# ma-compbio/MATCHA

Measured on AMD Instinct MI355X. Metric: training hyperedges/sec at k∈{2..5}, embed_dim=64; 1/2/4/8 MI355X, higher is better.
Workload: dtype f32; 1 GPU; hg38_1mb bins (N=3067), k in {2,3,4,5} mixed-k zero-padded to L=5, embed_dim=64, front end=table, neg_num=3, dropout on, AdamW lr=1e-3, 400000 known hyperedges; parallelism=dp1, hipgraph=False, table_gradient_exchange=none, embedding_backward=float atomics, exchange_overlapped=False

## Files before the change

### matcha_amd/csrc/fused_bwd.hip

```cpp
#include <stdlib.h>
#include <string.h>

#include <type_traits>

#include "bf16x3.hpp"
#include "kernels.hpp"
#include "tail_reduce.hpp"
#include "fb_unfold.hpp"

namespace matcha {

typedef float f32x16 __attribute__((ext_vector_type(16)));

namespace {

constexpr int kLd = 68;
constexpr int kMaxChunks = 64;
constexpr int kRsrcRaw32 = 0x00020000;
constexpr uint32_t kOffPastAny = 0x80000000u;

#define ZR8(p)                                                                                           \
  do {                                                                                                   \
    *reinterpret_cast<float4*>(p) = make_float4(0.f, 0.f, 0.f, 0.f);                                     \
    *reinterpret_cast<float4*>((p) + 4) = make_float4(0.f, 0.f, 0.f, 0.f);                               \
  } while (0)


#define FB_PIN(addr, x) asm volatile("" : "+v"(addr), "+v"((x).a), "+v"((x).b), "+v"((x).c), "+v"((x).d))
template <int ML>
__device__ __forceinline__ void attn_row8_kv(const float* __restrict__ Qs, const float* __restrict__ Xs, const float* __restrict__ Fs,
                                             const float* __restrict__ xpad, const float* __restrict__ Ps, float* __restrict__ dSs, int li, int li0,
                                             int k, int n_pad, int sub, float inv_temp, V8& o, V8& gq, V8& accK, V8& accV) {
  const float padf = (float)n_pad;
  const bool hp = n_pad > 0;
  float p[ML], ds[ML], pp;
  {
    const float4 pa = *reinterpret_cast<const float4*>(&Ps[li * 8]), pb = *reinterpret_cast<const float4*>(&Ps[li * 8 + 4]);
    const float w[8] = {pa.x, pa.y, pa.z, pa.w, pb.x, pb.y, pb.z, pb.w};
#pragma unroll
    for (int j = 0; j < ML; ++j) p[j] = (j < k) ? w[j] : 0.f;
    pp = hp ? w[7] : 0.f;
  }
  const float ppf = padf * pp;
  const int ro0 = li0 * kLd + 8 * sub;
  const V8 go = ld8(&Fs[li * kLd + 8 * sub]);
  const V8 vp = ld8(xpad + 8 * sub);
  const float dsp_raw = group_sum8_dpp(dot8(go, vp));
  float sig = ppf * dsp_raw;
  o = scale8(ppf, vp);
  V8 a = scale8(ppf * dsp_raw, vp);
  V8 vn = ld8(&Xs[ro0]), vn2 = ld8(&Xs[ro0 + (1 < k ? 1 : 0) * kLd]);
#pragma unroll
  for (int j = 0; j < ML; ++j) {
    const V8 v = vn;
    vn = vn2;
    if (j + 2 < ML) {
      int ad = ro0 + (j + 2 < k ? j + 2 : 0) * kLd;
      FB_PIN(ad, o);
      vn2 = ld8(&Xs[ad]);
    }
    axpy8(o, p[j], v);
    const float d = group_sum8_dpp(dot8(go, v));
    ds[j] = d;
    const float wd = p[j] * d;
    sig += wd;
    axpy8(a, wd, v);
  }
#pragma unroll
  for (int j = 0; j < ML; ++j) ds[j] = p[j] * (ds[j] - sig) * inv_temp;
  const float dspf = padf * (pp * (dsp_raw - sig) * inv_temp);
  axpy8(accV, ppf, go);
  {
    const float ns = -sig;
    axpy8(a, ns, o);
    gq = scale8(inv_temp, a);
  }
  {
    int ad = li * kLd + 8 * sub;
    FB_PIN(ad, gq);
    const V8 q = ld8(&Qs[ad]);
    axpy8(accK, dspf, q);
  }
  if (sub == 1) {
    float* dst = dSs + li * 8;
    *reinterpret_cast<float4*>(dst) = make_float4(ds[0], ds[1 % ML], ML > 2 ? ds[2 % ML] : 0.f, ML > 3 ? ds[3 % ML] : 0.f);
    if (ML > 4) *reinterpret_cast<float4*>(dst + 4) = make_float4(ds[4 % ML], ML > 5 ? ds[5 % ML] : 0.f, ML > 6 ? ds[6 % ML] : 0.f, ML > 7 ? ds[7 % ML] : 0.f);
  }
}

#define FB_PIN1(addr, s) asm volatile("" : "+v"(addr), "+v"(s))
template <int ML>
__device__ __forceinline__ void attn_row8_v(const float* __restrict__ Qs, const float* __restrict__ Xs, const float* __restrict__ Ys, const float* __restrict__ Ds,
                                            const float* __restrict__ xpad, const float* __restrict__ ypad, const float* __restrict__ Ps, float* __restrict__ dSs,
                                            int li, int li0, int k, int n_pad, int sub, float inv_temp, V8& gq, V8& accK, V8& accU) {
  const float padf = (float)n_pad;
  const bool hp = n_pad > 0;
  float p[ML], ds[ML], pp;
  {
    const float4 pa = *reinterpret_cast<const float4*>(&Ps[li * 8]), pb = *reinterpret_cast<const float4*>(&Ps[li * 8 + 4]);
    const float w[8] = {pa.x, pa.y, pa.z, pa.w, pb.x, pb.y, pb.z, pb.w};
#pragma unroll
    for (int j = 0; j < ML; ++j) p[j] = (j < k) ? w[j] : 0.f;
    pp = hp ? w[7] : 0.f;
  }
  const float ppf = padf * pp;
  const int ro0 = li0 * kLd + 8 * sub;
  const V8 go = ld8(&Ds[li * kLd + 8 * sub]);
  const float dsp_raw = group_sum8_dpp(dot8(go, ld8(ypad + 8 * sub)));
  float sig = ppf * dsp_raw;
  {
    V8 vn = ld8(&Ys[ro0]), vn2 = ld8(&Ys[ro0 + (1 < k ? 1 : 0) * kLd]);
    float part = 0.f;
#pragma unroll
    for (int j = 0; j < ML; ++j) {
      const V8 v = vn;
      vn = vn2;
      if (j + 2 < ML) {
        int ad = ro0 + (j + 2 < k ? j + 2 : 0) * kLd;
        FB_PIN1(ad, part);
        vn2 = ld8(&Ys[ad]);
      }
      part = dot8(go, v);
      const float d = group_sum8_dpp(part);
      ds[j] = d;
      sig += p[j] * d;
    }
  }
#pragma unroll
  for (int j = 0; j < ML; ++j) ds[j] = p[j] * (ds[j] - sig) * inv_temp;
  const float dspf = padf * (pp * (dsp_raw - sig) * inv_temp);
  axpy8(accU, ppf, go);
  gq = scale8(dspf, ld8(xpad + 8 * sub));
  {
    V8 vn = ld8(&Xs[ro0]), vn2 = ld8(&Xs[ro0 + (1 < k ? 1 : 0) * kLd]);
#pragma unroll
    for (int j = 0; j < ML; ++j) {
      const V8 v = vn;
      vn = vn2;
      if (j + 2 < ML) {
        int ad = ro0 + (j + 2 < k ? j + 2 : 0) * kLd;
        FB_PIN(ad, gq);
        vn2 = ld8(&Xs[ad]);
      }
      axpy8(gq, ds[j], v);
    }
  }
  {
    int ad = li * kLd + 8 * sub;
    FB_PIN(ad, gq);
    const V8 q = ld8(&Qs[ad]);
    axpy8(accK, dspf, q);
  }
  if (sub == 1) {
    float* dst = dSs + li * 8;
    *reinterpret_cast<float4*>(dst) = make_float4(ds[0], ds[1 % ML], ML > 2 ? ds[2 % ML] : 0.f, ML > 3 ? ds[3 % ML] : 0.f);
    if (ML > 4) *reinterpret_cast<float4*>(dst + 4) = make_float4(ds[4 % ML], ML > 5 ? ds[5 % ML] : 0.f, ML > 6 ? ds[6 % ML] : 0.f, ML > 7 ? ds[7 % ML] : 0.f);
  }
}

template <int ML>
__device__ __forceinline__ void attn_col8(const float* __restrict__ Qs, const float* __restrict__ Fs, const float* __restrict__ Ps,
                                          const float* __restrict__ dSs, int li, int li0, int k, int sub, V8& gk, V8& gv) {
  const int jj = li - li0;
  gk = zero8();
  gv = zero8();
  const int ro0 = li0 * kLd + 8 * sub;
  V8 qn = ld8(&Qs[ro0]), gn = ld8(&Fs[ro0]);
#pragma unroll
  for (int i = 0; i < ML; ++i) {
    const V8 q = qn, go = gn;
    const int ri = li0 + (i < k ? i : 0);
    const float pl = Ps[ri * 8 + jj], dl = dSs[ri * 8 + jj];
    const float pij = (i < k) ? pl : 0.f, dsij = (i < k) ? dl : 0.f;
    if (i + 1 < ML) {
      int a = ro0 + (i + 1 < k ? i + 1 : 0) * kLd;
      FB_PIN(a, gk);
      qn = ld8(&Qs[a]); gn = ld8(&Fs[a]);
    }
    axpy8(gv, pij, go);
    axpy8(gk, dsij, q);
  }
}

#ifdef FB_TIMING
#define FB_T(i) do { const long long now__ = wall_clock64(); tph[i] += now__ - tlast; tlast = now__; } while (0)
#else
#define FB_T(i) do { } while (0)
#endif

#define MFMA16(A, B, C) __builtin_amdgcn_mfma_f32_16x16x4f32((A), (B), (C), 0, 0, 0)

constexpr int kWgSlabM = 2 * 4096 + 4 * 64;
constexpr int kVecOffM = 2 * 4096;
constexpr int kTileH = 32 * kLd;
constexpr int kPS = 80;
constexpr int kPlane = 32 * kPS;
constexpr int kPT = 3 * kPlane;
typedef Planes<kPS, 16> PL;
__device__ __forceinline__ Frag3 frag_row(const short* __restrict__ p) { return PL::row(p); }
__device__ __forceinline__ void frag_store(short* __restrict__ p, const Frag3& f) { PL::store(p, f); }
__device__ __forceinline__ Frag3 frag_col(const short* __restrict__ p) { return PL::col(p); }

struct FusedBwdHArgs {
  const float* X; const float* dDyn; const int32_t* count; const int32_t* half_meta; const int32_t* tok_pos;
  int L; int nhalves; int nchunks;
  const float* mB; const float* mM;
  float* dxh; int64_t tcap;
  int dx_atomic;
  float* wslab;
  const float* rimg;
  const int32_t* xrow;
  const float* rn; int64_t rn_head;
  const float* vn;
  float* dx_node;
};
constexpr size_t kBwdLdsBytes = (size_t)2 * kTileH * 4 + (size_t)4 * kPT * 2 + (64 + 256 + 256 + 32 + 32) * 4;
static_assert(2 * kBwdLdsBytes <= 160 * 1024, "two workgroups per CU");

template <int ML, bool NODE, bool VTAB = false>
__global__ __launch_bounds__(256) __attribute__((amdgpu_waves_per_eu(2, 2))) void fused_bwdh_kernel(FusedBwdHArgs g) {
  static_assert(NODE || !VTAB, "the value table belongs to the node route");
  extern __shared__ __attribute__((aligned(16))) float lds[];
  float* Xs = lds;
  float* Gs = lds + kTileH;
  short* Xp = reinterpret_cast<short*>(lds + 2 * kTileH);
  short* Dp = Xp + kPT;
  short* RBp = Dp + kPT;
  short* FBp = RBp + kPT;
  float* Rs = reinterpret_cast<float*>(RBp);
  float* Fs = reinterpret_cast<float*>(FBp);
  float* Ds = reinterpret_cast<float*>(Dp);
  float* ypad = Ds + kTileH;
  float* sm = reinterpret_cast<float*>(FBp + kPT);
  float* xpad = sm;
  float* dSs = xpad + 64;
  float* Ps = dSs + 256;
  int* tinfo = reinterpret_cast<int*>(Ps + 256);
  int* keys_s = tinfo + 32;

  const int tid = threadIdx.x, lane = tid & 63, wave = tid >> 6;
  const int c16 = lane & 15, kq = lane >> 4;
  const int fb = 16 * wave;
  const int srow = tid >> 4, sc4 = (tid & 15) * 4;

  int head, chunk;
  if ((g.nchunks & 7) == 0) {
    const int xcd = blockIdx.x & 7, j = blockIdx.x >> 3;
    head = j & 7;
    chunk = (j >> 3) * 8 + xcd;
  } else {
    head = blockIdx.x & 7;
    chunk = blockIdx.x >> 3;
  }
  const int tr = g.count[1];
  int nh = g.count[3];
  if (nh > g.nhalves) nh = g.nhalves;
  const int per = (nh + g.nchunks - 1) / g.nchunks;
  const int tile_lo = chunk * per;
  const int tile_hi = (tile_lo + per < nh) ? tile_lo + per : nh;
  const float inv_temp = 0.125f;
#ifdef FB_TIMING
  long long tph[8] = {0, 0, 0, 0, 0, 0, 0, 0};
  long long tlast = wall_clock64();
#endif

  if (tid < 16) {
    const float4 xv = *reinterpret_cast<const float4*>(g.X + (NODE ? (int64_t)0 : (int64_t)tr * 64) + sc4);
    if constexpr (NODE) {
      *reinterpret_cast<float4*>(&xpad[sc4]) = xv;
    } else {
      float m, rs;
      ln_row16(xv, m, rs);
      *reinterpret_cast<float4*>(&xpad[sc4]) = make_float4((xv.x - m) * rs, (xv.y - m) * rs, (xv.z - m) * rs, (xv.w - m) * rs);
    }
  }
  if constexpr (VTAB) {
    static_assert((size_t)(kTileH + 64) * 4 <= (size_t)kPT * 2, "dDyn rows + y_pad fit the Dp region");
    if (tid >= 64 && tid < 80) *reinterpret_cast<float4*>(&ypad[sc4]) = *reinterpret_cast<const float4*>(g.vn + (int64_t)head * g.rn_head + sc4);
  }

  f32x4 ab0 = {0.f, 0.f, 0.f, 0.f}, ab1 = ab0, ab2 = ab0, ab3 = ab0, am0 = ab0, am1 = ab0, am2 = ab0, am3 = ab0;
  V8 accK = zero8(), accV = zero8();
  f2 cd0 = {0.f, 0.f}, cd1 = cd0;
  V8 accR = zero8();

  const int4* meta = reinterpret_cast<const int4*>(g.half_meta);
  const int4 mzero = make_int4(0, 0, 0, 0);
  int4 mc = tile_lo < tile_hi ? meta[tile_lo] : mzero;
// ... 63 lines not shown
      const P3 p0__ = split2(dm__.x, dm__.y), p1__ = split2(dm__.z, dm__.w);                             \
      short* d__ = Dp + row__ * kPS + sc4;                                                               \
      *reinterpret_cast<u32x2*>(d__) = (u32x2){p0__.h, p1__.h}; *reinterpret_cast<u32x2*>(d__ + kPlane) = (u32x2){p0__.m, p1__.m}; \
      *reinterpret_cast<u32x2*>(d__ + 2 * kPlane) = (u32x2){p0__.l, p1__.l};                             \
    }                                                                                                    \
    cd0 += (f2){dm__.x, dm__.y}; cd1 += (f2){dm__.z, dm__.w};                                            \
  } while (0)
#define FBH_RIMG_GLOAD(HALF)                                                                             \
  do {                                                                                                   \
    const f32x4* r__ = reinterpret_cast<const f32x4*>(g.rimg + ((int64_t)(HALF) * MATCHA_N_HEAD + head) * kImgRecH);  \
    if (tid < 64) pn = __builtin_nontemporal_load(r__ + 512 + tid);                                      \
    if (!r_tab) { ri0 = __builtin_nontemporal_load(r__ + tid); ri1 = __builtin_nontemporal_load(r__ + 256 + tid); } \
  } while (0)
  Frag3 Mf[2], Bf[2];
  {
    if constexpr (NODE) { FBH_KEY_GLOAD(0, mc); FBH_KEY_GLOAD(1, mc); }
    FBH_ROWS_GLOAD(mc, false);
    if constexpr (NODE) { if (r_tab) FBH_R_GLOAD(); FBH_KEY_GLOAD(0, mn); FBH_KEY_GLOAD(1, mn); }
    if (tile_lo < tile_hi) FBH_RIMG_GLOAD(tile_lo);
    const float* mp = g.mM + (int64_t)head * 4096 + (8 * kq) * 64 + fb + c16;
    const float* bp = g.mB + (int64_t)head * 4096 + (8 * kq) * 64 + fb + c16;
#pragma unroll
    for (int s = 0; s < 2; ++s) {
      float vm[8], vb[8];
#pragma unroll
      for (int j = 0; j < 8; ++j) { vm[j] = mp[(32 * s + j) * 64]; vb[j] = bp[(32 * s + j) * 64]; }
      Mf[s] = split8(vm); Bf[s] = split8(vb);
    }
  }

#define FBH_STAGE(M, DXN)                                                                                \
  do {                                                                                                   \
    const int n_real = (M).y;                                                                            \
    FBH_ROW_STAGE(0); FBH_ROW_STAGE(1);                                                                  \
    if (tid < 32) tinfo[tid] = tid < n_real ? ((tid - (tpn & 255)) | (tpn & ~255)) : 0;                  \
    if (((DXN) || (VTAB && g.dx_node)) && tid < 32) keys_s[tid] = kyn;                                   \
    if constexpr (VTAB) {                                                                                \
      *reinterpret_cast<f32x4*>(&Fs[srow * kLd + sc4]) = yi0; *reinterpret_cast<f32x4*>(&Fs[(srow + 16) * kLd + sc4]) = yi1; \
    }                                                                                                    \
    if (r_tab) {                                                                                         \
      *reinterpret_cast<f32x4*>(&Rs[srow * kLd + sc4]) = ri0; *reinterpret_cast<f32x4*>(&Rs[(srow + 16) * kLd + sc4]) = ri1; \
    } else {                                                                                             \
      f32x4* d__ = reinterpret_cast<f32x4*>(&Rs[(lane & 31) * kLd + 8 * wave + 4 * (lane >> 5)]);        \
      d__[0] = ri0; d__[8] = ri1;                                                                        \
    }                                                                                                    \
    if (tid < 64) reinterpret_cast<f32x4*>(Ps)[tid] = pn;                                                \
  } while (0)
  if (tile_lo < tile_hi) FBH_STAGE(mc, false);

  auto walk = [&](auto dxn_c) __attribute__((always_inline)) {
  constexpr bool DXN = decltype(dxn_c)::value;
  for (int tile = tile_lo; tile < tile_hi; ++tile) {
    const int4 mnn = tile + 2 < tile_hi ? meta[tile + 2] : mzero;
    const int t0 = mc.x, n_real = mc.y;
    __syncthreads();
    FB_T(7);
    int tid_ = tid;
    asm volatile("" : "+v"(tid_));
    const int lane = tid_ & 63, wave = tid_ >> 6;
    const int c16 = lane & 15, kq = lane >> 4;
    const int fb = 16 * wave;
    const int srow = tid_ >> 4, sc4 = (tid_ & 15) * 4;
    const int sub = lane & 7;
    (void)srow; (void)sc4;
    if constexpr (!VTAB) {
      f32x4 acc0 = {0.f, 0.f, 0.f, 0.f}, acc1 = acc0;
      const short* dp = Dp + c16 * kPS + 8 * kq;
#pragma unroll
      for (int s = 0; s < 2; ++s) {
        const Frag3 b0 = frag_row(dp + 32 * s), b1 = frag_row(dp + 16 * kPS + 32 * s);
        acc0 = mma6(acc0, Mf[s], b0); acc1 = mma6(acc1, Mf[s], b1);
      }
      *reinterpret_cast<f32x4*>(&Fs[c16 * kLd + fb + 4 * kq]) = acc0;
      *reinterpret_cast<f32x4*>(&Fs[(16 + c16) * kLd + fb + 4 * kq]) = acc1;
      FB_T(1);
      __syncthreads();
      FB_T(7);
    }
    if constexpr (VTAB) {
      FB_T(1);
      V8 q0, k0, v0;
      const int la = wave * 8 + (lane >> 3);
      const bool acta = la < n_real;
      int ia = 0;
      if (acta) { ia = tinfo[la]; attn_row8_v<ML>(Rs, Xs, Fs, Ds, xpad, ypad, Ps, dSs, la, ia & 255, ia >> 8, g.L - (ia >> 8), sub, inv_temp, q0, accK, accV); }
      __builtin_amdgcn_sched_barrier(0);
      FB_T(2);
      __syncthreads();
      FB_T(7);
      if (acta) {
        attn_col8<ML>(Rs, Ds, Ps, dSs, la, ia & 255, ia >> 8, sub, k0, v0);
        st8(&Gs[la * kLd + 8 * sub], k0);
      } else {
        ZR8(&Gs[la * kLd + 8 * sub]);
        v0 = zero8(); q0 = zero8();
      }
      frag_store(FBp + la * kPS + 8 * sub, split8(v0));
      FB_T(3);
      __syncthreads();
      FB_T(7);
      frag_store(RBp + la * kPS + 8 * sub, split8(q0));
      accR.a += q0.a; accR.b += q0.b; accR.c += q0.c; accR.d += q0.d;
    } else {
      V8 o0, q0, k0, v0;
      const int la = wave * 8 + (lane >> 3);
      const bool acta = la < n_real;
      int ia = 0;
      if (acta) { ia = tinfo[la]; attn_row8_kv<ML>(Rs, Xs, Fs, xpad, Ps, dSs, la, ia & 255, ia >> 8, g.L - (ia >> 8), sub, inv_temp, o0, q0, accK, accV); }
      __builtin_amdgcn_sched_barrier(0);
      FB_T(2);
      __syncthreads();
      FB_T(7);
      if (acta) {
        attn_col8<ML>(Rs, Fs, Ps, dSs, la, ia & 255, ia >> 8, sub, k0, v0);
        k0.a += v0.a; k0.b += v0.b; k0.c += v0.c; k0.d += v0.d;
        st8(&Gs[la * kLd + 8 * sub], k0);
      } else {
        ZR8(&Gs[la * kLd + 8 * sub]);
      }
      FB_T(3);
      __syncthreads();
      FB_T(7);
      if (!acta) { o0 = zero8(); q0 = zero8(); }
      frag_store(FBp + la * kPS + 8 * sub, split8(o0));
      frag_store(RBp + la * kPS + 8 * sub, split8(q0));
      accR.a += q0.a; accR.b += q0.b; accR.c += q0.c; accR.d += q0.d;
    }
    FB_T(4);
    __syncthreads();
    FB_T(7);
    FBH_ROWS_GLOAD(mn, DXN);
    if constexpr (NODE) { if (r_tab) FBH_R_GLOAD(); FBH_KEY_GLOAD(0, mnn); FBH_KEY_GLOAD(1, mnn); }
    if constexpr (DXN) { if (tile + 1 < tile_hi) FBH_RIMG_GLOAD(tile + 1); }
    if (DXN || g.dx_atomic) {
      const float* gp = Gs + (4 * kq) * kLd + fb + c16;
      f32x4 dx0 = {gp[0], gp[kLd], gp[2 * kLd], gp[3 * kLd]};
      f32x4 dx1 = {gp[16 * kLd], gp[17 * kLd], gp[18 * kLd], gp[19 * kLd]};
      const short* arow = RBp + c16 * kPS + 8 * kq;
#pragma unroll
      for (int s = 0; s < 2; ++s) {
        const Frag3 a0 = frag_row(arow + 32 * s), a1 = frag_row(arow + 16 * kPS + 32 * s);
        dx0 = mma6(dx0, a0, Bf[s]); dx1 = mma6(dx1, a1, Bf[s]);
      }
      if constexpr (VTAB) {
        const short* urow = FBp + c16 * kPS + 8 * kq;
#pragma unroll
        for (int s = 0; s < 2; ++s) {
          const Frag3 a0 = frag_row(urow + 32 * s), a1 = frag_row(urow + 16 * kPS + 32 * s);
          dx0 = mma6(dx0, a0, Mf[s]); dx1 = mma6(dx1, a1, Mf[s]);
        }
      }
      if constexpr (DXN) {
        const int4 ka = *reinterpret_cast<const int4*>(&keys_s[4 * kq]), kb = *reinterpret_cast<const int4*>(&keys_s[16 + 4 * kq]);
        const int k0[4] = {ka.x, ka.y, ka.z, ka.w}, k1[4] = {kb.x, kb.y, kb.z, kb.w};
        const __amdgpu_buffer_rsrc_t ah = __builtin_amdgcn_make_buffer_rsrc(g.dx_node + (int64_t)head * g.rn_head, 0, (int)(g.rn_head * 4), kRsrcRaw32);
        const uint32_t col4 = 4u * (uint32_t)(fb + c16);
#pragma unroll
        for (int reg = 0; reg < 4; ++reg) {
          __builtin_amdgcn_raw_ptr_buffer_atomic_fadd_f32(dx0[reg], ah, 4 * kq + reg < n_real ? (uint32_t)k0[reg] * 256u + col4 : kOffPastAny, 0, 0);
          __builtin_amdgcn_raw_ptr_buffer_atomic_fadd_f32(dx1[reg], ah, 16 + 4 * kq + reg < n_real ? (uint32_t)k1[reg] * 256u + col4 : kOffPastAny, 0, 0);
        }
      } else {
      float* out = g.dxh + ((int64_t)t0 + 4 * kq) * 64 + fb + c16;
#pragma unroll
      for (int reg = 0; reg < 4; ++reg) {
        if (4 * kq + reg < n_real) unsafeAtomicAdd(out + reg * 64, dx0[reg]);
        if (16 + 4 * kq + reg < n_real) unsafeAtomicAdd(out + (16 + reg) * 64, dx1[reg]);
      }
      }
    } else {
      f32x4 dx0 = *reinterpret_cast<const f32x4*>(&Gs[c16 * kLd + fb + 4 * kq]);
      f32x4 dx1 = *reinterpret_cast<const f32x4*>(&Gs[(16 + c16) * kLd + fb + 4 * kq]);
      const short* arow = RBp + c16 * kPS + 8 * kq;
#pragma unroll
      for (int s = 0; s < 2; ++s) {
        const Frag3 a0 = frag_row(arow + 32 * s), a1 = frag_row(arow + 16 * kPS + 32 * s);
        dx0 = mma6(dx0, Bf[s], a0); dx1 = mma6(dx1, Bf[s], a1);
      }
      if constexpr (VTAB) {
        const short* urow = FBp + c16 * kPS + 8 * kq;
#pragma unroll
        for (int s = 0; s < 2; ++s) {
          const Frag3 a0 = frag_row(urow + 32 * s), a1 = frag_row(urow + 16 * kPS + 32 * s);
          dx0 = mma6(dx0, Mf[s], a0); dx1 = mma6(dx1, Mf[s], a1);
        }
      }
      float* out = g.dxh + ((int64_t)head * g.tcap + t0 + c16) * 64 + fb + 4 * kq;
      if (c16 < n_real) *reinterpret_cast<f32x4*>(out) = dx0;
      if (16 + c16 < n_real) *reinterpret_cast<f32x4*>(out + 16 * 64) = dx1;
    }
    FB_T(5);
    if constexpr (!DXN) { if (tile + 1 < tile_hi) FBH_RIMG_GLOAD(tile + 1); }
    {
      const int blk = ((4 * kq + ((lane & 15) >> 2)) * kPS) + 4 * (lane & 3);
      const Frag3 xb = frag_col(Xp + blk + fb);
      Frag3 zb;
      if constexpr (!VTAB) zb = frag_col(FBp + blk + fb);
// ... 269 lines not shown
      dc += vb[mat * 64 + row];
      if (mat > 0) dpad += vb[192 + (mat - 1) * 64 + row];
    }
  fb_unfold_rows(a, slice, mat, head, s, dc, dpad, red);
}

__global__ __launch_bounds__(512) void fb_unfold2_kernel(Unfold2Args a) {
  fb_unfold2_vec(a, threadIdx.x >> 6, threadIdx.x & 63);
}

__global__ __launch_bounds__(256) void lnhat_bwd_kernel(const float* __restrict__ X, const float* __restrict__ dxh, int64_t tcap,
                                                        const float* __restrict__ dxpad, const float* __restrict__ dXs,
                                                        float* __restrict__ dZ0, const int32_t* __restrict__ count, int nslab) {
  const int T = count[0];
  const int64_t t = (int64_t)blockIdx.x * 16 + (threadIdx.x >> 4);
  const int c4 = (threadIdx.x & 15) * 4;
  if (t >= T) return;
  const float4 xv = *reinterpret_cast<const float4*>(X + t * 64 + c4);
  float m, rs;
  ln_row16(xv, m, rs);
  const float4 xh = make_float4((xv.x - m) * rs, (xv.y - m) * rs, (xv.z - m) * rs, (xv.w - m) * rs);
  float4 d;
  if (t < T - 1) {
    d = *reinterpret_cast<const float4*>(dxh + t * 64 + c4);
    for (int hd = 1; hd < nslab; ++hd) {
      const float4 v = *reinterpret_cast<const float4*>(dxh + ((int64_t)hd * tcap + t) * 64 + c4);
      d.x += v.x; d.y += v.y; d.z += v.z; d.w += v.w;
    }
  } else {
    d = *reinterpret_cast<const float4*>(dxpad + c4);
  }
  const float a = group_sum<16>((d.x + d.y) + (d.z + d.w)) * (1.f / 64.f);
  const float b = group_sum<16>((d.x * xh.x + d.y * xh.y) + (d.z * xh.z + d.w * xh.w)) * (1.f / 64.f);
  const float4 s = *reinterpret_cast<const float4*>(dXs + t * 64 + c4);
  float4 o;
  o.x = (rs * (d.x - a - xh.x * b) + s.x) * (1.f - xv.x * xv.x);
  o.y = (rs * (d.y - a - xh.y * b) + s.y) * (1.f - xv.y * xv.y);
  o.z = (rs * (d.z - a - xh.z * b) + s.z) * (1.f - xv.z * xv.z);
  o.w = (rs * (d.w - a - xh.w * b) + s.w) * (1.f - xv.w * xv.w);
  *reinterpret_cast<float4*>(dZ0 + t * 64 + c4) = o;
}

int chunks_for(int ntiles) {
  const int cus = device_cu_count();
  int c = cus / MATCHA_N_HEAD;
  if (c > kMaxChunks) c = kMaxChunks;
  if (c > ntiles) c = ntiles;
  return c < 1 ? 1 : c;
}

}

const float* fused_bwd_dxpad(const float* ws) { return ws + (size_t)MATCHA_N_HEAD * kMaxChunks * kWgSlab + 32 * 3 * 3 * 64; }

size_t fused_bwd_ws_floats(int64_t B, int L) {
  (void)B; (void)L;
  return (size_t)MATCHA_N_HEAD * kMaxChunks * kWgSlab + (size_t)32 * 3 * 3 * 64 + 64;
}

int launch_fused_bwd_merged(const matcha_tensors& p, const Ragged& rg, int64_t B, int L, const FusedBwdLaunch& a, matcha_tensors& grads, hipStream_t st) {
  const int64_t tcap = B * L + 1;
  const float *folded = a.folded, *X = a.x.X, *xhatN = a.x.xhat, *rn = a.x.rn, *vn = a.x.vn, *dXs = a.dXs;
  const int32_t* xrow = a.x.xrow;
  const bool dx_atomic = a.dx_atomic;
  float *dxh = a.dxh, *ws = a.ws;
  MATCHA_CHECK_ARG(!xrow || xhatN, "fused backward: the node route needs the table of normalised rows");
  MATCHA_CHECK_ARG(!rn || xrow, "fused backward: the r table belongs to the node route");
  MATCHA_CHECK_ARG(!vn || rn, "fused backward: the value table needs the r table");
  MATCHA_CHECK_ARG(!a.dx_node || (vn && dx_atomic && a.dx_zeroed), "fused backward: per-node d x_hat sums need the value table, the atomics and a caller that zeroed them");
  MATCHA_CHECK_ARG(!a.dx_node || a.x.rows * 256 < ((int64_t)1 << 31), "fused backward: a head's replica of the per-node sums is addressed through a buffer descriptor of < 2^31 bytes");
  if (dx_atomic && !a.dx_zeroed) MATCHA_TRY(zero_async(dxh, (size_t)tcap * 64 * sizeof(float), st));
  int nchunks = 2 * chunks_for(rg.nhalves);
  if (nchunks > kMaxChunks) nchunks = kMaxChunks;
  if (nchunks > rg.nhalves) nchunks = rg.nhalves > 0 ? rg.nhalves : 1;
  float* wslab = ws;
  float* chain = ws + (size_t)MATCHA_N_HEAD * kMaxChunks * kWgSlabM;
  float* part = ws + (size_t)MATCHA_N_HEAD * kMaxChunks * kWgSlab;
  float* dxpad = part + 32 * 3 * 3 * 64;
  const size_t wsz = (size_t)MATCHA_N_HEAD * 64 * 64, csz = (size_t)MATCHA_N_HEAD * 64;
  const MergedView mv = merged_view(a.merged);
  {
    FusedBwdHArgs g;
    g.X = xrow ? xhatN : X; g.dDyn = a.dDyn; g.count = rg.count; g.half_meta = rg.half_meta; g.tok_pos = rg.tok_pos; g.L = L; g.nhalves = rg.nhalves; g.nchunks = nchunks;
    g.mB = mv.B; g.mM = mv.M; g.dxh = dxh; g.tcap = tcap; g.dx_atomic = dx_atomic ? 1 : 0; g.wslab = wslab; g.rimg = a.rimg; g.xrow = xrow;
    g.rn = rn; g.rn_head = a.x.rows * 64; g.vn = vn; g.dx_node = a.dx_node ? dxh : nullptr;
    const size_t lds = kBwdLdsBytes;
    auto launch = [&](auto kfn) {
      (void)hipFuncSetAttribute(reinterpret_cast<const void*>(kfn), hipFuncAttributeMaxDynamicSharedMemorySize, 160 * 1024);
      hipLaunchKernelGGL(kfn, dim3(MATCHA_N_HEAD * nchunks), dim3(256), lds, st, g);
    };
    ProfScope ps(MATCHA_PROF_FUSED_BWD, (double)tcap * MATCHA_N_HEAD * 8.0 * 2.0 * 64.0 * 64.0, st);
    dispatch_ml(L, [&](auto ml) {
      constexpr int ML = decltype(ml)::value;
      if (vn) launch(fused_bwdh_kernel<ML, true, true>); else if (xrow) launch(fused_bwdh_kernel<ML, true>); else launch(fused_bwdh_kernel<ML, false>);
    });
    MATCHA_CHECK_LAUNCH("fused_bwdh_kernel");
  }
  {
    ChainArgs c;
    c.wslab = wslab; c.nchunks = nchunks; c.red = chain + (size_t)MATCHA_N_HEAD * kWgSlab;
    c.wq = folded; c.wk = folded + wsz; c.wv = folded + 2 * wsz; c.cq = folded + 3 * wsz; c.cv = c.cq + 2 * csz;
    c.fc1_w = p.fc1_w; c.out = chain; c.dxpad = dxpad;
    TailReduceArgs tl;
    if (a.tail) tl = *a.tail; else memset(&tl, 0, sizeof(tl));
    const int tail_blocks = a.tail ? kTailRoleBlocks : 0;
    hipLaunchKernelGGL(fbm_reduce_kernel, dim3((unsigned)(kFbmReduceBlocks + tail_blocks)), dim3(256), 0, st, c, tl, tail_blocks);
    MATCHA_CHECK_LAUNCH("fbm_reduce_kernel");
    UnfoldArgs u;
    u.wslab = chain; u.nchunks = 1; u.X = X; u.count = rg.count; u.x_pad_row0 = xrow ? 1 : 0;
    u.W[0] = p.w_q; u.W[1] = p.w_k; u.W[2] = p.w_v;
    u.g[0] = p.ln_q_g; u.g[1] = p.ln_k_g; u.g[2] = p.ln_v_g;
    u.b[0] = p.ln_q_b; u.b[1] = p.ln_k_b; u.b[2] = p.ln_v_b;
    u.gW[0] = grads.w_q; u.gW[1] = grads.w_k; u.gW[2] = grads.w_v; u.gfc1 = grads.fc1_w;
    u.part = part;
    MATCHA_CHECK_ARG(!a.unfold2 || a.paired, "fused backward: handing the final vectors on belongs to the paired launches");
    hipLaunchKernelGGL(fbm_chain_kernel, dim3(4, 4, MATCHA_N_HEAD), dim3(256), 0, st, c, u, a.paired ? 1 : 0, a.unfold2 ? 1 : 0);
    MATCHA_CHECK_LAUNCH("fbm_chain_kernel");
    if (!a.paired) {
      hipLaunchKernelGGL(fb_unfold_kernel, dim3(4, 4, MATCHA_N_HEAD), dim3(256), 0, st, u);
      MATCHA_CHECK_LAUNCH("fb_unfold_kernel");
    }
    Unfold2Args b;
    b.part = part; b.wslab = chain; b.nchunks = 1;
    b.dg[0] = grads.ln_q_g; b.dg[1] = grads.ln_k_g; b.dg[2] = grads.ln_v_g;
    b.db[0] = grads.ln_q_b; b.db[1] = grads.ln_k_b; b.db[2] = grads.ln_v_b;
    b.dfc1_b = grads.fc1_b; b.dxpad = dxpad; b.dxpad_add = a.unfold2 ? 2 : 1;
    if (a.unfold2) {
      *a.unfold2 = b;
    } else {
      hipLaunchKernelGGL(fb_unfold2_kernel, dim3(1), dim3(512), 0, st, b);
      MATCHA_CHECK_LAUNCH("fb_unfold2_kernel");
    }
  }
  if (float* dZ0 = a.dZ0) {
    MATCHA_CHECK_ARG(!xrow, "fused backward: the node route has no dZ0 output");
    hipLaunchKernelGGL(lnhat_bwd_kernel, dim3((unsigned)cdiv(tcap, 16)), dim3(256), 0, st, X, dxh, tcap, dxpad, dXs, dZ0, rg.count, dx_atomic ? 1 : MATCHA_N_HEAD);
    MATCHA_CHECK_LAUNCH("lnhat_bwd_kernel");
  }
  return MATCHA_OK;
}

}
```

### matcha_amd/csrc/fused_fwd32.hip

```cpp
#include "kernels.hpp"
#include "prep_heads.hpp"
#include "ragged_roles.hpp"

#ifndef F32_ABL
#define F32_ABL 0
#endif

namespace matcha {

typedef float f32x16 __attribute__((ext_vector_type(16)));

namespace {

constexpr int kLdH = 68;
constexpr int kHT = 32 * kLdH;
constexpr float kEps32 = 1e-5f;
constexpr int kTailVec32 = 2 * 4096;
constexpr int kTailSlab32 = 2 * 4096 + 10 * 64;

struct FL { f32x16 lo, hi; };

__device__ __forceinline__ float xhalf_sum(float v) {
  float a = v, b = v;
  asm volatile("s_nop 1\n\tv_permlane32_swap_b32 %0, %1" : "+v"(a), "+v"(b));
// ... 95 lines not shown
__device__ __forceinline__ FL fl_unpark_lds(const float* __restrict__ base, int off) {
  asm volatile("" : "+v"(off));
  return fl_load(base + off);
}
#define F32_WAVE_SYNC() asm volatile("s_waitcnt lgkmcnt(0)" ::: "memory")

#define MFMA32(A, B, C) __builtin_amdgcn_mfma_f32_32x32x2f32((A), (B), (C), 0, 0, 0)

#define MFMA_BF(A, B, C) __builtin_amdgcn_mfma_f32_32x32x16_bf16(__builtin_bit_cast(bf16x8, (A)), __builtin_bit_cast(bf16x8, (B)), (C), 0, 0, 0)
#ifndef F32_WIN
#define F32_WIN 6
#endif

struct B3 { u32x4 h, m, l; };
#define FL_CHUNK(V, C, J) ((C) < 2 ? (V).lo[8 * ((C) & 1) + (J)] : (V).hi[8 * ((C) & 1) + (J)])
#define FL_SPLIT(OUT, V, C)                                                                              \
  do {                                                                                                   \
    _Pragma("unroll") for (int q__ = 0; q__ < 4; ++q__) {                                                \
      if (F32_ABL & 128) { (OUT).h[q__] = __builtin_bit_cast(uint32_t, FL_CHUNK(V, C, 2 * q__)); (OUT).m[q__] = (OUT).h[q__]; (OUT).l[q__] = (OUT).h[q__]; continue; } \
      const P3 p__ = split2(FL_CHUNK(V, C, 2 * q__), FL_CHUNK(V, C, 2 * q__ + 1));                       \
      (OUT).h[q__] = p__.h; (OUT).m[q__] = p__.m; (OUT).l[q__] = p__.l;                                  \
    }                                                                                                    \
  } while (0)
#define WB_MMA(ACC, XB, S)                                                                               \
  do {                                                                                                   \
    const u32x4 ah__ = W_[(3 * (S)) % F32_WIN], am__ = W_[(3 * (S) + 1) % F32_WIN], al__ = W_[(3 * (S) + 2) % F32_WIN]; \
    if constexpr (((S) & 1) == 0) {                                                                      \
      ACC.lo = MFMA_BF(al__, (XB).h, ACC.lo); ACC.lo = MFMA_BF(ah__, (XB).l, ACC.lo); ACC.lo = MFMA_BF(am__, (XB).m, ACC.lo); \
      ACC.lo = MFMA_BF(am__, (XB).h, ACC.lo); ACC.lo = MFMA_BF(ah__, (XB).m, ACC.lo); ACC.lo = MFMA_BF(ah__, (XB).h, ACC.lo); \
    } else {                                                                                             \
      ACC.hi = MFMA_BF(al__, (XB).h, ACC.hi); ACC.hi = MFMA_BF(ah__, (XB).l, ACC.hi); ACC.hi = MFMA_BF(am__, (XB).m, ACC.hi); \
      ACC.hi = MFMA_BF(am__, (XB).h, ACC.hi); ACC.hi = MFMA_BF(ah__, (XB).m, ACC.hi); ACC.hi = MFMA_BF(ah__, (XB).h, ACC.hi); \
    }                                                                                                    \
  } while (0)
#define WB_REFILL(S, PF)                                                                                 \
  do {                                                                                                   \
    if ((PF) && !(F32_ABL & 32)) {                                                                       \
      W_[(3 * (S)) % F32_WIN] = wp[lane]; W_[(3 * (S) + 1) % F32_WIN] = (wp + 64)[lane]; W_[(3 * (S) + 2) % F32_WIN] = (wp + 128)[lane]; \
    }                                                                                                    \
    wp += 192;                                                                                           \
    asm volatile("" ::: "memory");          \
    __builtin_amdgcn_sched_barrier(0);                                                                   \
  } while (0)
#define WB_CHUNK(ACC, B, C, PF)                                                                          \
  do {                                                                                                   \
    B3 xb__;                                                                                             \
    FL_SPLIT(xb__, B, C);                                                                                \
    WB_MMA(ACC, xb__, 2 * (C)); WB_REFILL(2 * (C), PF); WB_MMA(ACC, xb__, 2 * (C) + 1); WB_REFILL(2 * (C) + 1, PF); \
  } while (0)
#define W32_CHAIN(ACC, B, PF_LAST)                                                                       \
  do { WB_CHUNK(ACC, B, 0, true); WB_CHUNK(ACC, B, 1, true); WB_CHUNK(ACC, B, 2, true); WB_CHUNK(ACC, B, 3, PF_LAST); } while (0)
#define W32_CHAIN_XS(ACC, XS, PF_LAST)                                                                   \
  do {                                                                                                   \
    WB_MMA(ACC, XS[0], 0); WB_REFILL(0, true); WB_MMA(ACC, XS[0], 1); WB_REFILL(1, true);                \
    WB_MMA(ACC, XS[1], 2); WB_REFILL(2, true); WB_MMA(ACC, XS[1], 3); WB_REFILL(3, true);                \
    WB_MMA(ACC, XS[2], 4); WB_REFILL(4, true); WB_MMA(ACC, XS[2], 5); WB_REFILL(5, true);                \
    WB_MMA(ACC, XS[3], 6); WB_REFILL(6, PF_LAST); WB_MMA(ACC, XS[3], 7); WB_REFILL(7, PF_LAST);          \
  } while (0)
#define W32_PRIME_AT(MAT)                                                                                \
  do {                                                                                                   \
    wp = g.wfrag + (MAT) * kFragU4;                                                                      \
    _Pragma("unroll") for (int i__ = 0; i__ < F32_WIN; ++i__) W_[i__] = (wp + i__ * 64)[lane];           \
    wp += F32_WIN * 64;                                                                                  \
  } while (0)

__device__ __forceinline__ FL fl_zero() {
  FL v;
#pragma unroll
  for (int e = 0; e < 16; ++e) { v.lo[e] = 0.f; v.hi[e] = 0.f; }
  return v;
}

}

__global__ __launch_bounds__(256) void prep_heads_kernel(PrepArgs a) {
  __shared__ __attribute__((aligned(16))) float sm[kPrepLdsFloats];
  prep_heads_role(a, blockIdx.x, blockIdx.y, blockIdx.z, sm);
}

struct Fwd32Args {
  const float* X;
  const int32_t* xrow;
  const int32_t* row_off; const int32_t* tok_slot; const int32_t* count; const int32_t* half_meta; const int32_t* tok_pos;
  int L;
  const u32x4* wfrag;
  HeadParams hp;
  const float* y; const float* w;
  float* Y; float* H1; float* H2;
  float* logits; float* row_loss;
  const uint64_t* seed;
  float p_fc1, p_pff;
  float* ddyn0; float* dXs; float* tslab; float alpha_over_B;
  int objective;
  float* qkv;
  float* tail_dh2;
  const float* rn;
  int rn_rows;
  float* dxs_node;
};

template <int ML>
__global__ __launch_bounds__(64) __attribute__((amdgpu_waves_per_eu(2, 2))) void fused_fwd32_kernel(Fwd32Args g) {
  extern __shared__ __attribute__((aligned(16))) float lds[];
#ifdef FF_TIMING
  long long tph[16] = {0};
  long long tlast = wall_clock64();
#define FF_T(i) do { const long long now__ = wall_clock64(); tph[i] += now__ - tlast; tlast = now__; } while (0)
#else
#define FF_T(i) do { } while (0)
#endif
  float* TK = lds;
  float* TV = lds + kHT;
  float* outs = lds + 2 * kHT;
  float* douts = outs + 32;
  const int lane = threadIdx.x, r = lane & 31, h = lane >> 5;

  const int4 meta = reinterpret_cast<const int4*>(g.half_meta)[blockIdx.x];
  const int t0 = meta.x, n = meta.y, b0 = meta.z, n_h = meta.w;
  if (n_h <= 0) return;
  const int tok_pad = g.count[1];
  const float inv_temp = 0.125f;
  const bool real = r < n;

  const u32x4* wp;
  u32x4 W_[F32_WIN];
  W32_PRIME_AT(g.rn ? 2 : 0);
  {
    const f32x4* bsrc = reinterpret_cast<const f32x4*>(g.wfrag + (kNMat + 1) * kFragU4);
    for (int i4 = lane; i4 < kNBias * 16; i4 += 64) reinterpret_cast<f32x4*>(TV)[i4] = bsrc[i4];
  }
#define F32_BIAS(ROW) fl_vec(TV + (ROW) * 64 + 4 * h)

  int64_t xoff = F32_ROW();
  if (g.xrow) xoff = (int64_t)g.xrow[F32_TOK()] * 64 + 4 * h;
  FL xh = fl_load(g.X + xoff);
  int pos = 0, k = 0;
  if (real) {
    const int tp = g.tok_pos[F32_TOK()];
    pos = tp & 255; k = tp >> 8;
  }
  const int li0 = r - pos;
  float rx;
  {
    float mean;
    fl_stats(xh, mean, rx);
#pragma unroll
    for (int e = 0; e < 16; ++e) { xh.lo[e] = (xh.lo[e] - mean) * rx; xh.hi[e] = (xh.hi[e] - mean) * rx; }
  }
  constexpr int kRec = kImgRecH;
  float* const img_base = g.qkv ? g.qkv + (int64_t)blockIdx.x * MATCHA_N_HEAD * kImgRecH : nullptr;
  const bool img_on = g.qkv != nullptr && real;
#define F32_IMG_STORE(ACC, HD, M)                                                                        \
  do {                                                                                                   \
    if (img_on && !(F32_ABL & 2)) {                                                                      \
      int l__ = lane;                                                                                    \
      asm volatile("" : "+v"(l__));                                                                      \
      f32x4* d__ = reinterpret_cast<f32x4*>(img_base + (HD) * kRec + (M) * 4096 + l__ * 4);             \
      _Pragma("unroll") for (int g__ = 0; g__ < 4; ++g__) {                                              \
        if (F32_ABL & 16) {                                                                              \
          d__[g__ * 64] = (f32x4){ACC.lo[4 * g__], ACC.lo[4 * g__ + 1], ACC.lo[4 * g__ + 2], ACC.lo[4 * g__ + 3]};   \
          d__[(4 + g__) * 64] = (f32x4){ACC.hi[4 * g__], ACC.hi[4 * g__ + 1], ACC.hi[4 * g__ + 2], ACC.hi[4 * g__ + 3]}; \
        } else {                                                                                         \
        __builtin_nontemporal_store((f32x4){ACC.lo[4 * g__], ACC.lo[4 * g__ + 1], ACC.lo[4 * g__ + 2], ACC.lo[4 * g__ + 3]}, d__ + g__ * 64); \
        __builtin_nontemporal_store((f32x4){ACC.hi[4 * g__], ACC.hi[4 * g__ + 1], ACC.hi[4 * g__ + 2], ACC.hi[4 * g__ + 3]}, d__ + (4 + g__) * 64); \
        }                                                                                                \
      }                                                                                                  \
// ... 299 lines not shown
struct NodeRArgs { const float* X; const u32x4* wfrag; float* rn; int rows; float* vn; int ncompact; CompactArgs compact; };
__global__ __launch_bounds__(64) void node_r_kernel(NodeRArgs g) {
  const int lane = threadIdx.x, r = lane & 31, h = lane >> 5;
  if ((int)blockIdx.y < g.ncompact) {
    __shared__ int offs[kCompactRoleSb + 1];
    tile_compact_role(g.compact, (int)blockIdx.x, (int)gridDim.x, lane, offs);
    return;
  }
  const int by = (int)blockIdx.y - g.ncompact;
  const int hd = by & 7;
  const bool vrole = by >= MATCHA_N_HEAD;
  const int row = (int)blockIdx.x * 32 + r;
  const bool live = row < g.rows;
  const u32x4* wp;
  u32x4 W_[F32_WIN];
  W32_PRIME_AT(vrole ? (hd < 7 ? 2 * hd + 2 : 15) : (hd == 0 ? 0 : 2 * hd - 1));
  FL xh = fl_load(g.X + (int64_t)(live ? row : g.rows - 1) * 64 + 4 * h);
  {
    float mean, rx;
    fl_stats(xh, mean, rx);
#pragma unroll
    for (int e = 0; e < 16; ++e) { xh.lo[e] = (xh.lo[e] - mean) * rx; xh.hi[e] = (xh.hi[e] - mean) * rx; }
  }
  B3 xs[4];
  FL_SPLIT(xs[0], xh, 0); FL_SPLIT(xs[1], xh, 1); FL_SPLIT(xs[2], xh, 2); FL_SPLIT(xs[3], xh, 3);
  FL q = F32_BIAS(kBiasR + hd);
  if (vrole) q = fl_zero();
  W32_CHAIN_XS(q, xs, false);
  if (live) fl_store_global((vrole ? g.vn : g.rn) + ((int64_t)hd * g.rows + row) * 64 + 4 * h, q);
}

size_t node_r_floats(int64_t rows) { return (size_t)MATCHA_N_HEAD * rows * 64; }
int launch_node_r(const float* XN, const float* frag, int64_t rows, float* rn, hipStream_t st, float* vn, const CompactArgs* compact) {
  NodeRArgs g;
  g.X = XN; g.wfrag = reinterpret_cast<const u32x4*>(frag); g.rn = rn; g.rows = (int)rows; g.vn = vn;
  g.ncompact = 0;
  g.compact = CompactArgs{};
  if (compact) {
    if (compact->first == 1 && compact->nsb <= kCompactRoleSb) { g.ncompact = 1; g.compact = *compact; }
    else MATCHA_TRY(launch_tile_compact(*compact, st));
  }
  ProfScope ps(MATCHA_PROF_FUSED_FWD, 0.0, st);
  hipLaunchKernelGGL(node_r_kernel, dim3((unsigned)cdiv(rows, 32), (vn ? 2 * MATCHA_N_HEAD : MATCHA_N_HEAD) + g.ncompact), dim3(64), 0, st, g);
  MATCHA_CHECK_LAUNCH("node_r_kernel");
  return MATCHA_OK;
}

static int fwd32h_max_halves() { return 2 * device_cu_count(); }

bool fused_small_batch(const Ragged& rg) { return rg.nhalves <= fwd32h_max_halves() && !options().disable_small_batch; }

size_t fused_frag_floats() { return (size_t)(kNMat + 1) * kFragU4 * 4 + (size_t)kNBias * 64; }
size_t fused_tail_slab32_floats(int64_t B, int L) { return (size_t)(ragged_halves_cap(B, L) + 2) * kTailSlab32; }

size_t fused_merged_floats() { return (size_t)2 * MATCHA_N_HEAD * 4096 + MATCHA_N_HEAD * 64 + 64; }
MergedView merged_view(const float* m) {
  return MergedView{m, m + (size_t)MATCHA_N_HEAD * 4096, m + (size_t)2 * MATCHA_N_HEAD * 4096, m + (size_t)2 * MATCHA_N_HEAD * 4096 + MATCHA_N_HEAD * 64};
}
void prep_heads_args(const matcha_tensors& p, float* folded, float* merged, float* frag, PrepArgs& a) {
  const size_t wsz = (size_t)MATCHA_N_HEAD * 64 * 64, csz = (size_t)MATCHA_N_HEAD * 64;
  a.Wq = p.w_q; a.Wk = p.w_k; a.Wv = p.w_v;
  a.gq = p.ln_q_g; a.gk = p.ln_k_g; a.gv = p.ln_v_g; a.bq = p.ln_q_b; a.bv = p.ln_v_b;
  a.fc1_w = p.fc1_w; a.fc1_b = p.fc1_b; a.p0w = p.pff0_w; a.p0b = p.pff0_b; a.p1w = p.pff1_w; a.p1b = p.pff1_b;
  a.fwq = folded; a.fwk = folded + wsz; a.fwv = folded + 2 * wsz; a.fcq = folded + 3 * wsz; a.fcv = a.fcq + 2 * csz;
  const MergedView v = merged_view(merged);
  a.B = const_cast<float*>(v.B); a.M = const_cast<float*>(v.M); a.bvec = const_cast<float*>(v.bvec); a.bdyn = const_cast<float*>(v.bdyn);
  a.frag = reinterpret_cast<u32x4*>(frag);
}
int launch_prep_heads(const matcha_tensors& p, float* folded, float* merged, float* frag, hipStream_t st) {
  PrepArgs a;
  prep_heads_args(p, folded, merged, frag, a);
  hipLaunchKernelGGL(prep_heads_kernel, dim3(kPrepGridX, kPrepGridY, kPrepGridZ), dim3(256), 0, st, a);
  MATCHA_CHECK_LAUNCH("prep_heads_kernel");
  return MATCHA_OK;
}

int launch_fused_fwd32(const matcha_tensors& p, const Ragged& rg, int64_t B, int L, const FusedFwdLaunch& a, hipStream_t st) {
  Fwd32Args g;
  g.xrow = a.x.xrow;
  MATCHA_CHECK_ARG(!a.x.rn || a.x.xrow, "fused forward: the r table belongs to the node route");
  g.rn = a.x.rn; g.rn_rows = (int)a.x.rows;
  g.tail_dh2 = nullptr; g.dxs_node = nullptr;
  g.X = a.x.X; g.row_off = rg.row_off; g.tok_slot = rg.tok_slot; g.count = rg.count; g.half_meta = rg.half_meta; g.tok_pos = rg.tok_pos;
  g.L = L;
  g.wfrag = reinterpret_cast<const u32x4*>(a.frag);
  g.hp = HeadParams{p.pff_ln_g, p.pff_ln_b, p.ln1_g, p.ln1_b, p.ln2_g, p.ln2_b, p.cls_w, p.cls_b};
  const bool target = a.objective == MATCHA_OBJECTIVE_SOFTPLUS_MSE ? a.y != nullptr : (a.y && a.w);
  g.objective = a.objective;
  g.y = a.y; g.w = a.w; g.Y = a.Y; g.H1 = a.H1; g.H2 = a.H2; g.logits = a.logits; g.row_loss = target ? a.row_loss : nullptr;
  g.seed = a.seed; g.p_fc1 = a.p_fc1; g.p_pff = a.p_pff;
  g.ddyn0 = target ? a.ddyn0 : nullptr; g.dXs = a.dXs; g.tslab = a.tslab; g.alpha_over_B = a.alpha / (float)B; g.qkv = a.rimg;
  ProfScope ps(MATCHA_PROF_FUSED_FWD, (double)(B * L + 1) * (MATCHA_N_HEAD * 4.0 + 2.0) * 2.0 * 64.0 * 64.0, st);
  if (a.small) {
    MATCHA_CHECK_ARG(!a.x.xrow, "fused forward: the node route runs the large-batch kernel only");
    const size_t ldsh = ((size_t)10 * kHT + 64) * sizeof(float);
    dispatch_ml(L, [&](auto ml) {
      auto kfn = fused_fwd32h_kernel<decltype(ml)::value>;
      (void)hipFuncSetAttribute(reinterpret_cast<const void*>(kfn), hipFuncAttributeMaxDynamicSharedMemorySize, (int)ldsh);
      hipLaunchKernelGGL(kfn, dim3(rg.nhalves), dim3(512), ldsh, st, g);
    });
    MATCHA_CHECK_LAUNCH("fused_fwd32h_kernel");
    return MATCHA_OK;
  }
  g.tail_dh2 = g.ddyn0 ? a.tail_dh2 : nullptr;
  MATCHA_CHECK_ARG(!a.dxs_node || (a.x.xrow && g.ddyn0), "fused forward: per-node dXs sums belong to the node route with the tail's backward in the kernel");
  g.dxs_node = a.dxs_node;
  const size_t lds = ((size_t)2 * kHT + 64) * sizeof(float);
  dispatch_ml(L, [&](auto ml) { hipLaunchKernelGGL(fused_fwd32_kernel<decltype(ml)::value>, dim3(rg.nhalves), dim3(64), lds, st, g); });
  MATCHA_CHECK_LAUNCH("fused_fwd32_kernel");
  return MATCHA_OK;
}

}
```

### matcha_amd/csrc/fused_fwd32_tail.hpp

```cpp
  uint32_t thr1 = 0, thr2 = 0, hrow1 = 0, hrow2 = 0;
  float ks1 = 1.f, ks2 = 1.f;
  const bool drop1 = g.p_fc1 > 0.f, drop2 = g.p_pff > 0.f;
  if (drop1 || drop2) {
    const uint32_t slot = (uint32_t)g.tok_slot[F32_TOK()];
    const uint64_t seed = *g.seed;
    hrow1 = lowbias32(slot ^ rng_key(seed, kStreamDropFc1));
    hrow2 = lowbias32(slot ^ rng_key(seed, kStreamDropPff));
    if (drop1) { thr1 = dropout_threshold(g.p_fc1); ks1 = 1.f / (1.f - g.p_fc1); }
    if (drop2) { thr2 = dropout_threshold(g.p_pff); ks2 = 1.f / (1.f - g.p_pff); }
  }
  F32_TAIL_SYNC();
  for (int i4 = lane; i4 < 112; i4 += 64) {
    const int v = i4 >> 4;
    const float* src = (v == 0 ? g.hp.gp : v == 1 ? g.hp.bp : v == 2 ? g.hp.g1 : v == 3 ? g.hp.b1 : v == 4 ? g.hp.g2 : v == 5 ? g.hp.b2 : g.hp.wc) + 4 * (i4 & 15);
    *reinterpret_cast<f32x4*>(TV + 4 * i4) = *reinterpret_cast<const f32x4*>(src);
  }
  float* T1 = TK;
  float* T2 = TV;
  float* myrow = krow;
  const float* tpar = T2 + 4 * h;
  uint32_t keep1 = 0, keep2 = 0;
  FL y;
  {
#pragma unroll
    for (int e = 0; e < 32; ++e) {
      const int f = 32 * (e >> 4) + 8 * ((e >> 2) & 3) + (e & 3);
      float v = e < 16 ? dyn.lo[e] : dyn.hi[e - 16];
      const bool kp = lowbias32((uint32_t)(f + 4 * h) ^ hrow1) >= thr1;
      keep1 |= kp ? (1u << e) : 0u;
      v = (kp && real) ? v * ks1 : 0.f;
      if (e < 16) y.lo[e] = v; else y.hi[e - 16] = v;
    }
    F32_PARK_Y(y);
  }
  FL h1 = F32_BIAS(kBiasConv0);
  W32_CHAIN(h1, y, true);
  {
#pragma unroll
    for (int e = 0; e < 32; ++e) {
      const int f = 32 * (e >> 4) + 8 * ((e >> 2) & 3) + (e & 3);
      float v = fast_tanh(e < 16 ? h1.lo[e] : h1.hi[e - 16]);
      const bool kp = lowbias32((uint32_t)(f + 4 * h) ^ hrow2) >= thr2;
      keep2 |= kp ? (1u << e) : 0u;
      v = kp ? v * ks2 : 0.f;
      if (e < 16) h1.lo[e] = v; else h1.hi[e - 16] = v;
    }
    F32_PARK_H1(h1);
  }
  FL h2 = y;
  {
    const FL b1v = F32_BIAS(kBiasConv1);
#pragma unroll
    for (int e = 0; e < 16; ++e) { h2.lo[e] += b1v.lo[e]; h2.hi[e] += b1v.hi[e]; }
  }
  W32_CHAIN(h2, h1, false);
  if (g.H2 && !g.ddyn0 && r <= n) fl_store_global(g.H2 + F32_ROW(), h2);
  FF_T(7);
  F32_TAIL_SYNC();
  float rh, ru;
  FL uh;
  {
    FL hh;
    {
      float mh;
      fl_stats(h2, mh, rh);
#pragma unroll
      for (int e = 0; e < 16; ++e) { hh.lo[e] = (h2.lo[e] - mh) * rh; hh.hi[e] = (h2.hi[e] - mh) * rh; }
    }
    FL u;
    const FL Gp = fl_vec(tpar + 0 * 64), Bp = fl_vec(tpar + 1 * 64);
#pragma unroll
    for (int e = 0; e < 16; ++e) { u.lo[e] = hh.lo[e] * Gp.lo[e] + Bp.lo[e]; u.hi[e] = hh.hi[e] * Gp.hi[e] + Bp.hi[e]; }
    if (g.ddyn0) F32_PARK_HH(hh);
    float mu;
    fl_stats(u, mu, ru);
#pragma unroll
    for (int e = 0; e < 16; ++e) { uh.lo[e] = (u.lo[e] - mu) * ru; uh.hi[e] = (u.hi[e] - mu) * ru; }
  }
  F32_XH_RELOAD();
  FL df;
  {
    const FL G1 = fl_vec(tpar + 2 * 64), B1 = fl_vec(tpar + 3 * 64);
    const FL G2 = fl_vec(tpar + 4 * 64), B2 = fl_vec(tpar + 5 * 64);
#pragma unroll
    for (int e = 0; e < 16; ++e) {
      df.lo[e] = (uh.lo[e] * G1.lo[e] + B1.lo[e]) - (xh.lo[e] * G2.lo[e] + B2.lo[e]);
      df.hi[e] = (uh.hi[e] * G1.hi[e] + B1.hi[e]) - (xh.hi[e] * G2.hi[e] + B2.hi[e]);
    }
  }
  {
    const FL Wc = fl_vec(tpar + 6 * 64);
    float s0 = 0.f, s1 = 0.f;
#pragma unroll
    for (int e = 0; e < 16; ++e) { s0 += df.lo[e] * df.lo[e] * Wc.lo[e]; s1 += df.hi[e] * df.hi[e] * Wc.hi[e]; }
    const float o = xhalf_sum(s0 + s1) + g.hp.bc[0];
    if (h == 0) outs[r] = real ? o : 0.f;
  }
  F32_TAIL_SYNC();
  for (int e = lane; e < n_h; e += 64) {
    const int64_t b = b0 + e;
    const int lo_g = g.row_off[b];
    const int lo = lo_g - t0, kk = g.row_off[b + 1] - lo_g;
    float yb = 0.f, wb = 0.f;
    const bool mse = g.objective == MATCHA_OBJECTIVE_SOFTPLUS_MSE;
    if (g.row_loss) { yb = g.y[b]; wb = mse ? 0.f : g.w[b]; }
    float tot = 0.f;
    for (int i = 0; i < kk; ++i) tot += outs[lo + i];
    const float z = tot / ((float)kk + 1e-15f);
    g.logits[b] = z;
    float dz = 0.f;
    if (mse) {
      const float big = z > 20.f ? 1.f : 0.f;
      const float err = (big != 0.f ? z : log1pf(expf(z))) - yb;
      if (g.row_loss) g.row_loss[b] = err * err;
      dz = g.alpha_over_B * 2.f * err * (big != 0.f ? 1.f : 1.f / (1.f + expf(-z)));
    } else {
      if (g.row_loss) g.row_loss[b] = wb * (fmaxf(z, 0.f) - z * yb + log1pf(expf(-fabsf(z))));
      if (g.ddyn0) dz = g.alpha_over_B * wb * (1.f / (1.f + expf(-z)) - yb);
    }
    if (g.ddyn0) {
      const float dout = dz / ((float)kk + 1e-15f);
      for (int i = 0; i < kk; ++i) douts[lo + i] = dout;
    }
  }
  FF_T(8);
  if (!g.ddyn0 || (F32_ABL & 4)) return;

  F32_TAIL_SYNC();
  const float dout = real ? douts[r] : 0.f;
  float* tsl = g.tslab + (int64_t)blockIdx.x * kTailSlab32;
#define F32_COLSUM(V, SLOT)                                                                              \
  do {                                                                                                   \
    F32_TAIL_SYNC();                                                                                     \
    fl_store(myrow, V);                                                                                  \
    F32_TAIL_SYNC();                                                                                     \
    float c0__ = 0.f, c1__ = 0.f, c2__ = 0.f, c3__ = 0.f;                                                \
    _Pragma("unroll") for (int t__ = 0; t__ < 32; t__ += 4) {                                            \
      c0__ += T1[t__ * kLdH + lane]; c1__ += T1[(t__ + 1) * kLdH + lane];                                \
      c2__ += T1[(t__ + 2) * kLdH + lane]; c3__ += T1[(t__ + 3) * kLdH + lane];                          \
    }                                                                                                    \
    cs_last = (c0__ + c1__) + (c2__ + c3__);                                                             \
    tsl[kTailVec32 + (SLOT) * 64 + lane] = cs_last;                                                      \
  } while (0)
  float cs_last = 0.f, db1 = 0.f;
  FL dh2;
  {
    FL ddn;
    {
      const FL Wc = fl_vec(tpar + 6 * 64);
      FL aw;
#pragma unroll
      for (int e = 0; e < 16; ++e) {
        aw.lo[e] = df.lo[e] * df.lo[e] * dout; aw.hi[e] = df.hi[e] * df.hi[e] * dout;
        ddn.lo[e] = 2.f * df.lo[e] * Wc.lo[e] * dout; ddn.hi[e] = 2.f * df.hi[e] * Wc.hi[e] * dout;
      }
      F32_COLSUM(aw, 6);
    }
    {
      const FL G2 = fl_vec(tpar + 4 * 64);
      FL t;
#pragma unroll
      for (int e = 0; e < 16; ++e) { t.lo[e] = -ddn.lo[e] * xh.lo[e]; t.hi[e] = -ddn.hi[e] * xh.hi[e]; }
      F32_COLSUM(t, 4);
#pragma unroll
      for (int e = 0; e < 16; ++e) { t.lo[e] = -ddn.lo[e] * G2.lo[e]; t.hi[e] = -ddn.hi[e] * G2.hi[e]; }
      const float a = xhalf_sum(fl_sum(t)) * (1.f / 64.f), b = xhalf_sum(fl_dot(t, xh)) * (1.f / 64.f);
#pragma unroll
      for (int e = 0; e < 16; ++e) { t.lo[e] = rx * (t.lo[e] - a - xh.lo[e] * b); t.hi[e] = rx * (t.hi[e] - a - xh.hi[e] * b); }
      F32_DXS_OUT(t);
    }
    {
      FL t;
#pragma unroll
      for (int e = 0; e < 16; ++e) { t.lo[e] = ddn.lo[e] * uh.lo[e]; t.hi[e] = ddn.hi[e] * uh.hi[e]; }
      F32_COLSUM(t, 2);
      F32_COLSUM(ddn, 3);
      db1 = cs_last;
    }
    FL du;
    {
      const FL G1 = fl_vec(tpar + 2 * 64);
#pragma unroll
      for (int e = 0; e < 16; ++e) { du.lo[e] = ddn.lo[e] * G1.lo[e]; du.hi[e] = ddn.hi[e] * G1.hi[e]; }
      const float a = xhalf_sum(fl_sum(du)) * (1.f / 64.f), b = xhalf_sum(fl_dot(du, uh)) * (1.f / 64.f);
#pragma unroll
// ... 100 lines not shown
```

### matcha_amd/csrc/kernels.hpp

```cpp
#pragma once
#include "common.hpp"

namespace matcha {

struct GemmArgs {
  const float* A[3];
  const float* B[3];
  float* C[3];
  int64_t M, N, K;
  int64_t lda, ldb, ldc;
  int batch;
  int flags;
  const float* bias[3];
  const float* residual;
  const float* aux;
  const int64_t* row_ids;
  const uint64_t* seed;
  uint32_t stream_id;
  float p_drop;
  float aux_scale;
  const int32_t* m_dev;
  const int32_t* a_row_map;
  const int32_t* c_row_map;
  const int32_t* seg;
  int n_groups;
  int64_t b_group_stride;
  const int32_t* rng_row_map;
};

struct Ragged {
  int32_t* row_off;
  int32_t* tok_slot;
  int64_t* tok_id;
  int32_t* count;
  int32_t* blk_sum;
  int nblk;
  int ntiles;
  int32_t* tok_pos;
  int32_t* tok_key;
  int32_t* tile_meta;
  int32_t* sb_tiles;
  int32_t* sb_cnt;
  int32_t* sb_first;
  int nsb, sb_cap;
  int32_t* half_meta;
  int32_t* tok_tile;
  int32_t* sb_htiles;
  int32_t* sb_hcnt;
  int nhalves, sb_hcap;
};
size_t ragged_bytes(int64_t B, int L);
int ragged_tiles_cap(int64_t B, int L);
int ragged_halves_cap(int64_t B, int L);
void ragged_carve(int64_t B, int L, char* base, Ragged& r);
struct PlanDeferred; struct TilePackArgs; struct CompactArgs;
int launch_ragged_plan(const int64_t* x, int64_t B, int L, int64_t n_nodes, int32_t* status, const Ragged& r, hipStream_t st, int level = 2,
                       int64_t* node_ids = nullptr, int32_t* node_cnt = nullptr, float* node_zero = nullptr,
                       PlanDeferred* defer = nullptr);

struct HeadParams {
  const float *gp, *bp, *g1, *b1, *g2, *b2, *wc, *bc;
};

int launch_gemm_rm(bool b_kn, const GemmArgs& g, hipStream_t st);
size_t gemm_tn_ws_bytes(int64_t M, int64_t N, int64_t R);
int launch_gemm_tn(const float* A, const float* B, float* C, float* colsum, int64_t M, int64_t N, int64_t R, int64_t lda,
                   int64_t ldb, const int64_t* b_gather, bool accumulate, void* ws, size_t ws_bytes, hipStream_t st,
                   const int32_t* r_dev = nullptr, const float* out_scale_dev = nullptr, float out_scale = 1.f);
int launch_slab_reduce(const float* slab, float* out1, int64_t n1, float* out2, int64_t stride, int P, bool accumulate, hipStream_t st,
                       const float* scale_dev = nullptr, float scale = 1.f);

struct BmmProduct {
  const float* A; int64_t a_rs, a_cs, a_hs;
  const float* B; int64_t b_rs, b_cs, b_hs;
  float* C; int64_t c_rs, c_hs;
  int accumulate;
};
bool bmm_heads_supported(int d);
int launch_bmm_heads(const BmmProduct* prods, int n, int d, hipStream_t st);

bool gemm_wide_eligible(bool b_kn, const GemmArgs& g);
int launch_gemm_wide(bool b_kn, const GemmArgs& g, hipStream_t st);
bool gemm_tn_wide_eligible(int64_t M, int64_t N, int64_t R, int64_t lda, int64_t ldb, const float* A, const float* B, const int64_t* b_gather);
size_t gemm_tn_wide_ws_bytes(int64_t M, int64_t N, int64_t R);
int launch_gemm_tn_wide(const float* A, const float* B, int64_t M, int64_t N, int64_t R, int64_t lda, int64_t ldb, bool colsum, void* ws,
                        size_t ws_bytes, const int32_t* r_dev, int* P_out, int64_t* slab_stride_out, hipStream_t st);

int launch_embed_fwd(const int64_t* x, int64_t T, int d, const float* table, const float* dense, const matcha_frozen& f,
                     int n_attr, const float* Wa, const float* ba, float* x0, hipStream_t st, const int32_t* t_dev = nullptr);
int launch_embed_scatter(const int64_t* x, int64_t T, int d, const float* dx0, float* dtable, hipStream_t st, const int32_t* t_dev = nullptr);
int launch_gather_rows(const int64_t* ids, int64_t T, int d, const float* table, int64_t n_nodes, float* rows, int32_t* status, hipStream_t st);
int launch_check_ids(const int64_t* ids, int64_t T, int64_t n_nodes, int32_t* status, hipStream_t st);
int launch_expand_embedding(const int64_t* x, int64_t B, int L, int d, const int32_t* row_off, const float* H2, const float* X, const float* gp,
                            const float* bp, float* dynamic, float* static_, hipStream_t st);

size_t table_grad_ws_bytes(int64_t n, int n_nodes);
int launch_table_grad(const int32_t* ids, const float* rows, int64_t n, int d, int n_nodes, float* dtable, void* ws, size_t ws_bytes, hipStream_t st);

struct Options {
  int disable_fused;
  int disable_merged;
  int disable_small_batch;
  int disable_wide_gemm;
  int disable_node_front;
  int disable_node_r;
  int disable_node_v;
  int disable_node_dx;
  int disable_launch_pairs;
  int debug_nan, fused_dbg;
};
Options& options();
int launch_fill_i32(int32_t* p, int n, int32_t v, hipStream_t st);
int zero_async(void* p, size_t bytes, hipStream_t st);
int launch_ln3_fwd(const float* X, int64_t T, int d, const float* gq, const float* bq, const float* gk, const float* bk,
                   const float* gv, const float* bv, float* qin, float* kin, float* vin, float* stats, hipStream_t st,
                   const int32_t* t_dev = nullptr);
int launch_ln3_bwd(const float* X, const float* dqin, const float* dkin, const float* dvin, const float* dXs, int64_t T, int d,
                   const float* gq, const float* gk, const float* gv, float* dZ0, float* slab, float* dgq, float* dbq,
                   float* dgk, float* dbk, float* dgv, float* dbv, hipStream_t st, const int32_t* t_dev = nullptr);
int launch_head_fwd(const int32_t* row_off, const float* H2, const float* X, int64_t B, int L, int d, const HeadParams& hp,
                    const float* y, const float* w, float* logits, float* row_loss, float* bce_out, hipStream_t st,
                    int objective = MATCHA_OBJECTIVE_BCE);
int launch_head_bwd(const int32_t* row_off, const float* H2, const float* X, int64_t B, int L, int d, const HeadParams& hp,
                    const float* y, const float* w, const float* logits, const float* dlogits, float alpha, float* dH2,
                    float* dXs, float* slab, const HeadParams& ghp, hipStream_t st, int objective = MATCHA_OBJECTIVE_BCE,
                    const int32_t* xrow = nullptr);
int launch_head_scores(const int32_t* row_off, const int32_t* tok_slot, const float* H2, const float* X, int64_t B, int L, int d,
                       const HeadParams& hp, float* scores, float* logits, int lowest, int64_t* order, hipStream_t st);
size_t colsum_slab_bytes(int64_t n, int nv, int d);
int launch_loss_reduce(const float* row_loss, int64_t B, float* bce_out, hipStream_t st, bool zero_recon = false,
                       float* zero_buf = nullptr, size_t zero_bytes = 0);

size_t fused_fold_floats();
size_t fused_tail_slab_floats(int64_t B, int L);
size_t fused_tail_partial_floats();
int launch_tail_reduce(const float* tslab, const Ragged& rg, int L, matcha_tensors& grads, hipStream_t st, bool halves, float* partial);
bool fused_small_batch(const Ragged& rg);

size_t fused_frag_floats();
size_t fused_tail_slab32_floats(int64_t B, int L);
size_t fused_merged_floats();
struct MergedView { const float* B; const float* M; const float* bvec; const float* bdyn; };
MergedView merged_view(const float* merged);
int launch_prep_heads(const matcha_tensors& p, float* folded, float* merged, float* frag, hipStream_t st);
struct NodeOperands {
  float* X;
  const int32_t* xrow;
  float* xhat;
  float* rn;
  float* vn;
  int64_t rows;
};
struct FusedFwdLaunch {
  const float* frag;
  NodeOperands x;
  bool small;
  const float *y, *w;
  int objective;
  float *Y, *H1, *H2;
  float *logits, *row_loss;
  const uint64_t* seed; float p_fc1, p_pff;
  float *ddyn0, *dXs, *tslab; float alpha;
  float* rimg;
  float* tail_dh2;
  float* dxs_node = nullptr;
};
int launch_fused_fwd32(const matcha_tensors& p, const Ragged& rg, int64_t B, int L, const FusedFwdLaunch& a, hipStream_t st);
size_t node_r_floats(int64_t rows);
int launch_node_r(const float* XN, const float* frag, int64_t rows, float* rn, hipStream_t st, float* vn = nullptr, const CompactArgs* compact = nullptr);
int tail_bwd_grid();
size_t tail_bwd_slab_floats();
int launch_tail_bwd64(const matcha_tensors& p, const float* dH2, const float* Y, const float* H1, const Ragged& rg, const uint64_t* seed, float p_fc1,
                      float p_pff, float* ddyn0, float* slab, const float* vslab, float* zero_rows, int64_t zero_floats, hipStream_t st,
                      const float* row_loss = nullptr, int64_t B = 0, float* losses = nullptr, bool zero_recon = false);

size_t fused_bwd_ws_floats(int64_t B, int L);
struct TailReduceArgs;
struct Unfold2Args;
struct FusedBwdLaunch {
  const float *folded, *merged;
  NodeOperands x;
  const float *dDyn, *dXs;
  const float* rimg;
  float* dxh;
  float* ws;
  float* dZ0;
  bool dx_atomic, dx_zeroed;
  bool dx_node = false;
  const TailReduceArgs* tail;
  bool paired = false;
  Unfold2Args* unfold2 = nullptr;
};
int launch_fused_bwd_merged(const matcha_tensors& p, const Ragged& rg, int64_t B, int L, const FusedBwdLaunch& a, matcha_tensors& grads, hipStream_t st);
size_t fused_qkv_floats(int64_t B, int L);
constexpr int kImgRecH = 2048 + 256;

const float* fused_bwd_dxpad(const float* ws);

bool enc128_shape(int d);
size_t enc128_ws_floats();
size_t enc128_rec_floats(const Ragged& rg);
int launch_enc128_fwd(const matcha_tensors& p, const float* lwB, const float* lwM, const float* X, const Ragged& rg, int64_t B, int L, float* Y, float* rec,
                      float* ws, const int32_t* tok_slot, const uint64_t* seed, float p_drop, hipStream_t st);
int launch_enc128_bwd(const matcha_tensors& p, const float* lwB, const float* lwM, const float* X, const float* dDyn, const float* dXs, const Ragged& rg,
                      int64_t B, int L, float* dxh, const float* rec, float* ws, float* lwdB, float* lwdM, matcha_tensors& grads, float* dZ0,
                      hipStream_t st);

bool front_bwd_supported(int d, int n_attr);
struct PrepSpec { const matcha_tensors* p; float* folded; float* merged; float* frag; };
int launch_front_fwd(const matcha_tensors& p, const int64_t* ids, const float* table, const float* dense, const matcha_frozen& f, int n_attr,
                     const Ragged& rg, int64_t tcap, float* x0, float* X, hipStream_t st, const PrepSpec* prep = nullptr,
                     const int32_t* count = nullptr,
                     const TilePackArgs* pack = nullptr);
size_t front_bwd_ws_floats();
int launch_front_bwd(const matcha_tensors& p, const float* X, const float* dxh, int nslab, int64_t tcap, const float* dxpad, const float* dXs, const float* x0,
                     const int64_t* ids, const matcha_frozen& f, int n_attr, const Ragged& rg, float* dX0, float* dtable, float* ws,
                     matcha_tensors& grads, hipStream_t st, int32_t* touched = nullptr,
                     const int32_t* node_count = nullptr);
int launch_node_xhat(const float* XN, const int32_t* node_count, int64_t rows_cap, float* xhatN, hipStream_t st);
int launch_node_scatter(const float* XN, const float* dxh, const float* dxpad, const float* dXs, const Ragged& rg, int64_t tcap, float* G, hipStream_t st,
                        const int32_t* node_count = nullptr, int64_t rows = 0,
                        const Unfold2Args* unfold2 = nullptr);

int launch_attn_fwd(const float* Q, const float* K, const float* V, const int32_t* row_off, int64_t B, int L, int d, float* O, float* P,
                    hipStream_t st, bool shared_kv = false);
int launch_attn_bwd(const float* Q, const float* K, const float* V, const float* P, const float* dO, const int32_t* row_off, int64_t B, int L,
                    int d, float* dQ, float* dK, float* dV, float* slab, hipStream_t st, bool shared_kv = false, float* dKsum = nullptr,
                    float* dVsum = nullptr);
size_t attn_bwd_slab_bytes(int64_t B, int d);
bool attn_wide_eligible(int d);
int launch_attn_fwd_wide(const float* Q, const float* K, const float* V, const int32_t* row_off, int64_t B, int L, int d, float inv_temp, float* O,
                         float* P, int nblk, hipStream_t st, bool shared_kv = false);
int launch_attn_bwd_wide(const float* Q, const float* K, const float* V, const float* P, const float* dO, const int32_t* row_off, int64_t B, int L,
                         int d, float inv_temp, float* dQ, float* dK, float* dV, float* slab, int nblk, hipStream_t st, bool shared_kv = false,
                         float* dKs = nullptr, float* dVs = nullptr);

size_t long_plan_bytes(int64_t B, int L);
void long_plan_carve(int64_t B, int L, char* base, Ragged& r, uint32_t** mask);
int launch_long_plan(const int64_t* x, int64_t B, int L, int64_t n_nodes, int32_t* status, const Ragged& r, uint32_t* mask, hipStream_t st);
int launch_attn_long(const float* Q, const float* K, const float* V, const int32_t* row_off, int64_t B, int L, int d, int64_t kv_ld, int kv_head,
                     float* O, hipStream_t st, const uint32_t* mask = nullptr, float* attn = nullptr);
size_t attn_long_bwd_slab_bytes(int64_t B, int d);
int launch_attn_long_bwd(const float* Q, const float* K, const float* V, const float* dO, const int32_t* row_off, int64_t B, int L, int d,
                         int64_t kv_ld, int kv_head, float* dQ, float* dK, float* dV, float* slab, hipStream_t st);

}
```

### matcha_amd/csrc/layerwise.hip

```cpp
#include <string.h>

#include <mutex>

#include "layerwise.hpp"

namespace matcha {

GemmArgs gemm1(const TokenChain& w, const float* A, const float* B, float* C, int64_t M, int64_t N, int64_t K, bool b_kn) {
  GemmArgs g;
  memset(&g, 0, sizeof(g));
  g.A[0] = A; g.B[0] = B; g.C[0] = C; g.batch = 1;
  g.M = M; g.N = N; g.K = K; g.lda = K; g.ldb = b_kn ? N : K; g.ldc = N;
  g.aux_scale = 1.f;
  g.m_dev = w.rg.count;
  g.rng_row_map = w.rg.tok_slot;
  return g;
}

int merged_weights(const matcha_shape& s, const matcha_tensors& p, const TokenChain& w, hipStream_t st) {
  const int64_t d = s.d, hd = (int64_t)MATCHA_N_HEAD * d;
  const BmmProduct pr[2] = {
      {p.w_k, 1, d, d * d, p.w_q, d, 1, d * d, w.lwB, d, d * d, 0},
      {p.fc1_w, hd, 1, d, p.w_v, d, 1, d * d, w.lwM, hd, d, 0}};
  return launch_bmm_heads(pr, 2, s.d, st);
// ... 102 lines not shown
    if (recon_out && zero_recon) MATCHA_TRY(zero_async(recon_out, 2 * sizeof(float), c.st));
  } else {
    MATCHA_TRY(adj_forward(s, p, c.f, c.o, w.rg.tok_id, Tn, w.node, recon_out, w.adj_ws, w.adj_ws_bytes, c.st, w.rg.count, w.rg.tok_slot));
  }
  MATCHA_TRY(launch_embed_fwd(w.rg.tok_id, Tn, d, s.mode == 0 ? p.table : nullptr, s.mode == 0 ? nullptr : w.node, c.f, s.n_attr, p.attr_w, p.attr_b, w.x0,
                              c.st, w.rg.count));
  GemmArgs g = gemm1(w, w.x0, p.next_w, w.X, Tn, d, d);
  g.flags = MATCHA_EPI_BIAS | MATCHA_EPI_TANH; g.bias[0] = p.next_b;
  MATCHA_TRY(launch_gemm_rm(false, g, c.st));
  nan_check("x0", w.x0, w.rg.count, 0, d, c.st);
  nan_check("X", w.X, w.rg.count, 0, d, c.st);
  return MATCHA_OK;
}

int chain_attn_fwd(const ChainCall& c, const TokenChain& w) {
  const matcha_shape& s = c.s;
  const matcha_tensors& p = c.p;
  const int64_t Tn = c.Tn(), B = c.B;
  const int d = s.d, L = c.L;
  const int64_t hd = (int64_t)MATCHA_N_HEAD * d;
  const int32_t* cnt = w.rg.count;
  const bool train = c.o.training != 0;
  MATCHA_TRY(launch_ln3_fwd(w.X, Tn, d, p.ln_q_g, p.ln_q_b, p.ln_k_g, p.ln_k_b, p.ln_v_g, p.ln_v_b, w.qin, w.kin, w.vin, w.stats, c.st, cnt));
  if (c.c.merged) {
    MATCHA_TRY(merged_weights(s, p, w, c.st));
    GemmArgs g = gemm1(w, w.qin, w.lwB, w.Q, Tn, hd, d);
    MATCHA_TRY(launch_gemm_rm(false, g, c.st));
  } else {
    GemmArgs g = gemm1(w, w.qin, p.w_q, w.Q, Tn, hd, d);
    g.A[1] = w.kin; g.B[1] = p.w_k; g.C[1] = w.K;
    g.A[2] = w.vin; g.B[2] = p.w_v; g.C[2] = w.V;
    g.batch = 3;
    MATCHA_TRY(launch_gemm_rm(false, g, c.st));
  }
  nan_check("qin", w.qin, cnt, 0, d, c.st);
  nan_check("Q", w.Q, cnt, 0, hd, c.st);
  nan_check("K", w.K, cnt, 0, hd, c.st);
  nan_check("V", w.V, cnt, 0, hd, c.st);
  if (c.c.long_attn) {
    if (c.c.merged) MATCHA_TRY(launch_attn_long(w.Q, w.kin, w.vin, w.rg.row_off, B, L, d, d, 0, w.O, c.st, w.mask, w.P));
    else MATCHA_TRY(launch_attn_long(w.Q, w.K, w.V, w.rg.row_off, B, L, d, hd, d, w.O, c.st, w.mask, w.P));
    if (c.c.keep) MATCHA_TRY(launch_long_zero_row(w.O, w.rg.row_off + B, hd, c.st));
  } else {
    if (c.c.merged) MATCHA_TRY(launch_attn_fwd(w.Q, w.kin, w.vin, w.rg.row_off, B, L, d, w.O, w.P, c.st, true));
    else MATCHA_TRY(launch_attn_fwd(w.Q, w.K, w.V, w.rg.row_off, B, L, d, w.O, w.P, c.st));
  }
  nan_check("O", w.O, cnt + 1, 0, hd, c.st);
  GemmArgs g = gemm1(w, w.O, c.c.merged ? w.lwM : p.fc1_w, w.Y, Tn, d, hd);
  g.flags = MATCHA_EPI_BIAS | MATCHA_EPI_ROWMASK; g.bias[0] = p.fc1_b; g.row_ids = w.rg.tok_id;
  if (train && c.o.p_drop_fc1 > 0.f) { g.flags |= MATCHA_EPI_DROPOUT; g.seed = c.o.seed; g.stream_id = kStreamDropFc1; g.p_drop = c.o.p_drop_fc1; }
  return launch_gemm_rm(false, g, c.st);
}

int chain_tail_fwd(const ChainCall& c, const TokenChain& w, const float* y, const float* w_bce, float* logits, float* losses, int objective,
                   bool stop_before_head) {
  const matcha_tensors& p = c.p;
  const int64_t Tn = c.Tn();
  const int d = c.s.d;
  const bool train = c.o.training != 0;
  {
    GemmArgs g = gemm1(w, w.Y, p.pff0_w, w.H1, Tn, d, d);
    g.flags = MATCHA_EPI_BIAS | MATCHA_EPI_TANH; g.bias[0] = p.pff0_b;
    if (train && c.o.p_drop_pff > 0.f) { g.flags |= MATCHA_EPI_DROPOUT; g.seed = c.o.seed; g.stream_id = kStreamDropPff; g.p_drop = c.o.p_drop_pff; }
    MATCHA_TRY(launch_gemm_rm(false, g, c.st));
  }
  {
    GemmArgs g = gemm1(w, w.H1, p.pff1_w, w.H2, Tn, d, d);
    g.flags = MATCHA_EPI_BIAS | MATCHA_EPI_RESIDUAL; g.bias[0] = p.pff1_b; g.residual = w.Y;
    MATCHA_TRY(launch_gemm_rm(false, g, c.st));
  }
  nan_check("Y", w.Y, w.rg.count, 0, d, c.st);
  nan_check("H1", w.H1, w.rg.count, 0, d, c.st);
  nan_check("H2", w.H2, w.rg.count, 0, d, c.st);
  if (stop_before_head) return MATCHA_OK;
  HeadParams hp = {p.pff_ln_g, p.pff_ln_b, p.ln1_g, p.ln1_b, p.ln2_g, p.ln2_b, p.cls_w, p.cls_b};
  MATCHA_TRY(launch_head_fwd(w.rg.row_off, w.H2, w.X, c.B, c.L, d, hp, y, w_bce, w.logits ? w.logits : logits, w.row_loss, losses, c.st, objective));
  if (w.logits && logits && hipMemcpyAsync(logits, w.logits, c.B * sizeof(float), hipMemcpyDeviceToDevice, c.st) != hipSuccess) {
    set_error("%s: logits copy failed", c.fn); return MATCHA_EHIP;
  }
  return MATCHA_OK;
}

int chain_tail_bwd(const ChainCall& c, const TokenChain& w, const float* X, const int32_t* xrow, const float* y, const float* w_bce, const float* dlogits,
                   int objective, matcha_tensors& g_) {
  const matcha_tensors& p = c.p;
  const int64_t Tn = c.Tn();
  const int d = c.s.d;
  const int32_t* cnt = w.rg.count;
  const bool train = c.o.training != 0;
  const bool drop_fc1 = train && c.o.p_drop_fc1 > 0.f, drop_pff = train && c.o.p_drop_pff > 0.f;
  HeadParams hp = {p.pff_ln_g, p.pff_ln_b, p.ln1_g, p.ln1_b, p.ln2_g, p.ln2_b, p.cls_w, p.cls_b};
  HeadParams ghp = {g_.pff_ln_g, g_.pff_ln_b, g_.ln1_g, g_.ln1_b, g_.ln2_g, g_.ln2_b, g_.cls_w, g_.cls_b};
  MATCHA_TRY(launch_head_bwd(w.rg.row_off, w.H2, X, c.B, c.L, d, hp, y, w_bce, w.logits, dlogits, c.o.alpha, w.dH2, w.dXs, w.slab, ghp, c.st, objective, xrow));
  MATCHA_TRY(launch_gemm_tn(w.dH2, w.H1, g_.pff1_w, g_.pff1_b, d, d, Tn, d, d, nullptr, true, w.gemm_ws, w.gemm_ws_bytes, c.st, cnt));
  {
    GemmArgs g = gemm1(w, w.dH2, p.pff1_w, w.dZ1, Tn, d, d, true);
    g.flags = MATCHA_EPI_DTANH; g.aux = w.H1;
    if (drop_pff) { g.flags |= MATCHA_EPI_DROPOUT; g.seed = c.o.seed; g.stream_id = kStreamDropPff; g.p_drop = c.o.p_drop_pff; g.aux_scale = 1.f - c.o.p_drop_pff; }
    MATCHA_TRY(launch_gemm_rm(true, g, c.st));
  }
  MATCHA_TRY(launch_gemm_tn(w.dZ1, w.Y, g_.pff0_w, g_.pff0_b, d, d, Tn, d, d, nullptr, true, w.gemm_ws, w.gemm_ws_bytes, c.st, cnt));
  GemmArgs g = gemm1(w, w.dZ1, p.pff0_w, w.ddyn0, Tn, d, d, true);
  g.flags = MATCHA_EPI_RESIDUAL | MATCHA_EPI_ROWMASK; g.residual = w.dH2; g.row_ids = w.rg.tok_id;
  if (drop_fc1) { g.flags |= MATCHA_EPI_DROPOUT; g.seed = c.o.seed; g.stream_id = kStreamDropFc1; g.p_drop = c.o.p_drop_fc1; }
  return launch_gemm_rm(true, g, c.st);
}

int chain_attn_bwd(const ChainCall& c, const TokenChain& w, matcha_tensors& g_) {
  const matcha_shape& s = c.s;
  const matcha_tensors& p = c.p;
  const int64_t Tn = c.Tn(), B = c.B;
  const int d = s.d, L = c.L;
  const int64_t hd = (int64_t)MATCHA_N_HEAD * d;
  const int32_t* cnt = w.rg.count;
  if (c.c.merged) {
    MATCHA_TRY(zero_async(w.lwdM, (size_t)hd * d * sizeof(float), c.st));
    MATCHA_TRY(zero_async(w.lwdB, (size_t)hd * d * sizeof(float), c.st));
    MATCHA_TRY(launch_gemm_tn(w.ddyn0, w.O, w.lwdM, g_.fc1_b, d, hd, Tn, d, hd, nullptr, true, w.gemm_ws, w.gemm_ws_bytes, c.st, cnt));
    {
      GemmArgs g = gemm1(w, w.ddyn0, w.lwM, w.dO, Tn, hd, d, true);
      MATCHA_TRY(launch_gemm_rm(true, g, c.st));
    }
    if (c.c.long_attn) MATCHA_TRY(launch_attn_long_bwd(w.Q, w.kin, w.vin, w.dO, w.rg.row_off, B, L, d, d, 0, w.dQ, w.dkin, w.dvin, w.slab, c.st));
    else MATCHA_TRY(launch_attn_bwd(w.Q, w.kin, w.vin, w.P, w.dO, w.rg.row_off, B, L, d, w.dQ, w.dK, w.dV, w.slab, c.st, true, w.dkin, w.dvin));
    MATCHA_TRY(launch_gemm_tn(w.dQ, w.qin, w.lwdB, nullptr, hd, d, Tn, hd, d, nullptr, true, w.gemm_ws, w.gemm_ws_bytes, c.st, cnt));
    {
      GemmArgs g = gemm1(w, w.dQ, w.lwB, w.dqin, Tn, d, hd, true);
      MATCHA_TRY(launch_gemm_rm(true, g, c.st));
    }
    MATCHA_TRY(merged_chain(s, p, g_, w, c.st));
  } else {
    MATCHA_TRY(launch_gemm_tn(w.ddyn0, w.O, g_.fc1_w, g_.fc1_b, d, hd, Tn, d, hd, nullptr, true, w.gemm_ws, w.gemm_ws_bytes, c.st, cnt));
    {
      GemmArgs g = gemm1(w, w.ddyn0, p.fc1_w, w.dO, Tn, hd, d, true);
      MATCHA_TRY(launch_gemm_rm(true, g, c.st));
    }
    if (c.c.long_attn) MATCHA_TRY(launch_attn_long_bwd(w.Q, w.K, w.V, w.dO, w.rg.row_off, B, L, d, hd, d, w.dQ, w.dK, w.dV, w.slab, c.st));
    else MATCHA_TRY(launch_attn_bwd(w.Q, w.K, w.V, w.P, w.dO, w.rg.row_off, B, L, d, w.dQ, w.dK, w.dV, w.slab, c.st));
    MATCHA_TRY(launch_gemm_tn(w.dQ, w.qin, g_.w_q, nullptr, hd, d, Tn, hd, d, nullptr, true, w.gemm_ws, w.gemm_ws_bytes, c.st, cnt));
    MATCHA_TRY(launch_gemm_tn(w.dK, w.kin, g_.w_k, nullptr, hd, d, Tn, hd, d, nullptr, true, w.gemm_ws, w.gemm_ws_bytes, c.st, cnt));
    MATCHA_TRY(launch_gemm_tn(w.dV, w.vin, g_.w_v, nullptr, hd, d, Tn, hd, d, nullptr, true, w.gemm_ws, w.gemm_ws_bytes, c.st, cnt));
    GemmArgs g = gemm1(w, w.dQ, p.w_q, w.dqin, Tn, d, hd, true);
    g.A[1] = w.dK; g.B[1] = p.w_k; g.C[1] = w.dkin;
    g.A[2] = w.dV; g.B[2] = p.w_v; g.C[2] = w.dvin;
    g.batch = 3;
    MATCHA_TRY(launch_gemm_rm(true, g, c.st));
  }
  MATCHA_TRY(launch_ln3_bwd(w.X, w.dqin, w.dkin, w.dvin, w.dXs, Tn, d, p.ln_q_g, p.ln_k_g, p.ln_v_g, w.dZ0, w.slab, g_.ln_q_g, g_.ln_q_b, g_.ln_k_g,
                            g_.ln_k_b, g_.ln_v_g, g_.ln_v_b, c.st, cnt));
  return encoder_done(c.o, c.st, c.fn);
}

int chain_front_bwd(const ChainCall& c, const TokenChain& w, const float* drecon, matcha_tensors& g_, int32_t* touched) {
  const matcha_shape& s = c.s;
  const int64_t Tn = c.Tn();
  const int d = s.d;
  const int32_t* cnt = w.rg.count;
  const int64_t* ids = w.rg.tok_id;
  MATCHA_TRY(launch_gemm_tn(w.dZ0, w.x0, g_.next_w, g_.next_b, d, d, Tn, d, d, nullptr, true, w.gemm_ws, w.gemm_ws_bytes, c.st, cnt));
  {
    GemmArgs g = gemm1(w, w.dZ0, c.p.next_w, w.dX0, Tn, d, d, true);
    MATCHA_TRY(launch_gemm_rm(true, g, c.st));
  }
  MATCHA_CHECK_ARG(c.f.attr_table, "%s: the layer-by-layer attribute_nn backward gathers attr_table rows (also under attr_mode 1)", c.fn);
  MATCHA_TRY(launch_gemm_tn(w.dX0, c.f.attr_table, g_.attr_w, g_.attr_b, d, s.n_attr, Tn, d, c.f.attr_ld > 0 ? c.f.attr_ld : s.n_attr, ids, true,
                            w.gemm_ws, w.gemm_ws_bytes, c.st, cnt));
  if (s.mode == 0) {
    MATCHA_CHECK_ARG(g_.table, "%s: table mode without a table gradient buffer", c.fn);
    if (c.o.deterministic || c.o.sparse_table_grad) MATCHA_TRY(table_gradient(s, c.o, w, Tn, g_, c.st));
    else MATCHA_TRY(launch_embed_scatter(ids, Tn, d, w.dX0, g_.table, c.st, cnt));
    if (touched) MATCHA_TRY(launch_fill_i32(touched, 2, 1, c.st));
    return MATCHA_OK;
  }
  return adj_backward(s, c.p, c.f, c.o, ids, Tn, w.dX0, drecon, g_, touched, w.adj_ws, w.adj_ws_bytes, w.gemm_ws, w.gemm_ws_bytes, c.st, w.rg.tok_slot);
}

// ... 26 lines not shown
```

### matcha_amd/csrc/layerwise.hpp

```cpp
#pragma once
#include <unordered_map>
#include <utility>

#include "kernels.hpp"

namespace matcha {

int adj_forward(const matcha_shape& s, const matcha_tensors& p, const matcha_frozen& f, const matcha_step_opts& o, const int64_t* x, int64_t T,
                float* node_out, float* recon_out, void* ws, size_t ws_bytes, hipStream_t st, const int32_t* t_dev, const int32_t* slot_map,
                float* fused_x0 = nullptr, float* fused_X = nullptr, bool save = false, bool fused_node = false);
int adj_backward(const matcha_shape& s, const matcha_tensors& p, const matcha_frozen& f, const matcha_step_opts& o, const int64_t* x, int64_t T,
                 float* dnode, const float* drecon, matcha_tensors& g, int32_t* touched, void* ws, size_t ws_bytes, void* gemm_ws,
                 size_t gemm_ws_bytes, hipStream_t st, const int32_t* slot_map, bool fused = false);
size_t adj_workspace_bytes(const matcha_shape& s, int64_t T);

struct TokenChain {
  Ragged rg;
  float *x0, *X, *qin, *kin, *vin, *stats, *Q, *K, *V, *P, *O, *Y, *H1, *H2, *row_loss, *logits, *node;
  float *dH2, *dXs, *dZ1, *ddyn0, *dO, *dQ, *dK, *dV, *dqin, *dkin, *dvin, *dZ0, *dX0;
  float* slab;      size_t slab_bytes;
  float* gemm_ws;   size_t gemm_ws_bytes;
  void* adj_ws;     size_t adj_ws_bytes;
  void* tg_ws;      size_t tg_ws_bytes;
  float *lwB, *lwM, *lwdB, *lwdM;
  uint32_t* mask;
};

struct ChainOpts {
  bool merged;
  bool long_attn;
  bool keep;
};

struct ChainCall {
  const matcha_shape& s; const matcha_tensors& p; const matcha_frozen& f; const matcha_step_opts& o;
  int64_t B; int L; hipStream_t st; ChainOpts c; const char* fn;
  int64_t Tn() const { return B * L + 1; }
};

GemmArgs gemm1(const TokenChain& w, const float* A, const float* B, float* C, int64_t M, int64_t N, int64_t K, bool b_kn = false);
int merged_weights(const matcha_shape& s, const matcha_tensors& p, const TokenChain& w, hipStream_t st);
int merged_chain(const matcha_shape& s, const matcha_tensors& p, matcha_tensors& g, const TokenChain& w, hipStream_t st);
void chain_scratch_bytes(const matcha_shape& s, int64_t B, int L, bool long_attn, TokenChain& w);
int check_shape_fields(const matcha_shape* s, const char* fn);
int check_chain_params(const matcha_tensors& p, const matcha_frozen& f, const char* fn);

int chain_front_fwd(const ChainCall& c, const TokenChain& w, float* recon_out, bool zero_recon);
int chain_attn_fwd(const ChainCall& c, const TokenChain& w);
int chain_tail_fwd(const ChainCall& c, const TokenChain& w, const float* y, const float* w_bce, float* logits, float* losses, int objective,
                   bool stop_before_head);
int chain_tail_bwd(const ChainCall& c, const TokenChain& w, const float* X, const int32_t* xrow, const float* y, const float* w_bce, const float* dlogits,
                   int objective, matcha_tensors& g);
int chain_attn_bwd(const ChainCall& c, const TokenChain& w, matcha_tensors& g);
int chain_front_bwd(const ChainCall& c, const TokenChain& w, const float* drecon, matcha_tensors& g, int32_t* touched);

int table_gradient(const matcha_shape& s, const matcha_step_opts& o, const TokenChain& w, int64_t Tn, matcha_tensors& g, hipStream_t st);
int encoder_done(const matcha_step_opts& o, hipStream_t st, const char* fn = "matcha_backward");
void nan_check(const char* name, const float* p, const int32_t* rows_dev, int64_t rows, int64_t width, hipStream_t st);

struct StepRoute {
  bool compact;
  bool half_plan;
  bool fused;
  bool merged_layerwise, enc128;
  bool front, adj_fused;
  bool small;
  bool lif;
  bool split_tail, dx_zeroed;
  bool node;
  bool node_r, node_v;
  bool node_dx;
  bool paired;
  bool long_rows;
};
extern std::unordered_map<const void*, std::pair<StepRoute, uint64_t>> g_fwd_state;
void note_forward(const void* ws, const StepRoute& route);
bool recorded_route(const void* ws, StepRoute& route);
void forget_forward(const void* ws);

}
```

### matcha_amd/csrc/model.hip

```cpp
#include <stdlib.h>
#include <string.h>

#include <unordered_map>

#include "layerwise.hpp"
#include "tail_reduce.hpp"
#include "fb_unfold.hpp"
#include "ragged_roles.hpp"

namespace matcha {

thread_local char g_err[512] = "";
void set_error(const char* fmt, ...) {
  va_list ap;
  va_start(ap, fmt);
  vsnprintf(g_err, sizeof(g_err), fmt, ap);
  va_end(ap);
}

int device_cu_count() {
  static int cache[64] = {};
  int dev = 0;
  if (hipGetDevice(&dev) != hipSuccess) { (void)hipGetLastError(); return 256; }
  if (dev >= 0 && dev < 64 && cache[dev] > 0) return cache[dev];
  int n = 0;
  if (hipDeviceGetAttribute(&n, hipDeviceAttributeMultiprocessorCount, dev) != hipSuccess || n <= 0) { (void)hipGetLastError(); return 256; }
  if (dev >= 0 && dev < 64) cache[dev] = n;
  return n;
}

int g_prof_class = 0;
static hipEvent_t* g_prof_ev = nullptr;
static int g_prof_cap = 0, g_prof_used = 0;
static double g_prof_work = 0.0;
void prof_record(bool start, double work, hipStream_t st) {
  if (start) {
    if (g_prof_used + 2 > g_prof_cap) {
      const int ncap = g_prof_cap ? 2 * g_prof_cap : 1024;
      hipEvent_t* ne = (hipEvent_t*)realloc(g_prof_ev, sizeof(hipEvent_t) * ncap);
      if (!ne) return;
      g_prof_ev = ne;
      for (int i = g_prof_cap; i < ncap; ++i)
        if (hipEventCreate(&g_prof_ev[i]) != hipSuccess) { g_prof_cap = i & ~1; return; }
      g_prof_cap = ncap;
    }
    g_prof_work += work;
    (void)hipEventRecord(g_prof_ev[g_prof_used], st);
  } else if (g_prof_used + 1 < g_prof_cap) {
    (void)hipEventRecord(g_prof_ev[g_prof_used + 1], st);
    g_prof_used += 2;
  }
}

int g_launch_log = 0;
namespace {
struct LaunchCount { const char* name; int64_t n; };
constexpr int kLaunchNames = 128;
LaunchCount g_launches[kLaunchNames];
int g_launch_names = 0;
}
void note_launch(const char* name) {
  for (int i = 0; i < g_launch_names; ++i)
    if (g_launches[i].name == name || strcmp(g_launches[i].name, name) == 0) { ++g_launches[i].n; return; }
  if (g_launch_names < kLaunchNames) g_launches[g_launch_names++] = LaunchCount{name, 1};
}

bool adj_fused_eligible(const matcha_shape& s, const matcha_frozen& f);

struct Workspace : TokenChain {
  float* folded;
  float* enc;
  float* enc_rec; size_t enc_rec_floats;
  float* merged;
  float* frag;
  float* fb_ws;
  float* tslab;
  float* tpart;
  float* tslab2;
  float* qkv;
  float* front_ws;
  float *XN, *x0N, *xhN, *GN; int64_t* node_ids; int32_t* node_cnt;
  float* RN;
  float* VN;
  size_t total;
};

struct OptionName { const char* name; int Options::*field; };
static const OptionName kOptionNames[] = {
    {"disable_fused", &Options::disable_fused}, {"disable_merged", &Options::disable_merged}, {"disable_small_batch", &Options::disable_small_batch},
    {"disable_wide_gemm", &Options::disable_wide_gemm}, {"disable_node_front", &Options::disable_node_front}, {"disable_node_r", &Options::disable_node_r}, {"disable_node_v", &Options::disable_node_v}, {"disable_node_dx", &Options::disable_node_dx}, {"disable_launch_pairs", &Options::disable_launch_pairs}, {"debug_nan", &Options::debug_nan}, {"fused_dbg", &Options::fused_dbg}};
Options& options() {
  static Options o = [] {
    Options v;
    memset(&v, 0, sizeof(v));
    for (const OptionName& n : kOptionNames) {
      char env[64] = "MATCHA_";
      size_t k = strlen(env);
      for (const char* c = n.name; *c && k + 1 < sizeof(env); ++c) env[k++] = (char)((*c >= 'a' && *c <= 'z') ? *c - 32 : *c);
      env[k] = 0;
      const char* e = getenv(env);
      if (e) v.*(n.field) = (*e == 0) ? 1 : atoi(e);
      if (e && v.*(n.field) == 0 && strcmp(e, "0") != 0) v.*(n.field) = 1;
    }
    return v;
  }();
  return o;
}
static bool merged_layerwise_shape(const matcha_shape& s) { return s.d >= 128 && s.d % 64 == 0; }
static bool merged_layerwise(const matcha_shape& s) { return merged_layerwise_shape(s) && attn_wide_eligible(s.d) && !options().disable_merged; }
static bool enc128_enabled(const matcha_shape& s, const matcha_step_opts& o) { return enc128_shape(s.d) && merged_layerwise(s) && options().disable_fused != 1 && !o.deterministic && !o.sparse_table_grad; }
static bool fused_enabled(const matcha_shape& s) { return s.d == 64 && options().disable_fused != 1 && !options().disable_merged; }
static bool node_front_shape(const matcha_shape& s, int64_t B, int L) { return s.mode == 0 && s.d == 64 && front_bwd_supported(s.d, s.n_attr) && B * L + 1 >= 4 * ((int64_t)s.n_nodes + 1); }
static bool node_v_shape(const matcha_shape& s, int64_t B, int L) { return B * L + 1 >= 64 * ((int64_t)s.n_nodes + 1); }
static bool node_dx_shape(const matcha_shape& s, int64_t B, int L) { return node_v_shape(s, B, L); }
static bool has_target(int objective, const float* y, const float* w) { return objective == MATCHA_OBJECTIVE_SOFTPLUS_MSE ? y != nullptr : (y && w); }
static int check_objective(int32_t objective, const char* fn) {
  if (objective == MATCHA_OBJECTIVE_BCE || objective == MATCHA_OBJECTIVE_SOFTPLUS_MSE) return MATCHA_OK;
  set_error("%s: unknown objective %d (MATCHA_OBJECTIVE_BCE or MATCHA_OBJECTIVE_SOFTPLUS_MSE)", fn, (int)objective);
  return MATCHA_EINVAL;
}
static size_t carve(const matcha_shape& s, int64_t B, int L, char* base, Workspace& w, bool compact = false) {
  const int64_t Tn = B * L + 1, d = s.d, hd = (int64_t)MATCHA_N_HEAD * d;
  size_t off = 0;
  auto take_always = [&](size_t n_floats) {
    float* p = base ? (float*)(base + off) : nullptr;
    off += align_up(n_floats * sizeof(float), 256);
    return p;
  };
  auto take = [&](size_t n_floats) { return compact ? (float*)nullptr : take_always(n_floats); };
  {
    const size_t rb = ragged_bytes(B, L);
    if (base) ragged_carve(B, L, base + off, w.rg);
    off += align_up(rb, 256);
  }
  w.x0 = take_always(Tn * d); w.X = take_always(Tn * d);
  w.qin = take(Tn * d); w.kin = take(Tn * d); w.vin = take(Tn * d);
  w.stats = take(Tn * 2);
  w.Q = take(Tn * hd); w.K = take(Tn * hd); w.V = take(Tn * hd);
  w.P = take(B * MATCHA_N_HEAD * L * L);
  w.O = take(Tn * hd);
  w.Y = take(Tn * d); w.H1 = take(Tn * d); w.H2 = take(Tn * d);
  w.row_loss = take_always(B); w.logits = take_always(B);
  w.node = take_always(s.mode == 1 ? Tn * d : 0);
  w.dH2 = take(Tn * d); w.dXs = take(Tn * d); w.dZ1 = take(Tn * d); w.ddyn0 = take(Tn * d);
  w.dO = w.O; w.dQ = w.K; w.dK = w.Q; w.dV = w.V;
  w.dqin = w.qin; w.dkin = w.kin; w.dvin = w.vin;
  w.dZ0 = take(Tn * d); w.dX0 = take(Tn * d);
  chain_scratch_bytes(s, B, L, false, w);
  w.slab = take(w.slab_bytes / sizeof(float));
  w.gemm_ws = take(w.gemm_ws_bytes / sizeof(float));
  w.adj_ws_bytes = (s.mode == 1) ? adj_workspace_bytes(s, Tn) : 0;
  w.adj_ws = take_always(w.adj_ws_bytes / sizeof(float));
  w.folded = take_always(s.d == 64 ? fused_fold_floats() : 0);
  w.frag = take_always(s.d == 64 ? fused_frag_floats() : 0);
  w.merged = take_always(s.d == 64 ? fused_merged_floats() : 0);
  {
    const size_t nm = merged_layerwise_shape(s) ? (size_t)hd * d : 0;
    w.lwB = take_always(nm); w.lwM = take_always(nm);
    w.lwdB = take(nm); w.lwdM = take(nm);
  }
  w.enc = take_always(enc128_shape((int)d) ? enc128_ws_floats() : 0);
  w.enc_rec = w.Q;
  w.enc_rec_floats = (w.Q && w.O) ? (size_t)((w.O + Tn * hd) - w.Q) : 0;
  w.fb_ws = take(s.d == 64 ? fused_bwd_ws_floats(B, L) : 0);
  w.tpart = take(s.d == 64 ? fused_tail_partial_floats() : 0);
  w.tslab = take(s.d == 64 ? fused_tail_slab32_floats(B, L) : 0);
  w.tslab2 = take(s.d == 64 ? tail_bwd_slab_floats() : 0);
  w.qkv = take(s.d == 64 ? fused_qkv_floats(B, L) : 0);
  w.front_ws = take(front_bwd_supported(s.d, s.n_attr) ? front_bwd_ws_floats() : 0);
  w.tg_ws_bytes = (s.mode == 0 && !compact) ? table_grad_ws_bytes(Tn, s.n_nodes) : 0;
  w.tg_ws = take(w.tg_ws_bytes / sizeof(float));
  {
    const size_t nn = node_front_shape(s, B, L) ? (size_t)(s.n_nodes + 1) : 0;
    w.XN = take_always(nn * 64); w.x0N = take(nn * 64); w.xhN = take(nn * 64); w.GN = take(nn * 64);
    w.node_ids = reinterpret_cast<int64_t*>(take_always(nn * 2));
    w.node_cnt = reinterpret_cast<int32_t*>(take_always(nn ? 64 : 0));
    w.RN = nn ? (compact ? take_always(node_r_floats((int64_t)nn)) : w.Q) : nullptr;
    w.VN = (nn && !compact && w.Q) ? w.Q + node_r_floats((int64_t)nn) : nullptr;
  }
  w.total = off;
  return off;
}

static bool compact_forward(const matcha_shape& s, const matcha_step_opts& o, bool force_layerwise) { return !force_layerwise && o.forward_only && fused_enabled(s); }
static StepRoute decide_route(const matcha_shape& s, const matcha_step_opts& o, int64_t B, int L, const Workspace& w, const matcha_frozen& f,
                              const float* y, const float* w_bce, int objective, bool force_layerwise, bool want_losses) {
  StepRoute r;
  r.compact = compact_forward(s, o, force_layerwise);
  r.fused = !force_layerwise && fused_enabled(s);
  r.merged_layerwise = merged_layerwise(s);
  r.enc128 = !force_layerwise && enc128_enabled(s, o) && (o.forward_only || enc128_rec_floats(w.rg) <= w.enc_rec_floats);
  r.half_plan = fused_enabled(s) || r.enc128;
  r.front = r.fused && front_bwd_supported(s.d, s.n_attr) && (options().disable_fused & 2) == 0;
  r.adj_fused = r.front && s.mode == 1 && adj_fused_eligible(s, f);
  r.small = r.fused && fused_small_batch(w.rg);
  const bool atomics = !o.deterministic && !o.sparse_table_grad;
  r.node = r.front && node_front_shape(s, B, L) && !r.small && atomics && !options().disable_node_front;
  r.node_r = r.node && !options().disable_node_r;
  r.node_v = r.node_r && !o.forward_only && w.VN && node_v_shape(s, B, L) && !options().disable_node_v;
  r.lif = r.fused && o.loss_in_forward && !o.forward_only && has_target(objective, y, w_bce);
  r.split_tail = r.lif && !r.small && (options().fused_dbg & 1) == 0;
  r.dx_zeroed = r.lif && atomics && (r.split_tail || r.small) && want_losses;
  r.node_dx = r.node_v && r.lif && r.split_tail && r.dx_zeroed && node_dx_shape(s, B, L) && !options().disable_node_dx;
  r.paired = r.fused && !options().disable_launch_pairs;
  r.long_rows = false;
  return r;
}
static NodeOperands node_operands(const StepRoute& r, const matcha_shape& s, const Workspace& w) {
  const int64_t rows = (int64_t)s.n_nodes + 1;
  return r.node ? NodeOperands{w.XN, w.rg.tok_key, w.xhN, r.node_r ? w.RN : nullptr, r.node_v ? w.VN : nullptr, rows} : NodeOperands{w.X, nullptr, nullptr, nullptr, nullptr, rows};
}

static int check_shape(const matcha_shape* s, int64_t B, int32_t L) {
  MATCHA_TRY(check_shape_fields(s, nullptr));
  MATCHA_CHECK_ARG(L >= 1 && L <= MATCHA_MAX_L, "L=%d outside 1..%d", L, MATCHA_MAX_L);
  MATCHA_CHECK_ARG(B >= 1 && B * (int64_t)L < (1ll << 31) - 2, "B=%lld must be >= 1 and B*L < 2^31", (long long)B);
  MATCHA_CHECK_ARG(s->d == 64 || B * (int64_t)L + 1 <= 65535ll * 128, "B*L=%lld exceeds the %lld token rows the layer-by-layer kernels (embed_dim != 64) launch",
                   (long long)(B * (int64_t)L), 65535ll * 128);
  return MATCHA_OK;
}

}

using namespace matcha;

extern "C" int matcha_abi_version(void) { return MATCHA_ABI_VERSION; }
extern "C" const char* matcha_last_error(void) { return g_err; }
extern "C" int matcha_device_count(void) {
  int n = 0;
  if (hipGetDeviceCount(&n) != hipSuccess) { (void)hipGetLastError(); return 0; }
  return n;
}

extern "C" int matcha_profile_select(int32_t kernel_class) {
  g_prof_class = kernel_class;
  g_prof_used = 0;
  g_prof_work = 0.0;
  return MATCHA_OK;
}

extern "C" int matcha_launch_log(int32_t on) {
  if (on) g_launch_names = 0;
  g_launch_log = on ? 1 : 0;
  return MATCHA_OK;
}

extern "C" int matcha_launch_log_read(char* out, size_t cap) {
  MATCHA_CHECK_ARG(out && cap > 0, "matcha_launch_log_read: null buffer");
  size_t n = 0;
  out[0] = 0;
  for (int i = 0; i < g_launch_names; ++i) {
    const int k = snprintf(out + n, cap - n, "%s %lld\n", g_launches[i].name, (long long)g_launches[i].n);
    if (k < 0 || (size_t)k >= cap - n) { set_error("matcha_launch_log_read: buffer too small"); return MATCHA_ENOMEM; }
    n += (size_t)k;
  }
  return MATCHA_OK;
}

extern "C" int matcha_profile_read(double* total_ms, int64_t* launches, double* work) {
  double ms = 0.0;
  for (int i = 0; i + 1 < g_prof_used; i += 2) {
    if (hipEventSynchronize(g_prof_ev[i + 1]) != hipSuccess) { set_error("matcha_profile_read: event sync failed"); return MATCHA_EHIP; }
    float t = 0.f;
    if (hipEventElapsedTime(&t, g_prof_ev[i], g_prof_ev[i + 1]) != hipSuccess) { set_error("matcha_profile_read: elapsed failed"); return MATCHA_EHIP; }
    ms += t;
  }
  if (total_ms) *total_ms = ms;
  if (launches) *launches = g_prof_used / 2;
  if (work) *work = g_prof_work;
  g_prof_used = 0;
  g_prof_work = 0.0;
  return MATCHA_OK;
}

extern "C" size_t matcha_workspace_bytes(const matcha_shape* shp, int64_t B, int32_t L) {
  if (check_shape(shp, B, L) != MATCHA_OK) return 0;
  Workspace w;
  return carve(*shp, B, L, nullptr, w);
}

extern "C" size_t matcha_workspace_bytes_forward(const matcha_shape* shp, int64_t B, int32_t L) {
  if (check_shape(shp, B, L) != MATCHA_OK) return 0;
  Workspace w;
  return carve(*shp, B, L, nullptr, w, fused_enabled(*shp));
}

static int forward_impl(const matcha_shape* shp, const matcha_tensors* params, const matcha_frozen* frozen,
                        const matcha_step_opts* opts, const int64_t* x, int64_t B, int32_t L, const float* y,
                        const float* w_bce, float* logits, float* losses, void* ws, size_t ws_bytes,
                        matcha_stream_t stream, bool force_layerwise, bool stop_before_head, int objective) {
  MATCHA_TRY(check_shape(shp, B, L));
  MATCHA_CHECK_ARG(params && frozen && opts && x && ws, "matcha_forward: null pointer");
  MATCHA_CHECK_ARG(((uintptr_t)ws) % 256 == 0, "matcha_forward: workspace must be 256-byte aligned");
  const matcha_shape& s = *shp;
  const matcha_tensors& p = *params;
  hipStream_t st = (hipStream_t)stream;
  Workspace w;
  const size_t need = carve(s, B, L, (char*)ws, w, compact_forward(s, *opts, force_layerwise));
  if (ws_bytes < need) { set_error("matcha_forward: workspace %zu < %zu bytes", ws_bytes, need); return MATCHA_ENOMEM; }
  const int64_t Tn = B * L + 1;
  const bool train = opts->training != 0;
  MATCHA_CHECK_ARG(!train || opts->seed || (opts->p_drop_adj <= 0 && opts->p_drop_fc1 <= 0 && opts->p_drop_pff <= 0),
                   "matcha_forward: training with dropout needs opts->seed");
  MATCHA_TRY(check_chain_params(p, *frozen, "matcha_forward"));
  const int32_t* cnt = w.rg.count;
  const int64_t* ids = w.rg.tok_id;

  const StepRoute route = decide_route(s, *opts, B, L, w, *frozen, y, w_bce, objective, force_layerwise, losses != nullptr);
  const bool keep = !opts->forward_only;
  const NodeOperands nx = node_operands(route, s, w);
  const bool tgt = has_target(objective, y, w_bce);
  PlanDeferred deferred;
  deferred.pending = false;
  MATCHA_TRY(launch_ragged_plan(x, B, L, s.n_nodes, opts->status, w.rg, st, route.half_plan ? 1 : 0, route.node ? w.node_ids : nullptr, route.node ? w.node_cnt : nullptr,
                                (route.node && keep) ? w.GN : nullptr,
                                (route.paired && route.node) ? &deferred : nullptr));
  float* recon_out = losses ? losses + 1 : nullptr;
  const bool recon_zero_in_loss = s.mode == 0 && recon_out && route.fused && tgt;
  if (s.mode == 0) MATCHA_CHECK_ARG(p.table, "matcha_forward: table mode without table");
  const ChainCall chain{s, p, *frozen, *opts, B, L, st, {route.merged_layerwise, false, keep}, "matcha_forward"};
  if (!route.front) {
    MATCHA_TRY(chain_front_fwd(chain, w, recon_out, !recon_zero_in_loss));
  } else if (s.mode == 0) {
    if (recon_out && !recon_zero_in_loss) MATCHA_TRY(zero_async(recon_out, 2 * sizeof(float), st));
  } else if (route.adj_fused) {
    MATCHA_TRY(adj_forward(s, p, *frozen, *opts, ids, Tn, nullptr, recon_out, w.adj_ws, w.adj_ws_bytes, st, cnt, w.rg.tok_slot, keep ? w.x0 : nullptr, w.X, keep));
  } else {
    MATCHA_TRY(adj_forward(s, p, *frozen, *opts, ids, Tn, w.node, recon_out, w.adj_ws, w.adj_ws_bytes, st, cnt, w.rg.tok_slot));
  }
  const bool prep_in_front = route.front && !route.adj_fused;
  if (prep_in_front) {
    const PrepSpec prep = {&p, w.folded, w.merged, w.frag};
    if (route.node) {
      MATCHA_TRY(launch_front_fwd(p, w.node_ids, p.table, nullptr, *frozen, s.n_attr, w.rg, nx.rows, keep ? w.x0N : nullptr, nx.X, st, &prep, w.node_cnt,
                                  deferred.pending ? &deferred.pack : nullptr));
      if (keep) MATCHA_TRY(launch_node_xhat(nx.X, w.node_cnt, nx.rows, nx.xhat, st));
      if (nx.rn) MATCHA_TRY(launch_node_r(nx.X, w.frag, nx.rows, nx.rn, st, nx.vn, deferred.pending ? &deferred.compact : nullptr));
      else if (deferred.pending) MATCHA_TRY(launch_tile_compact(deferred.compact, st));
    } else
    MATCHA_TRY(launch_front_fwd(p, ids, s.mode == 0 ? p.table : nullptr, s.mode == 0 ? nullptr : w.node, *frozen, s.n_attr, w.rg, Tn, keep ? w.x0 : nullptr, w.X, st, &prep));
  }
  if (keep) note_forward(ws, route); else forget_forward(ws);
  if (route.fused) {
    const bool save = keep && !route.lif;
    if (!prep_in_front) MATCHA_TRY(launch_prep_heads(p, w.folded, w.merged, w.frag, st));
    float* lg_out = (logits && !save) ? logits : w.logits;
    FusedFwdLaunch a;
    a.frag = w.frag; a.small = route.small; a.y = y; a.w = w_bce; a.objective = objective; a.logits = lg_out; a.row_loss = w.row_loss;
    a.x = nx;
    a.Y = keep ? w.Y : nullptr; a.H1 = keep ? w.H1 : nullptr; a.H2 = keep ? w.H2 : nullptr; a.rimg = keep ? w.qkv : nullptr;
    a.seed = opts->seed; a.p_fc1 = train ? opts->p_drop_fc1 : 0.f; a.p_pff = train ? opts->p_drop_pff : 0.f; a.alpha = opts->alpha;
    a.ddyn0 = route.lif ? w.ddyn0 : nullptr; a.dXs = w.dXs; a.tslab = w.tslab; a.tail_dh2 = route.split_tail ? w.dH2 : nullptr;
    a.dxs_node = route.node_dx ? w.GN : nullptr;
    MATCHA_CHECK_ARG(!route.node_dx || nx.rows <= Tn, "matcha_forward: the heads' per-node d x_hat rows do not fit dO");
    MATCHA_TRY(launch_fused_fwd32(p, w.rg, B, L, a, st));
    if (route.split_tail)
      MATCHA_TRY(launch_tail_bwd64(p, w.dH2, w.Y, w.H1, w.rg, opts->seed, a.p_fc1, a.p_pff, w.ddyn0, w.tslab2, w.tslab, route.dx_zeroed ? w.dO : nullptr,
                                   route.node_dx ? (int64_t)MATCHA_N_HEAD * nx.rows * 64 : 0, st, w.row_loss, B, tgt ? losses : nullptr, recon_zero_in_loss));
    const bool zero_in_loss = route.dx_zeroed && !route.split_tail;
    if (tgt && losses && !route.split_tail)
      MATCHA_TRY(launch_loss_reduce(w.row_loss, B, losses, st, recon_zero_in_loss, zero_in_loss ? w.dO : nullptr, zero_in_loss ? (size_t)Tn * 64 * sizeof(float) : 0));
    if (logits && lg_out != logits && hipMemcpyAsync(logits, w.logits, B * sizeof(float), hipMemcpyDeviceToDevice, st) != hipSuccess) {
      set_error("logits copy failed"); return MATCHA_EHIP;
    }
    return MATCHA_OK;
  }
  if (route.enc128) {
    MATCHA_TRY(merged_weights(s, p, w, st));
    MATCHA_TRY(launch_enc128_fwd(p, w.lwB, w.lwM, w.X, w.rg, B, L, w.Y, keep ? w.enc_rec : nullptr, w.enc, w.rg.tok_slot, opts->seed,
                                 (train && opts->p_drop_fc1 > 0.f) ? opts->p_drop_fc1 : 0.f, st));
  } else {
    MATCHA_TRY(chain_attn_fwd(chain, w));
  }
  return chain_tail_fwd(chain, w, y, w_bce, logits, losses, objective, stop_before_head);
}

extern "C" int matcha_forward(const matcha_shape* shp, const matcha_tensors* params, const matcha_frozen* frozen,
                              const matcha_step_opts* opts, const int64_t* x, int64_t B, int32_t L, const float* y,
                              const float* w_bce, float* logits, float* losses, void* ws, size_t ws_bytes,
                              matcha_stream_t stream) {
  return forward_impl(shp, params, frozen, opts, x, B, L, y, w_bce, logits, losses, ws, ws_bytes, stream, false, false, MATCHA_OBJECTIVE_BCE);
}

extern "C" int matcha_forward_objective(int32_t objective, const matcha_shape* shp, const matcha_tensors* params, const matcha_frozen* frozen,
                                        const matcha_step_opts* opts, const int64_t* x, int64_t B, int32_t L, const float* y,
                                        const float* w, float* logits, float* losses, void* ws, size_t ws_bytes, matcha_stream_t stream) {
  MATCHA_TRY(check_objective(objective, "matcha_forward_objective"));
  return forward_impl(shp, params, frozen, opts, x, B, L, y, w, logits, losses, ws, ws_bytes, stream, false, false, objective);
}

extern "C" int matcha_get_embedding(const matcha_shape* shp, const matcha_tensors* params, const matcha_frozen* frozen,
                                    const matcha_step_opts* opts, const int64_t* x, int64_t B, int32_t L, float* dynamic,
                                    float* static_, float* attn, float* losses, void* ws, size_t ws_bytes, matcha_stream_t stream) {
  MATCHA_CHECK_ARG(dynamic && static_ && opts, "matcha_get_embedding: null pointer");
  matcha_step_opts o = *opts;
  o.forward_only = 0;
  o.loss_in_forward = 0;
  MATCHA_TRY(forward_impl(shp, params, frozen, &o, x, B, L, nullptr, nullptr, nullptr, losses, ws, ws_bytes, stream, true, true, MATCHA_OBJECTIVE_BCE));
  Workspace w;
  carve(*shp, B, L, (char*)ws, w);
  if (attn && hipMemcpyAsync(attn, w.P, (size_t)B * MATCHA_N_HEAD * L * L * sizeof(float), hipMemcpyDeviceToDevice, (hipStream_t)stream) != hipSuccess) {
    set_error("matcha_get_embedding: attention copy failed"); return MATCHA_EHIP;
  }
  return launch_expand_embedding(x, B, L, shp->d, w.rg.row_off, w.H2, w.X, params->pff_ln_g, params->pff_ln_b, dynamic, static_, (hipStream_t)stream);
}

extern "C" int matcha_debug_layout(const matcha_shape* shp, int64_t B, int32_t L, char* out, size_t cap) {
  MATCHA_TRY(check_shape(shp, B, L));
  MATCHA_CHECK_ARG(out && cap > 0, "matcha_debug_layout: null buffer");
  Workspace w;
  char* const base = reinterpret_cast<char*>((uintptr_t)1 << 20);
  const size_t total = carve(*shp, B, L, base, w);
  struct { const char* name; const void* p; } f[] = {
      {"plan", w.rg.row_off}, {"x0", w.x0}, {"X", w.X}, {"qin", w.qin}, {"kin", w.kin}, {"vin", w.vin}, {"stats", w.stats}, {"Q", w.Q}, {"K", w.K}, {"V", w.V},
      {"P", w.P}, {"O_dxh", w.O}, {"Y", w.Y}, {"H1", w.H1}, {"H2", w.H2}, {"row_loss", w.row_loss}, {"logits", w.logits}, {"node", w.node}, {"dH2", w.dH2},
      {"dXs", w.dXs}, {"dZ1", w.dZ1}, {"ddyn0", w.ddyn0}, {"dZ0", w.dZ0}, {"dX0", w.dX0}, {"slab", w.slab}, {"gemm_ws", w.gemm_ws}, {"adj_ws", w.adj_ws},
      {"folded", w.folded}, {"frag", w.frag}, {"merged", w.merged}, {"lwB", w.lwB}, {"lwM", w.lwM}, {"lwdB", w.lwdB}, {"lwdM", w.lwdM}, {"enc", w.enc}, {"fb_ws", w.fb_ws},
      {"tpart", w.tpart}, {"tslab", w.tslab}, {"tslab2", w.tslab2}, {"qkv_records", w.qkv}, {"front_ws", w.front_ws}, {"tg_ws", w.tg_ws}, {"XN", w.XN}, {"x0N", w.x0N}, {"xhN", w.xhN}, {"GN", w.GN},
      {"node_ids", w.node_ids}, {"node_cnt", w.node_cnt}, {"RN", w.RN}, {"VN", w.VN}};
  size_t n = 0;
  for (const auto& e : f) {
    if (!e.p) continue;
    const int k = snprintf(out + n, cap - n, "%s %zu\n", e.name, (size_t)((const char*)e.p - base));
    if (k < 0 || (size_t)k >= cap - n) { set_error("matcha_debug_layout: buffer too small"); return MATCHA_ENOMEM; }
    n += (size_t)k;
  }
  const int k = snprintf(out + n, cap - n, "end %zu\n", total);
  if (k < 0 || (size_t)k >= cap - n) { set_error("matcha_debug_layout: buffer too small"); return MATCHA_ENOMEM; }
  return MATCHA_OK;
}

extern "C" int matcha_random_chrom_dev_supported(const matcha_shape* shp, const matcha_frozen* frozen) {
  if (!shp || !frozen) return 0;
  if (shp->mode == 0) return 1;
  return adj_fused_eligible(*shp, *frozen) && fused_enabled(*shp) && front_bwd_supported(shp->d, shp->n_attr) ? 1 : 0;
}

extern "C" int matcha_set_option(const char* name, int32_t value) {
  MATCHA_CHECK_ARG(name, "matcha_set_option: null name");
  for (const OptionName& n : kOptionNames)
    if (strcmp(n.name, name) == 0) { options().*(n.field) = value; return MATCHA_OK; }
  set_error("matcha_set_option: unknown option '%s'", name);
  return MATCHA_EINVAL;
}

extern "C" int32_t matcha_get_option(const char* name) {
  if (!name) return -1;
  for (const OptionName& n : kOptionNames)
    if (strcmp(n.name, name) == 0) return options().*(n.field);
  return -1;
}

extern "C" int matcha_table_grad_rows(const matcha_shape* shp, int64_t B, int32_t L, void* ws, size_t ws_bytes,
                                      const int32_t** ids, const float** rows, const int32_t** n_tokens, int64_t* cap) {
  MATCHA_TRY(check_shape(shp, B, L));
  MATCHA_CHECK_ARG(ws && ids && rows && cap, "matcha_table_grad_rows: null pointer");
  MATCHA_CHECK_ARG(shp->mode == 0, "matcha_table_grad_rows: table mode only");
  Workspace w;
  const size_t need = carve(*shp, B, L, (char*)ws, w);
  if (ws_bytes < need) { set_error("matcha_table_grad_rows: workspace %zu < %zu bytes", ws_bytes, need); return MATCHA_ENOMEM; }
  *ids = w.rg.tok_key;
  *rows = w.dX0;
  if (n_tokens) *n_tokens = w.rg.count + 1;
  *cap = B * (int64_t)L + 1;
  return MATCHA_OK;
}

static int backward_impl(const matcha_shape* shp, const matcha_tensors* params, const matcha_frozen* frozen,
                         const matcha_step_opts* opts, const int64_t* x, int64_t B, int32_t L, const float* y,
                         const float* w_bce, const float* dlogits, const float* drecon, matcha_tensors* grads,
                         int32_t* touched, void* ws, size_t ws_bytes, matcha_stream_t stream, int objective) {
  MATCHA_TRY(check_shape(shp, B, L));
  MATCHA_CHECK_ARG(params && frozen && opts && x && ws && grads, "matcha_backward: null pointer");
  MATCHA_CHECK_ARG(dlogits || has_target(objective, y, w_bce),
                   objective == MATCHA_OBJECTIVE_BCE ? "matcha_backward: need dlogits or (y, w)" : "matcha_backward: need dlogits or y");
  const matcha_shape& s = *shp;
  const matcha_tensors& p = *params;
  matcha_tensors& g_ = *grads;
  hipStream_t st = (hipStream_t)stream;
  Workspace w;
  const size_t need = carve(s, B, L, (char*)ws, w);
  if (ws_bytes < need) { set_error("matcha_backward: workspace %zu < %zu bytes", ws_bytes, need); return MATCHA_ENOMEM; }
  const int64_t Tn = B * L + 1;
  const int64_t* ids = w.rg.tok_id;

  StepRoute route;
  MATCHA_CHECK_ARG(recorded_route(ws, route) && !route.long_rows,
                   "matcha_backward: no matcha_forward on record for this workspace (one backward per forward, same ws pointer)");
  MATCHA_CHECK_ARG(!route.fused || route.lif == (opts->loss_in_forward && has_target(objective, y, w_bce)),
                   "matcha_backward: loss_in_forward / targets differ from the forward's on this workspace");
  MATCHA_CHECK_ARG(!(route.lif && dlogits), "matcha_backward: opts->loss_in_forward excludes an explicit dlogits");
  forget_forward(ws);
  const bool tail_in_bwd = route.lif && (route.split_tail || route.small);
  const bool dx_zeroed = route.dx_zeroed && !opts->deterministic && !opts->sparse_table_grad;
  TailReduceArgs tail_args;
  const NodeOperands nx = node_operands(route, s, w);
  const ChainCall chain{s, p, *frozen, *opts, B, L, st, {route.merged_layerwise, false, true}, "matcha_backward"};
  if (route.lif) {
    if (route.split_tail) tail_reduce_args(w.tslab2, w.rg, L, g_, true, tail_bwd_grid(), true, tail_args);
    else if (route.small) tail_reduce_args(w.tslab, w.rg, L, g_, true, -1, false, tail_args);
    else MATCHA_TRY(launch_tail_reduce(w.tslab, w.rg, L, g_, st, true, w.tpart));
  } else {
    MATCHA_TRY(chain_tail_bwd(chain, w, nx.X, nx.xrow, y, w_bce, dlogits, objective, g_));
  }
  if (route.fused) {
    const bool dx_atomic = !opts->deterministic && !opts->sparse_table_grad;
    MATCHA_CHECK_ARG(!route.node || dx_atomic, "matcha_backward: deterministic / sparse_table_grad differ from the forward's on this workspace");
    FusedBwdLaunch a;
    a.folded = w.folded; a.merged = w.merged; a.x = nx; a.dDyn = w.ddyn0; a.dXs = w.dXs; a.rimg = w.qkv;
    a.dxh = w.dO; a.ws = w.fb_ws; a.dZ0 = route.front ? nullptr : w.dZ0;
    a.dx_atomic = dx_atomic; a.dx_zeroed = dx_zeroed; a.tail = tail_in_bwd ? &tail_args : nullptr;
    a.dx_node = route.node_dx;
    Unfold2Args unfold2;
    const bool unfold2_in_scatter = route.paired && route.front && route.node;
    a.paired = route.paired; a.unfold2 = unfold2_in_scatter ? &unfold2 : nullptr;
    MATCHA_CHECK_ARG(!route.node_dx || (dx_zeroed && nx.rows <= Tn), "matcha_backward: the heads' per-node d x_hat rows do not fit dO");
    MATCHA_TRY(launch_fused_bwd_merged(p, w.rg, B, L, a, g_, st));
    if (!unfold2_in_scatter) MATCHA_TRY(encoder_done(*opts, st));
    if (route.front) {
      if (s.mode == 0) MATCHA_CHECK_ARG(g_.table, "matcha_backward: table mode without a table gradient buffer");
      if (route.node) {
        MATCHA_TRY(launch_node_scatter(nx.X, w.dO, fused_bwd_dxpad(w.fb_ws), w.dXs, w.rg, Tn, w.GN, st, route.node_dx ? w.node_cnt : nullptr, nx.rows,
                                       unfold2_in_scatter ? &unfold2 : nullptr));
        if (unfold2_in_scatter) MATCHA_TRY(encoder_done(*opts, st));
        MATCHA_TRY(launch_front_bwd(p, nx.X, nullptr, 1, nx.rows, fused_bwd_dxpad(w.fb_ws), w.GN, w.x0N, w.node_ids, *frozen, s.n_attr, w.rg, nullptr, g_.table, w.front_ws, g_, st, touched, w.node_cnt));
        return MATCHA_OK;
      }
      const bool rows_out = s.mode == 1 || opts->deterministic || opts->sparse_table_grad;
      MATCHA_TRY(launch_front_bwd(p, w.X, w.dO, dx_atomic ? 1 : MATCHA_N_HEAD, Tn, fused_bwd_dxpad(w.fb_ws), w.dXs, w.x0, ids, *frozen, s.n_attr, w.rg,
                                  rows_out ? w.dX0 : nullptr, rows_out ? nullptr : g_.table, w.front_ws, g_, st, s.mode == 0 ? touched : nullptr));
      if (s.mode == 0) MATCHA_TRY(table_gradient(s, *opts, w, Tn, g_, st));
      else MATCHA_TRY(adj_backward(s, p, *frozen, *opts, ids, Tn, w.dX0, drecon, g_, touched, w.adj_ws, w.adj_ws_bytes, w.gemm_ws, w.gemm_ws_bytes, st, w.rg.tok_slot, route.adj_fused));
      return MATCHA_OK;
    }
  } else if (route.enc128) {
    MATCHA_TRY(launch_enc128_bwd(p, w.lwB, w.lwM, w.X, w.ddyn0, w.dXs, w.rg, B, L, w.dqin, w.enc_rec, w.enc, w.lwdB, w.lwdM, g_, w.dZ0, st));
    MATCHA_TRY(merged_chain(s, p, g_, w, st));
    MATCHA_TRY(encoder_done(*opts, st));
  } else {
    MATCHA_TRY(chain_attn_bwd(chain, w, g_));
  }
  return chain_front_bwd(chain, w, drecon, g_, touched);
}

extern "C" int matcha_backward(const matcha_shape* shp, const matcha_tensors* params, const matcha_frozen* frozen,
                               const matcha_step_opts* opts, const int64_t* x, int64_t B, int32_t L, const float* y,
                               const float* w_bce, const float* dlogits, const float* drecon, matcha_tensors* grads,
                               int32_t* touched, void* ws, size_t ws_bytes, matcha_stream_t stream) {
  return backward_impl(shp, params, frozen, opts, x, B, L, y, w_bce, dlogits, drecon, grads, touched, ws, ws_bytes, stream, MATCHA_OBJECTIVE_BCE);
}

extern "C" int matcha_backward_objective(int32_t objective, const matcha_shape* shp, const matcha_tensors* params, const matcha_frozen* frozen,
                                         const matcha_step_opts* opts, const int64_t* x, int64_t B, int32_t L, const float* y,
                                         const float* w, const float* dlogits, const float* drecon, matcha_tensors* grads,
                                         int32_t* touched, void* ws, size_t ws_bytes, matcha_stream_t stream) {
  MATCHA_TRY(check_objective(objective, "matcha_backward_objective"));
  return backward_impl(shp, params, frozen, opts, x, B, L, y, w, dlogits, drecon, grads, touched, ws, ws_bytes, stream, objective);
}

extern "C" int matcha_node_embeddings(const matcha_shape* shp, const matcha_tensors* params, const matcha_frozen* frozen,
                                      const int64_t* ids, int64_t T, float* rows, void* ws, size_t ws_bytes,
                                      int32_t* status, matcha_stream_t stream) {
  MATCHA_CHECK_ARG(shp && params && frozen && ids && rows, "matcha_node_embeddings: null pointer");
  MATCHA_CHECK_ARG(shp->d >= 4 && shp->d <= 256 && shp->d % 4 == 0, "matcha_node_embeddings: d=%d", shp->d);
  hipStream_t st = (hipStream_t)stream;
  if (shp->mode == 0) {
    MATCHA_CHECK_ARG(params->table, "matcha_node_embeddings: null table");
    return launch_gather_rows(ids, T, shp->d, params->table, shp->n_nodes, rows, status, st);
  }
  MATCHA_TRY(launch_check_ids(ids, T, shp->n_nodes, status, st));
  matcha_step_opts o;
  memset(&o, 0, sizeof(o));
  o.random_chrom = -1;
  MATCHA_CHECK_ARG(ws && ws_bytes >= adj_workspace_bytes(*shp, T), "matcha_node_embeddings: adj mode needs a workspace of matcha_workspace_bytes()");
  return adj_forward(*shp, *params, *frozen, o, ids, T, rows, nullptr, ws, ws_bytes, st, nullptr, nullptr, nullptr, nullptr, false, true);
}
```

### matcha_amd/csrc/ragged.hip

```cpp
#include "kernels.hpp"
#include "ragged_roles.hpp"

namespace matcha {

constexpr int kRpt = 1;
constexpr int kRowsPerBlock = 256 * kRpt;

__device__ __forceinline__ int block_exclusive_scan_256(int v, int* lds4, int* total) {
  const int lane = threadIdx.x & 63, wave = threadIdx.x >> 6;
  int incl = v;
#pragma unroll
  for (int o = 1; o < 64; o <<= 1) {
    const int u = __shfl_up(incl, o, 64);
    if (lane >= o) incl += u;
  }
  if (lane == 63) lds4[wave] = incl;
  __syncthreads();
  int base = 0;
  for (int w = 0; w < wave; ++w) base += lds4[w];
  if (total) *total = lds4[0] + lds4[1] + lds4[2] + lds4[3];
  return base + incl - v;
}

__global__ __launch_bounds__(256) void row_count_kernel(const int64_t* __restrict__ x, int64_t B, int L, int32_t* __restrict__ blk_sum) {
  __shared__ int lds4[4];
  const int64_t b0 = (int64_t)blockIdx.x * kRowsPerBlock + threadIdx.x * kRpt;
  int cnt = 0;
  for (int i = 0; i < kRpt; ++i)
    if (b0 + i < B)
      for (int l = 0; l < L; ++l) cnt += x[(b0 + i) * L + l] != 0 ? 1 : 0;
  int total;
  (void)block_exclusive_scan_256(cnt, lds4, &total);
  if (threadIdx.x == 0) blk_sum[blockIdx.x] = total;
}

__global__ __launch_bounds__(1024) void row_scan_kernel(int32_t* __restrict__ blk_sum, int nblk, int32_t* __restrict__ count,
                                                        int32_t* __restrict__ sb_first, int nsb, int32_t n_rows) {
  __shared__ int part[1024];
  for (int i = threadIdx.x; i <= nsb; i += 1024) sb_first[i] = n_rows;
  const int chunk = (nblk + 1023) / 1024;
  const int b0 = threadIdx.x * chunk, b1 = (b0 + chunk < nblk) ? b0 + chunk : nblk;
  int local = 0;
  for (int b = b0; b < b1; ++b) local += blk_sum[b];
  __shared__ int wtot[16];
  const int lane = threadIdx.x & 63, wave = threadIdx.x >> 6;
  int incl = local;
#pragma unroll
  for (int o = 1; o < 64; o <<= 1) {
    const int u = __shfl_up(incl, o, 64);
    if (lane >= o) incl += u;
  }
  if (lane == 63) wtot[wave] = incl;
  __syncthreads();
  int wbase = 0, total = 0;
#pragma unroll
  for (int w2 = 0; w2 < 16; ++w2) { const int v = wtot[w2]; if (w2 < wave) wbase += v; total += v; }
  part[threadIdx.x] = wbase + incl - local;
  if (threadIdx.x == 0) {
    count[0] = total + 1;
    count[1] = total;
  }
  int run = part[threadIdx.x];
  for (int b = b0; b < b1; ++b) { const int v = blk_sum[b]; blk_sum[b] = run; run += v; }
}

__global__ __launch_bounds__(256) void row_fill_kernel(const int64_t* __restrict__ x, int64_t B, int L, const int32_t* __restrict__ blk_base,
                                                       const int32_t* __restrict__ count, int32_t* __restrict__ row_off,
                                                       int32_t* __restrict__ tok_slot, int64_t* __restrict__ tok_id,
                                                       int32_t* __restrict__ tok_pos, int32_t* __restrict__ sb_first, int super_tok,
                                                       int32_t* __restrict__ tok_key, int64_t n_nodes, int32_t* __restrict__ status,
                                                       int64_t* __restrict__ node_ids, int32_t* __restrict__ node_cnt, float* __restrict__ node_zero) {
  __shared__ int lds4[4];
  const int64_t b0 = (int64_t)blockIdx.x * kRowsPerBlock + threadIdx.x * kRpt;
  int64_t v[kRpt][MATCHA_MAX_L], vp[MATCHA_MAX_L];
#pragma unroll
  for (int i = 0; i < kRpt; ++i) {
    const int64_t bc = b0 + i < B ? b0 + i : B - 1;
#pragma unroll
    for (int l = 0; l < MATCHA_MAX_L; ++l) v[i][l] = x[bc * L + (l < L ? l : L - 1)];
  }
  {
    const int64_t bp = b0 > 0 ? (b0 - 1 < B ? b0 - 1 : B - 1) : 0;
#pragma unroll
    for (int l = 0; l < MATCHA_MAX_L; ++l) vp[l] = x[bp * L + (l < L ? l : L - 1)];
  }
  int kk[kRpt], cnt = 0;
#pragma unroll
  for (int i = 0; i < kRpt; ++i) {
    int k = 0;
#pragma unroll
    for (int l = 0; l < MATCHA_MAX_L; ++l) {
      v[i][l] = (b0 + i < B && l < L) ? v[i][l] : 0;
      k += v[i][l] != 0 ? 1 : 0;
    }
    kk[i] = k;
    cnt += k;
  }
  int kprev = 0;
#pragma unroll
  for (int l = 0; l < MATCHA_MAX_L; ++l) kprev += (b0 > 0 && l < L && vp[l] != 0) ? 1 : 0;
  int pos = blk_base[blockIdx.x] + block_exclusive_scan_256(cnt, lds4, nullptr);
#pragma unroll
  for (int i = 0; i < kRpt; ++i) {
    const int64_t b = b0 + i;
    if (b < B) {
      row_off[b] = pos;
      const int k = kk[i];
      if (b == 0 || pos / super_tok != (pos - kprev) / super_tok) sb_first[pos / super_tok] = (int32_t)b;
      kprev = k;
      int nth = 0;
#pragma unroll
      for (int l = 0; l < MATCHA_MAX_L; ++l) {
        int64_t id = v[i][l];
        if (id != 0) {
          if (id < 0 || id > n_nodes) {
            if (status) atomicOr(status, MATCHA_STATUS_BAD_ID);
            id = 0;
          }
          tok_slot[pos] = (int32_t)(b * L + l); tok_id[pos] = id; tok_key[pos] = (int32_t)id; tok_pos[pos] = nth | (k << 8); ++pos; ++nth;
        }
      }
    }
  }
  const int tr = count[1];
  if (blockIdx.x == 0 && threadIdx.x == 0) {
    row_off[B] = tr;
    tok_slot[tr] = (int32_t)(B * L);
    tok_id[tr] = 0;
    tok_pos[tr] = 0;
  }
  for (int64_t i = tr + (int64_t)blockIdx.x * 256 + threadIdx.x; i < B * L + 1; i += (int64_t)gridDim.x * 256) tok_key[i] = 0;
  if (node_ids) {
    for (int64_t i = (int64_t)blockIdx.x * 256 + threadIdx.x; i <= n_nodes; i += (int64_t)gridDim.x * 256) node_ids[i] = i;
    if (blockIdx.x == 0 && threadIdx.x == 0) { node_cnt[0] = (int32_t)(n_nodes + 1); node_cnt[1] = (int32_t)n_nodes; }
  }
  if (node_zero)
    for (int64_t i = (int64_t)blockIdx.x * 256 + threadIdx.x; i < (n_nodes + 1) * 16; i += (int64_t)gridDim.x * 256)
      reinterpret_cast<float4*>(node_zero)[i] = make_float4(0.f, 0.f, 0.f, 0.f);
}

__global__ __launch_bounds__(64) void tile_pack_kernel(TilePackArgs a) {
  tile_pack_role(a, (int)blockIdx.y * a.nsb + (int)blockIdx.x, threadIdx.x);
}

__global__ __launch_bounds__(1024) void tile_compact_kernel(CompactArgs a) {
  const int nsb = a.nsb, x0 = a.first;
  int32_t* __restrict__ count = a.count;
  const int which = (int)blockIdx.x + x0;
  if (x0 != 0 && threadIdx.x == 0) count[2] = 0;
  const int32_t* __restrict__ sb_tiles = a.sb_tiles[which];
  int32_t* __restrict__ sb_cnt = a.sb_cnt[which];
  const int cap_per_sb = a.cap_per_sb[which], ntiles_cap = a.ntiles_cap[which];
  int32_t* __restrict__ meta = a.meta[which];
  __shared__ int wtot[16];
  __shared__ int carry;
  if (threadIdx.x == 0) carry = 0;
  __syncthreads();
  const int lane = threadIdx.x & 63, wave = threadIdx.x >> 6;
  for (int base = 0; base < nsb; base += 1024) {
    const int i = base + threadIdx.x;
    const int c = i < nsb ? sb_cnt[i] : 0;
    int incl = c;
#pragma unroll
    for (int o = 1; o < 64; o <<= 1) {
      const int u = __shfl_up(incl, o, 64);
      if (lane >= o) incl += u;
    }
    if (lane == 63) wtot[wave] = incl;
    __syncthreads();
    int wbase = 0, tot = 0;
#pragma unroll
    for (int w2 = 0; w2 < 16; ++w2) { const int v = wtot[w2]; if (w2 < wave) wbase += v; tot += v; }
    if (i < nsb) sb_cnt[i] = carry + wbase + incl - c;
    __syncthreads();
    if (threadIdx.x == 0) carry += tot;
    __syncthreads();
  }
  const int total = carry < ntiles_cap ? carry : ntiles_cap;
  if (threadIdx.x == 0) count[2 + which] = total;
  __syncthreads();
  const int4* __restrict__ src = reinterpret_cast<const int4*>(sb_tiles);
  int4* __restrict__ dst = reinterpret_cast<int4*>(meta);
  __shared__ int offs[1025];
  if (nsb <= 1024) {
    for (int i = threadIdx.x; i < nsb; i += 1024) offs[i] = sb_cnt[i];
    if (threadIdx.x == 0) offs[nsb] = total;
    __syncthreads();
    for (int i0 = threadIdx.x; i0 < total; i0 += 4 * 1024) {
      int4 v[4];
#pragma unroll
      for (int u = 0; u < 4; ++u) {
// ... 107 lines not shown
                                  reinterpret_cast<int4*>(a.sb_tiles[which]) + (int64_t)sb * a.cap_per_sb[which], lane);
    if (lane == 0) cnt[which][sb] = nt;
  }
  __syncthreads();
  for (int which = first; which < 2; ++which) {
    int off[kSmallSb + 1];
    int run = 0;
    for (int sb = 0; sb < a.nsb; ++sb) { off[sb] = run; run += cnt[which][sb]; }
    const int tot = run < a.ntiles_cap[which] ? run : a.ntiles_cap[which];
    if (tid == 0) a.count[2 + which] = tot;
    const int4* src = reinterpret_cast<const int4*>(a.sb_tiles[which]);
    int4* dst = reinterpret_cast<int4*>(a.meta[which]);
    for (int sb = wave; sb < a.nsb; sb += 16)
      for (int j = lane; j < cnt[which][sb]; j += 64)
        if (off[sb] + j < a.ntiles_cap[which]) dst[off[sb] + j] = src[(int64_t)sb * a.cap_per_sb[which] + j];
    for (int i = tot + tid; i < a.ntiles_cap[which] + 2; i += 1024) dst[i] = make_int4(0, 0, 0, 0);
  }
  if (first != 0 && tid == 0) a.count[2] = 0;
  if (a.level >= 2) {
    __syncthreads();
    const int4* tm = reinterpret_cast<const int4*>(a.meta[0]);
    for (int t = wave; t < a.ntiles_cap[0]; t += 16) {
      const int4 m = tm[t];
      if (lane < m.y) a.tok_tile[m.x + lane] = (int32_t)((t << 6) | lane);
    }
  }
}

static inline int super_blocks(int64_t T) { return (int)cdiv(T + 1, kSuperTok); }
static inline int super_cap(int L) { return (int)cdiv(kSuperTok + L, 64 - L) + 2; }
static inline int tiles_cap(int64_t T, int L) { return (int)cdiv(T + 1, 64 - L) + super_blocks(T); }
static inline int super_hcap(int L) { return (int)cdiv(kSuperTok + L, 32 - L) + 2; }
static inline int halves_cap(int64_t T, int L) { return (int)cdiv(T + 1, 32 - L) + super_blocks(T); }

int ragged_tiles_cap(int64_t B, int L) { return tiles_cap(B * L, L); }
int ragged_halves_cap(int64_t B, int L) { return halves_cap(B * L, L); }

size_t ragged_bytes(int64_t B, int L) {
  const int64_t T = B * L;
  size_t n = 0;
  n += align_up((size_t)(B + 1) * 4, 256);
  n += align_up((size_t)(T + 1) * 4, 256);
  n += align_up((size_t)(T + 1) * 8, 256);
  n += 256;
  n += align_up((size_t)cdiv(B, kRowsPerBlock) * 4, 256);
  n += align_up((size_t)(T + 1) * 4, 256);
  n += align_up((size_t)(T + 1) * 4, 256);
  n += align_up((size_t)(tiles_cap(T, L) + 2) * 16, 256);
  n += align_up((size_t)super_blocks(T) * super_cap(L) * 16, 256);
  n += align_up((size_t)super_blocks(T) * 4, 256);
  n += align_up((size_t)(super_blocks(T) + 1) * 4, 256);
  n += align_up((size_t)(halves_cap(T, L) + 2) * 16, 256);
  n += align_up((size_t)super_blocks(T) * super_hcap(L) * 16, 256);
  n += align_up((size_t)super_blocks(T) * 4, 256);
  n += align_up((size_t)(T + 1) * 4, 256);
  return n;
}

void ragged_carve(int64_t B, int L, char* base, Ragged& r) {
  const int64_t T = B * L;
  size_t off = 0;
  auto take = [&](size_t bytes) { char* p = base + off; off += align_up(bytes, 256); return p; };
  r.row_off = (int32_t*)take((size_t)(B + 1) * 4);
  r.tok_slot = (int32_t*)take((size_t)(T + 1) * 4);
  r.tok_id = (int64_t*)take((size_t)(T + 1) * 8);
  r.count = (int32_t*)take(256);
  r.blk_sum = (int32_t*)take((size_t)cdiv(B, kRowsPerBlock) * 4);
  r.nblk = (int)cdiv(B, kRowsPerBlock);
  r.ntiles = tiles_cap(T, L);
  r.tok_pos = (int32_t*)take((size_t)(T + 1) * 4);
  r.tok_key = (int32_t*)take((size_t)(T + 1) * 4);
  r.tile_meta = (int32_t*)take((size_t)(r.ntiles + 2) * 16);
  r.nsb = super_blocks(T);
  r.sb_cap = super_cap(L);
  r.sb_tiles = (int32_t*)take((size_t)r.nsb * r.sb_cap * 16);
  r.sb_cnt = (int32_t*)take((size_t)r.nsb * 4);
  r.sb_first = (int32_t*)take((size_t)(r.nsb + 1) * 4);
  r.nhalves = halves_cap(T, L);
  r.sb_hcap = super_hcap(L);
  r.half_meta = (int32_t*)take((size_t)(r.nhalves + 2) * 16);
  r.sb_htiles = (int32_t*)take((size_t)r.nsb * r.sb_hcap * 16);
  r.sb_hcnt = (int32_t*)take((size_t)r.nsb * 4);
  r.tok_tile = (int32_t*)take((size_t)(T + 1) * 4);
}

int launch_tile_pack(const TilePackArgs& a, hipStream_t st) {
  hipLaunchKernelGGL(tile_pack_kernel, dim3(a.nsb, 2 - a.first), dim3(64), 0, st, a);
  MATCHA_CHECK_LAUNCH("tile_pack_kernel");
  return MATCHA_OK;
}
int launch_tile_compact(const CompactArgs& a, hipStream_t st) {
  hipLaunchKernelGGL(tile_compact_kernel, dim3(2 - a.first), dim3(1024), 0, st, a);
  MATCHA_CHECK_LAUNCH("tile_compact_kernel");
  return MATCHA_OK;
}

int launch_ragged_plan(const int64_t* x, int64_t B, int L, int64_t n_nodes, int32_t* status, const Ragged& r, hipStream_t st, int level,
                       int64_t* node_ids, int32_t* node_cnt, float* node_zero, PlanDeferred* defer) {
  if (defer) defer->pending = false;
  if (B <= kSmallRows && r.nsb <= kSmallSb && !options().disable_small_batch) {
    PlanSmallArgs a;
    a.x = x; a.B = B; a.L = L; a.n_nodes = n_nodes; a.status = status;
    a.row_off = r.row_off; a.tok_slot = r.tok_slot; a.tok_id = r.tok_id; a.tok_pos = r.tok_pos; a.tok_key = r.tok_key; a.count = r.count; a.sb_first = r.sb_first;
    a.nsb = r.nsb; a.level = level;
    a.sb_tiles[0] = r.sb_tiles; a.cap_per_sb[0] = r.sb_cap; a.ntiles_cap[0] = r.ntiles; a.meta[0] = r.tile_meta;
    a.sb_tiles[1] = r.sb_htiles; a.cap_per_sb[1] = r.sb_hcap; a.ntiles_cap[1] = r.nhalves; a.meta[1] = r.half_meta;
    a.tok_tile = r.tok_tile;
    a.node_ids = node_ids; a.node_cnt = node_cnt; a.node_zero = node_zero;
    hipLaunchKernelGGL(plan_small_kernel, dim3(1), dim3(1024), 0, st, a);
    MATCHA_CHECK_LAUNCH("plan_small_kernel");
    return MATCHA_OK;
  }
  hipLaunchKernelGGL(row_count_kernel, dim3(r.nblk), dim3(256), 0, st, x, B, L, r.blk_sum);
  MATCHA_CHECK_LAUNCH("row_count_kernel");
  hipLaunchKernelGGL(row_scan_kernel, dim3(1), dim3(1024), 0, st, r.blk_sum, r.nblk, r.count, r.sb_first, r.nsb, (int32_t)B);
  MATCHA_CHECK_LAUNCH("row_scan_kernel");
  hipLaunchKernelGGL(row_fill_kernel, dim3(r.nblk), dim3(256), 0, st, x, B, L, r.blk_sum, r.count, r.row_off, r.tok_slot, r.tok_id, r.tok_pos, r.sb_first, kSuperTok,
                     r.tok_key, n_nodes, status, node_ids, node_cnt, node_zero);
  MATCHA_CHECK_LAUNCH("row_fill_kernel");
  if (level <= 0) return MATCHA_OK;
  const int first = level >= 2 ? 0 : 1;
  TilePackArgs pa;
  pa.row_off = r.row_off; pa.B = B; pa.nsb = r.nsb; pa.sb_first = r.sb_first; pa.first = first; pa.ntasks = r.nsb * (2 - first);
  pa.cap_per_sb[0] = r.sb_cap; pa.sb_tiles[0] = r.sb_tiles; pa.sb_cnt[0] = r.sb_cnt;
  pa.cap_per_sb[1] = r.sb_hcap; pa.sb_tiles[1] = r.sb_htiles; pa.sb_cnt[1] = r.sb_hcnt;
  CompactArgs ca;
  ca.sb_tiles[0] = r.sb_tiles; ca.sb_cnt[0] = r.sb_cnt; ca.cap_per_sb[0] = r.sb_cap; ca.ntiles_cap[0] = r.ntiles; ca.meta[0] = r.tile_meta;
  ca.sb_tiles[1] = r.sb_htiles; ca.sb_cnt[1] = r.sb_hcnt; ca.cap_per_sb[1] = r.sb_hcap; ca.ntiles_cap[1] = r.nhalves; ca.meta[1] = r.half_meta;
  ca.nsb = r.nsb; ca.count = r.count; ca.first = first;
  if (defer && level == 1) {
    defer->pending = true; defer->pack = pa; defer->compact = ca;
    return MATCHA_OK;
  }
  MATCHA_TRY(launch_tile_pack(pa, st));
  MATCHA_TRY(launch_tile_compact(ca, st));
  if (level >= 2) {
    hipLaunchKernelGGL(tok_tile_kernel, dim3(r.ntiles), dim3(64), 0, st, r.tile_meta, r.tok_tile);
    MATCHA_CHECK_LAUNCH("tok_tile_kernel");
  }
  return MATCHA_OK;
}

}

using namespace matcha;

extern "C" size_t matcha_ragged_plan_bytes(int64_t B, int32_t L) {
  if (B < 1 || L < 1 || L > MATCHA_MAX_L || B * (int64_t)L >= (1ll << 31) - 2) return 0;
  return ragged_bytes(B, L);
}

extern "C" int matcha_ragged_plan(const int64_t* x, int64_t B, int32_t L, int32_t n_nodes, int32_t* status, void* ws, size_t ws_bytes,
                                  matcha_ragged_view* view, matcha_stream_t stream) {
  MATCHA_CHECK_ARG(x && ws && view, "matcha_ragged_plan: null pointer");
  MATCHA_CHECK_ARG(B >= 1 && L >= 1 && L <= MATCHA_MAX_L && B * (int64_t)L < (1ll << 31) - 2, "matcha_ragged_plan: B=%lld L=%d", (long long)B, L);
  MATCHA_CHECK_ARG(n_nodes >= 1, "matcha_ragged_plan: n_nodes=%d", n_nodes);
  MATCHA_CHECK_ARG(((uintptr_t)ws) % 256 == 0, "matcha_ragged_plan: workspace must be 256-byte aligned");
  if (ws_bytes < ragged_bytes(B, L)) { set_error("matcha_ragged_plan: workspace %zu < %zu bytes", ws_bytes, ragged_bytes(B, L)); return MATCHA_ENOMEM; }
  Ragged r;
  ragged_carve(B, L, (char*)ws, r);
  view->row_off = r.row_off; view->tok_slot = r.tok_slot; view->tok_id = r.tok_id; view->tok_key = r.tok_key; view->tok_pos = r.tok_pos;
  view->count = r.count; view->tile_meta = r.tile_meta; view->tiles_cap = r.ntiles;
  view->half_meta = r.half_meta; view->halves_cap = r.nhalves; view->tok_tile = r.tok_tile;
  return launch_ragged_plan(x, B, L, n_nodes, status, r, (hipStream_t)stream, 2);
}
```

### matcha_amd/csrc/token_kernels.hip

```cpp
#include <string.h>

#include "attr_src.hpp"
#include "kernels.hpp"
#include "loss_reduce.hpp"
#include "token_row.hpp"

namespace matcha {

template <int NCH>
__device__ __forceinline__ float dot_rows(const Row& a, const Row& b) {
  float s = 0.f;
#pragma unroll
  for (int c = 0; c < NCH; ++c) s += (a.v[c].x * b.v[c].x + a.v[c].y * b.v[c].y) + (a.v[c].z * b.v[c].z + a.v[c].w * b.v[c].w);
  return s;
}
template <int NCH>
__device__ __forceinline__ float sum_row(const Row& a) {
  float s = 0.f;
#pragma unroll
  for (int c = 0; c < NCH; ++c) s += (a.v[c].x + a.v[c].y) + (a.v[c].z + a.v[c].w);
  return s;
}
#define ROW_FOREACH(NCH, expr)                                    \
  _Pragma("unroll") for (int c = 0; c < NCH; ++c) {               \
// ... 310 lines not shown
    if (t >= T) break;
    Row x, xh, dq, dk, dv, dxh, dx, ds;
    load_row<NCH>(X + t * d, s, d, x);
    float mean, rstd;
    row_stats<NCH>(x, s, d, mean, rstd);
    normalize<NCH>(x, s, d, mean, rstd, xh);
    load_row<NCH>(dqin + t * d, s, d, dq);
    load_row<NCH>(dkin + t * d, s, d, dk);
    load_row<NCH>(dvin + t * d, s, d, dv);
    acc_mul_row<NCH>(part[0], dq, xh); acc_row<NCH>(part[1], dq);
    acc_mul_row<NCH>(part[2], dk, xh); acc_row<NCH>(part[3], dk);
    acc_mul_row<NCH>(part[4], dv, xh); acc_row<NCH>(part[5], dv);
    mul_rows<NCH>(dq, Gq, dxh);
    acc_mul_row<NCH>(dxh, dk, Gk);
    acc_mul_row<NCH>(dxh, dv, Gv);
    ln_bwd_row<NCH>(dxh, xh, rstd, s, d, dx);
    load_row<NCH>(dXs + t * d, s, d, ds);
#pragma unroll
    for (int c = 0; c < NCH; ++c) {
      dx.v[c].x = (dx.v[c].x + ds.v[c].x) * (1.f - x.v[c].x * x.v[c].x);
      dx.v[c].y = (dx.v[c].y + ds.v[c].y) * (1.f - x.v[c].y * x.v[c].y);
      dx.v[c].z = (dx.v[c].z + ds.v[c].z) * (1.f - x.v[c].z * x.v[c].z);
      dx.v[c].w = (dx.v[c].w + ds.v[c].w) * (1.f - x.v[c].w * x.v[c].w);
    }
    store_row<NCH>(dZ0 + t * d, s, d, dx);
  }
  block_colsum_store<NCH, 6>(part, d, slab + (int64_t)blockIdx.x * 6 * d, lds);
}

template <int NCH>
__global__ __launch_bounds__(256) void head_fwd_kernel(const int32_t* __restrict__ row_off, const float* __restrict__ H2,
                                                       const float* __restrict__ X, int64_t B, int L, int d, HeadParams hp,
                                                       const float* __restrict__ y, const float* __restrict__ w,
                                                       float* __restrict__ logits, float* __restrict__ row_loss, int objective) {
  const int s = threadIdx.x & 15;
  const int64_t b = (int64_t)blockIdx.x * 16 + (threadIdx.x >> 4);
  if (b >= B) return;
  Row Gp, Bp, G1, B1, G2, B2, Wc;
  load_row<NCH>(hp.gp, s, d, Gp); load_row<NCH>(hp.bp, s, d, Bp);
  load_row<NCH>(hp.g1, s, d, G1); load_row<NCH>(hp.b1, s, d, B1);
  load_row<NCH>(hp.g2, s, d, G2); load_row<NCH>(hp.b2, s, d, B2);
  load_row<NCH>(hp.wc, s, d, Wc);
  const float bc = hp.bc[0];
  float total = 0.f, cnt = 0.f;
  const int t_lo = row_off[b], t_hi = row_off[b + 1];
  for (int64_t t = t_lo; t < t_hi; ++t) {
    Row h, hh, u, uh, dn, xr, xh, sn;
    float m, r;
    load_row<NCH>(H2 + t * d, s, d, h);
    row_stats<NCH>(h, s, d, m, r); normalize<NCH>(h, s, d, m, r, hh); affine<NCH>(hh, Gp, Bp, u);
    row_stats<NCH>(u, s, d, m, r); normalize<NCH>(u, s, d, m, r, uh); affine<NCH>(uh, G1, B1, dn);
    load_row<NCH>(X + t * d, s, d, xr);
    row_stats<NCH>(xr, s, d, m, r); normalize<NCH>(xr, s, d, m, r, xh); affine<NCH>(xh, G2, B2, sn);
    float o = 0.f;
#pragma unroll
    for (int c = 0; c < NCH; ++c) {
      const float a = dn.v[c].x - sn.v[c].x, e = dn.v[c].y - sn.v[c].y, f = dn.v[c].z - sn.v[c].z, g = dn.v[c].w - sn.v[c].w;
      o += (a * a * Wc.v[c].x + e * e * Wc.v[c].y) + (f * f * Wc.v[c].z + g * g * Wc.v[c].w);
    }
    o = group_sum<kTPT>(o) + bc;
    total += o;
    cnt += 1.f;
  }
  const float z = total / (cnt + 1e-15f);
  if (s == 0) {
    logits[b] = z;
    if (row_loss && objective == MATCHA_OBJECTIVE_SOFTPLUS_MSE) {
      const float e = (z > 20.f ? z : log1pf(expf(z))) - y[b];
      row_loss[b] = e * e;
    } else if (row_loss) {
      const float yy = y[b];
      row_loss[b] = w[b] * (fmaxf(z, 0.f) - z * yy + log1pf(expf(-fabsf(z))));
    }
  }
}

template <int NCH>
__global__ __launch_bounds__(256) void head_bwd_kernel(const int32_t* __restrict__ row_off, const float* __restrict__ H2,
                                                       const float* __restrict__ X, int64_t B, int L, int d, HeadParams hp,
                                                       const float* __restrict__ y, const float* __restrict__ w,
                                                       const float* __restrict__ logits, const float* __restrict__ dlogits,
                                                       float alpha, float* __restrict__ dH2, float* __restrict__ dXs,
                                                       float* __restrict__ slab, int rows_per_blk, int objective,
                                                       const int32_t* __restrict__ xrow) {
  __shared__ float lds[16 * 256];
  __shared__ float lds_bc[16];
  const int s = threadIdx.x & 15, slot = threadIdx.x >> 4;
  Row Gp, Bp, G1, B1, G2, B2, Wc;
  load_row<NCH>(hp.gp, s, d, Gp); load_row<NCH>(hp.bp, s, d, Bp);
  load_row<NCH>(hp.g1, s, d, G1); load_row<NCH>(hp.b1, s, d, B1);
  load_row<NCH>(hp.g2, s, d, G2); load_row<NCH>(hp.b2, s, d, B2);
  load_row<NCH>(hp.wc, s, d, Wc);
  Row part[7];
#pragma unroll
  for (int v = 0; v < 7; ++v) zero_row<NCH>(part[v]);
  float part_bc = 0.f;
  const int64_t b0 = (int64_t)blockIdx.x * rows_per_blk;
  for (int i = slot; i < rows_per_blk; i += 16) {
    const int64_t b = b0 + i;
    if (b >= B) break;
    const int t_lo = row_off[b], t_hi = row_off[b + 1];
    const float cnt = (float)(t_hi - t_lo);
    float dz;
    if (dlogits) dz = dlogits[b];
    else if (objective == MATCHA_OBJECTIVE_SOFTPLUS_MSE) {
      const float z = logits[b];
      const float e = (z > 20.f ? z : log1pf(expf(z))) - y[b];
      dz = alpha * 2.f * e * (z > 20.f ? 1.f : 1.f / (1.f + expf(-z))) / (float)B;
    } else {
      const float z = logits[b];
      const float sg = 1.f / (1.f + expf(-z));
      dz = alpha * w[b] * (sg - y[b]) / (float)B;
    }
    const float dout = dz / (cnt + 1e-15f);
    for (int64_t t = t_lo; t < t_hi; ++t) {
      Row h, hh, u, uh, dn, xr, xh, sn;
      float m, rh, ru, rx;
      load_row<NCH>(H2 + t * d, s, d, h);
      row_stats<NCH>(h, s, d, m, rh); normalize<NCH>(h, s, d, m, rh, hh); affine<NCH>(hh, Gp, Bp, u);
      row_stats<NCH>(u, s, d, m, ru); normalize<NCH>(u, s, d, m, ru, uh); affine<NCH>(uh, G1, B1, dn);
      load_row<NCH>(X + (xrow ? (int64_t)xrow[t] : t) * d, s, d, xr);
      row_stats<NCH>(xr, s, d, m, rx); normalize<NCH>(xr, s, d, m, rx, xh); affine<NCH>(xh, G2, B2, sn);
      Row ddn, dsn, tmp, du, dhh, dh, dxs;
#pragma unroll
      for (int c = 0; c < NCH; ++c) {
        const float a = dn.v[c].x - sn.v[c].x, e = dn.v[c].y - sn.v[c].y, f = dn.v[c].z - sn.v[c].z, g = dn.v[c].w - sn.v[c].w;
        part[6].v[c].x += a * a * dout; part[6].v[c].y += e * e * dout; part[6].v[c].z += f * f * dout; part[6].v[c].w += g * g * dout;
        ddn.v[c].x = 2.f * a * Wc.v[c].x * dout; ddn.v[c].y = 2.f * e * Wc.v[c].y * dout;
        ddn.v[c].z = 2.f * f * Wc.v[c].z * dout; ddn.v[c].w = 2.f * g * Wc.v[c].w * dout;
        dsn.v[c].x = -ddn.v[c].x; dsn.v[c].y = -ddn.v[c].y; dsn.v[c].z = -ddn.v[c].z; dsn.v[c].w = -ddn.v[c].w;
      }
      if (s == 0) part_bc += dout;
      acc_mul_row<NCH>(part[2], ddn, uh); acc_row<NCH>(part[3], ddn);
      mul_rows<NCH>(ddn, G1, tmp);
      ln_bwd_row<NCH>(tmp, uh, ru, s, d, du);
      acc_mul_row<NCH>(part[0], du, hh); acc_row<NCH>(part[1], du);
      mul_rows<NCH>(du, Gp, dhh);
      ln_bwd_row<NCH>(dhh, hh, rh, s, d, dh);
      store_row<NCH>(dH2 + t * d, s, d, dh);
      acc_mul_row<NCH>(part[4], dsn, xh); acc_row<NCH>(part[5], dsn);
      mul_rows<NCH>(dsn, G2, tmp);
      ln_bwd_row<NCH>(tmp, xh, rx, s, d, dxs);
      store_row<NCH>(dXs + t * d, s, d, dxs);
    }
  }
  if (blockIdx.x == 0 && slot == 0) {
    Row zr;
    zero_row<NCH>(zr);
    const int64_t tp = row_off[B];
    store_row<NCH>(dH2 + tp * d, s, d, zr);
    store_row<NCH>(dXs + tp * d, s, d, zr);
  }
  block_colsum_store<NCH, 7>(part, d, slab + (int64_t)blockIdx.x * (7 * d + 1), lds);
  if (s == 0) lds_bc[slot] = part_bc;
  __syncthreads();
  if (threadIdx.x == 0) {
    float a = 0.f;
    for (int t = 0; t < 16; ++t) a += lds_bc[t];
    slab[(int64_t)blockIdx.x * (7 * d + 1) + 7 * d] = a;
  }
}

__global__ __launch_bounds__(1024) void loss_reduce_kernel(const float* __restrict__ row_loss, int64_t B, float* __restrict__ out, int zero_recon,
                                                           float4* __restrict__ zero_buf, int64_t zero_n4) {
  __shared__ float red[16];
  if (blockIdx.x > 0) {
    for (int64_t i = (int64_t)(blockIdx.x - 1) * 1024 + threadIdx.x; i < zero_n4; i += (int64_t)(gridDim.x - 1) * 1024) zero_buf[i] = make_float4(0.f, 0.f, 0.f, 0.f);
    return;
  }
  loss_reduce_role<1024>(row_loss, B, out, zero_recon, red);
}

struct ColsumDst {
  float* p[8];
};
__global__ __launch_bounds__(1024) void colsum_reduce_kernel(const float* __restrict__ slab, int nblk, int nv, int d, int stride,
                                                             ColsumDst dst) {
  __shared__ float part[16][64];
  const int o = threadIdx.x & 63, q = threadIdx.x >> 6;
  const int i = blockIdx.x * 64 + o;
  float s0 = 0.f, s1 = 0.f;
  if (i < stride) {
    int b = q;
    for (; b + 16 < nblk; b += 32) { s0 += slab[(int64_t)b * stride + i]; s1 += slab[(int64_t)(b + 16) * stride + i]; }
    if (b < nblk) s0 += slab[(int64_t)b * stride + i];
  }
  part[q][o] = s0 + s1;
  __syncthreads();
  if (q == 0 && i < stride) {
    float s = 0.f;
#pragma unroll
    for (int t = 0; t < 16; ++t) s += part[t][o];
    const int v = i / d, j = i - v * d;
    if (dst.p[v]) dst.p[v][j] += s;
  }
// ... 51 lines not shown
  MATCHA_CHECK_ARG(p && bytes % 4 == 0 && (reinterpret_cast<uintptr_t>(p) & 3) == 0, "zero_async: unaligned buffer");
  const int64_t n = (int64_t)(bytes / 4);
  hipLaunchKernelGGL(zero_f32_kernel, dim3((unsigned)cdiv(cdiv(n, 4), 256)), dim3(256), 0, st, (float*)p, n);
  MATCHA_CHECK_LAUNCH("zero_f32_kernel");
  return MATCHA_OK;
}

int launch_fill_i32(int32_t* p, int n, int32_t v, hipStream_t st) {
  if (n <= 0) return MATCHA_OK;
  hipLaunchKernelGGL(fill_i32_kernel, dim3((unsigned)cdiv(n, 64)), dim3(64), 0, st, p, n, v);
  MATCHA_CHECK_LAUNCH("fill_i32_kernel");
  return MATCHA_OK;
}

int launch_embed_scatter(const int64_t* x, int64_t T, int d, const float* dx0, float* dtable, hipStream_t st, const int32_t* t_dev) {
  if (T <= 0) return MATCHA_OK;
  ProfScope ps(MATCHA_PROF_EMBED_SCATTER, (double)T * (8.0 + 8.0 * d), st);
  hipLaunchKernelGGL(embed_scatter_kernel, dim3((unsigned)cdiv(T * d, 256)), dim3(256), 0, st, x, T, d, dx0, dtable, t_dev);
  MATCHA_CHECK_LAUNCH("embed_scatter_kernel");
  return MATCHA_OK;
}

int launch_ln3_fwd(const float* X, int64_t T, int d, const float* gq, const float* bq, const float* gk, const float* bk,
                   const float* gv, const float* bv, float* qin, float* kin, float* vin, float* stats, hipStream_t st, const int32_t* t_dev) {
  if (T <= 0) return MATCHA_OK;
  dim3 grid((unsigned)cdiv(T, 16));
  ProfScope ps(MATCHA_PROF_LN3_FWD, (double)T * 16.0 * d, st);
  DISPATCH_NCH(d, hipLaunchKernelGGL((ln3_fwd_kernel<NCH>), grid, dim3(256), 0, st, X, T, d, gq, bq, gk, bk, gv, bv, qin, kin, vin, stats, t_dev));
  MATCHA_CHECK_LAUNCH("ln3_fwd_kernel");
  return MATCHA_OK;
}

int colsum_blocks(int64_t n, int* per_blk) {
  int64_t blocks = cdiv(n, 64);
  if (blocks > 512) blocks = 512;
  if (blocks < 1) blocks = 1;
  int64_t per = cdiv(cdiv(n, blocks), 16) * 16;
  if (per < 16) per = 16;
  *per_blk = (int)per;
  return (int)cdiv(n, per);
}

int launch_ln3_bwd(const float* X, const float* dqin, const float* dkin, const float* dvin, const float* dXs, int64_t T, int d,
                   const float* gq, const float* gk, const float* gv, float* dZ0, float* slab, float* dgq, float* dbq,
                   float* dgk, float* dbk, float* dgv, float* dbv, hipStream_t st, const int32_t* t_dev) {
  if (T <= 0) return MATCHA_OK;
  int per;
  const int nblk = colsum_blocks(T, &per);
  ProfScope ps(MATCHA_PROF_LN3_BWD, (double)T * 24.0 * d, st);
  DISPATCH_NCH(d, hipLaunchKernelGGL((ln3_bwd_kernel<NCH>), dim3(nblk), dim3(256), 0, st, X, dqin, dkin, dvin, dXs, T, d, gq, gk, gv, dZ0, slab, per, t_dev));
  MATCHA_CHECK_LAUNCH("ln3_bwd_kernel");
  ColsumDst dst = {{dgq, dbq, dgk, dbk, dgv, dbv, nullptr, nullptr}};
  hipLaunchKernelGGL(colsum_reduce_kernel, dim3((unsigned)cdiv(6 * d, 64)), dim3(1024), 0, st, slab, nblk, 6, d, 6 * d, dst);
  MATCHA_CHECK_LAUNCH("colsum_reduce_kernel");
  return MATCHA_OK;
}

int launch_loss_reduce(const float* row_loss, int64_t B, float* bce_out, hipStream_t st, bool zero_recon, float* zero_buf, size_t zero_bytes) {
  MATCHA_CHECK_ARG(zero_bytes % 16 == 0 && (uintptr_t)zero_buf % 16 == 0, "loss_reduce: zero_buf");
  const int64_t n4 = zero_buf ? (int64_t)(zero_bytes / 16) : 0;
  int zb = (int)cdiv(n4, 4096);
  if (zb > 64) zb = 64;
  hipLaunchKernelGGL(loss_reduce_kernel, dim3(1 + zb), dim3(1024), 0, st, row_loss, B, bce_out, zero_recon ? 1 : 0, reinterpret_cast<float4*>(zero_buf), n4);
  MATCHA_CHECK_LAUNCH("loss_reduce_kernel");
  return MATCHA_OK;
}

int launch_head_fwd(const int32_t* row_off, const float* H2, const float* X, int64_t B, int L, int d, const HeadParams& hp,
                    const float* y, const float* w, float* logits, float* row_loss, float* bce_out, hipStream_t st, int objective) {
  if (B <= 0) return MATCHA_OK;
  float* rl = (objective == MATCHA_OBJECTIVE_SOFTPLUS_MSE ? y != nullptr : (y && w)) ? row_loss : nullptr;
  ProfScope ps(MATCHA_PROF_HEAD_FWD, (double)B * L * (8.0 * d + 8.0), st);
  DISPATCH_NCH(d, hipLaunchKernelGGL((head_fwd_kernel<NCH>), dim3((unsigned)cdiv(B, 16)), dim3(256), 0, st, row_off, H2, X, B, L, d, hp, y, w, logits, rl, objective));
  MATCHA_CHECK_LAUNCH("head_fwd_kernel");
  if (rl && bce_out) {
    hipLaunchKernelGGL(loss_reduce_kernel, dim3(1), dim3(1024), 0, st, rl, B, bce_out, 0, (float4*)nullptr, (int64_t)0);
    MATCHA_CHECK_LAUNCH("loss_reduce_kernel");
  }
  return MATCHA_OK;
}

int launch_head_bwd(const int32_t* row_off, const float* H2, const float* X, int64_t B, int L, int d, const HeadParams& hp,
                    const float* y, const float* w, const float* logits, const float* dlogits, float alpha, float* dH2,
                    float* dXs, float* slab, const HeadParams& ghp, hipStream_t st, int objective, const int32_t* xrow) {
  if (B <= 0) return MATCHA_OK;
  int per;
  const int nblk = colsum_blocks(B, &per);
  {
    ProfScope ps(MATCHA_PROF_HEAD_BWD, (double)B * L * (16.0 * d + 8.0), st);
    DISPATCH_NCH(d, hipLaunchKernelGGL((head_bwd_kernel<NCH>), dim3(nblk), dim3(256), 0, st, row_off, H2, X, B, L, d, hp, y, w, logits, dlogits, alpha, dH2, dXs, slab, per, objective, xrow));
  }
  MATCHA_CHECK_LAUNCH("head_bwd_kernel");
  ColsumDst dst = {{(float*)ghp.gp, (float*)ghp.bp, (float*)ghp.g1, (float*)ghp.b1, (float*)ghp.g2, (float*)ghp.b2, (float*)ghp.wc, (float*)ghp.bc}};
  hipLaunchKernelGGL(colsum_reduce_kernel, dim3((unsigned)cdiv(7 * d + 1, 64)), dim3(1024), 0, st, slab, nblk, 7, d, 7 * d + 1, dst);
  MATCHA_CHECK_LAUNCH("colsum_reduce_kernel");
  return MATCHA_OK;
}

size_t colsum_slab_bytes(int64_t n, int nv, int d) {
  int per;
  const int nblk = colsum_blocks(n, &per);
  return align_up(((size_t)nblk * nv * d + nblk) * sizeof(float), 256);
}

}

using namespace matcha;

extern "C" int matcha_embed_fwd(const int64_t* x, int64_t T, int32_t d, const float* table, const float* dense,
                                const float* attr_table, int32_t n_attr, const float* attr_w, const float* attr_b,
                                float* x0, matcha_stream_t stream) {
  MATCHA_CHECK_ARG(x && attr_table && attr_w && attr_b && x0, "matcha_embed_fwd: null pointer");
  MATCHA_CHECK_ARG(d % 4 == 0 && d > 0 && d <= 256, "matcha_embed_fwd: d=%d must be a multiple of 4, <= 256", d);
  matcha_frozen f;
  memset(&f, 0, sizeof(f));
  f.attr_table = attr_table;
  return launch_embed_fwd(x, T, d, table, dense, f, n_attr, attr_w, attr_b, x0, (hipStream_t)stream, nullptr);
}

extern "C" int matcha_embed_scatter_bwd(const int64_t* x, int64_t T, int32_t d, const float* dx0, float* dtable,
                                        matcha_stream_t stream) {
  MATCHA_CHECK_ARG(x && dx0 && dtable, "matcha_embed_scatter_bwd: null pointer");
  return launch_embed_scatter(x, T, d, dx0, dtable, (hipStream_t)stream, nullptr);
}

extern "C" int matcha_ln3_fwd(const float* X, int64_t T, int32_t d, const float* gq, const float* bq, const float* gk,
                              const float* bk, const float* gv, const float* bv, float* qin, float* kin, float* vin,
                              float* stats, matcha_stream_t stream) {
  MATCHA_CHECK_ARG(X && gq && bq && gk && bk && gv && bv && qin && kin && vin, "matcha_ln3_fwd: null pointer");
  MATCHA_CHECK_ARG(d % 4 == 0 && d > 0 && d <= 256, "matcha_ln3_fwd: d=%d must be a multiple of 4, <= 256", d);
  return launch_ln3_fwd(X, T, d, gq, bq, gk, bk, gv, bv, qin, kin, vin, stats, (hipStream_t)stream, nullptr);
}
```

Baseline: 59.66 million hyperedges/s.

## Sort rows by arity within plan blocks and trim attention loops to wave max k

The ragged plan now reorders rows inside each 256-row block by their real arity k and records the permutation in row_ord, which the forward tail and head backward use to map back to the caller's labels and weights. The fused backward attention loops gain a compile-time trip count taken from the wave's maximum k through a ballot, so waves whose hyperedges are all short skip the padded iterations. Sorting is meant to make waves uniform in k so this trimming pays off more often. The cost is extra ballots and scans in the plan kernel, more template instantiations and code size, and row_ord sharing storage with tok_tile, which only works while the plan stops at the half tiles.

```diff
diff --git a/matcha_amd/csrc/fused_bwd.hip b/matcha_amd/csrc/fused_bwd.hip
--- a/matcha_amd/csrc/fused_bwd.hip
+++ b/matcha_amd/csrc/fused_bwd.hip
@@ -28,12 +28,34 @@
 
 #define FB_PIN(addr, x) asm volatile("" : "+v"(addr), "+v"((x).a), "+v"((x).b), "+v"((x).c), "+v"((x).d))
 template <int ML>
+__device__ __forceinline__ int wave_trip_count(int k, bool trim) {
+  int kn = ML;
+  if (trim) {
+    kn = 1;
+#pragma unroll
+    for (int q = 1; q < ML; ++q)
+      if (__ballot(k > q) != 0ull) kn = q + 1;
+  }
+  return kn;
+}
+template <int ML, int KN = 2, class F>
+__device__ __forceinline__ void trip_dispatch(int kn, F&& f) {
+  if constexpr (KN >= ML) {
+    f(std::integral_constant<int, ML>{});
+  } else {
+    if (kn <= KN) f(std::integral_constant<int, KN>{});
+    else trip_dispatch<ML, KN + 1>(kn, f);
+  }
+}
+template <int ML, int KN>
 __device__ __forceinline__ void attn_row8_kv(const float* __restrict__ Qs, const float* __restrict__ Xs, const float* __restrict__ Fs,
                                              const float* __restrict__ xpad, const float* __restrict__ Ps, float* __restrict__ dSs, int li, int li0,
                                              int k, int n_pad, int sub, float inv_temp, V8& o, V8& gq, V8& accK, V8& accV) {
   const float padf = (float)n_pad;
   const bool hp = n_pad > 0;
   float p[ML], ds[ML], pp;
+#pragma unroll
+  for (int j = 0; j < ML; ++j) ds[j] = 0.f;
   {
     const float4 pa = *reinterpret_cast<const float4*>(&Ps[li * 8]), pb = *reinterpret_cast<const float4*>(&Ps[li * 8 + 4]);
     const float w[8] = {pa.x, pa.y, pa.z, pa.w, pb.x, pb.y, pb.z, pb.w};
@@ -51,10 +73,10 @@
   V8 a = scale8(ppf * dsp_raw, vp);
   V8 vn = ld8(&Xs[ro0]), vn2 = ld8(&Xs[ro0 + (1 < k ? 1 : 0) * kLd]);
 #pragma unroll
-  for (int j = 0; j < ML; ++j) {
+  for (int j = 0; j < KN; ++j) {
     const V8 v = vn;
     vn = vn2;
-    if (j + 2 < ML) {
+    if (j + 2 < KN) {
       int ad = ro0 + (j + 2 < k ? j + 2 : 0) * kLd;
       FB_PIN(ad, o);
       vn2 = ld8(&Xs[ad]);
@@ -89,13 +111,15 @@
 }
 
 #define FB_PIN1(addr, s) asm volatile("" : "+v"(addr), "+v"(s))
-template <int ML>
+template <int ML, int KN>
 __device__ __forceinline__ void attn_row8_v(const float* __restrict__ Qs, const float* __restrict__ Xs, const float* __restrict__ Ys, const float* __restrict__ Ds,
                                             const float* __restrict__ xpad, const float* __restrict__ ypad, const float* __restrict__ Ps, float* __restrict__ dSs,
                                             int li, int li0, int k, int n_pad, int sub, float inv_temp, V8& gq, V8& accK, V8& accU) {
   const float padf = (float)n_pad;
   const bool hp = n_pad > 0;
   float p[ML], ds[ML], pp;
+#pragma unroll
+  for (int j = 0; j < ML; ++j) ds[j] = 0.f;
   {
     const float4 pa = *reinterpret_cast<const float4*>(&Ps[li * 8]), pb = *reinterpret_cast<const float4*>(&Ps[li * 8 + 4]);
     const float w[8] = {pa.x, pa.y, pa.z, pa.w, pb.x, pb.y, pb.z, pb.w};
@@ -112,10 +136,10 @@
     V8 vn = ld8(&Ys[ro0]), vn2 = ld8(&Ys[ro0 + (1 < k ? 1 : 0) * kLd]);
     float part = 0.f;
 #pragma unroll
-    for (int j = 0; j < ML; ++j) {
+    for (int j = 0; j < KN; ++j) {
       const V8 v = vn;
       vn = vn2;
-      if (j + 2 < ML) {
+      if (j + 2 < KN) {
         int ad = ro0 + (j + 2 < k ? j + 2 : 0) * kLd;
         FB_PIN1(ad, part);
         vn2 = ld8(&Ys[ad]);
@@ -134,10 +158,10 @@
   {
     V8 vn = ld8(&Xs[ro0]), vn2 = ld8(&Xs[ro0 + (1 < k ? 1 : 0) * kLd]);
 #pragma unroll
-    for (int j = 0; j < ML; ++j) {
+    for (int j = 0; j < KN; ++j) {
       const V8 v = vn;
       vn = vn2;
-      if (j + 2 < ML) {
+      if (j + 2 < KN) {
         int ad = ro0 + (j + 2 < k ? j + 2 : 0) * kLd;
         FB_PIN(ad, gq);
         vn2 = ld8(&Xs[ad]);
@@ -158,7 +182,7 @@
   }
 }
 
-template <int ML>
+template <int ML, int KN>
 __device__ __forceinline__ void attn_col8(const float* __restrict__ Qs, const float* __restrict__ Fs, const float* __restrict__ Ps,
                                           const float* __restrict__ dSs, int li, int li0, int k, int sub, V8& gk, V8& gv) {
   const int jj = li - li0;
@@ -167,12 +191,12 @@
   const int ro0 = li0 * kLd + 8 * sub;
   V8 qn = ld8(&Qs[ro0]), gn = ld8(&Fs[ro0]);
 #pragma unroll
-  for (int i = 0; i < ML; ++i) {
+  for (int i = 0; i < KN; ++i) {
     const V8 q = qn, go = gn;
     const int ri = li0 + (i < k ? i : 0);
     const float pl = Ps[ri * 8 + jj], dl = dSs[ri * 8 + jj];
     const float pij = (i < k) ? pl : 0.f, dsij = (i < k) ? dl : 0.f;
-    if (i + 1 < ML) {
+    if (i + 1 < KN) {
       int a = ro0 + (i + 1 < k ? i + 1 : 0) * kLd;
       FB_PIN(a, gk);
       qn = ld8(&Qs[a]); gn = ld8(&Fs[a]);
@@ -204,6 +228,7 @@
 struct FusedBwdHArgs {
   const float* X; const float* dDyn; const int32_t* count; const int32_t* half_meta; const int32_t* tok_pos;
   int L; int nhalves; int nchunks;
+  int k_trim;
   const float* mB; const float* mM;
   float* dxh; int64_t tcap;
   int dx_atomic;
@@ -433,14 +458,19 @@
       V8 q0, k0, v0;
       const int la = wave * 8 + (lane >> 3);
       const bool acta = la < n_real;
-      int ia = 0;
-      if (acta) { ia = tinfo[la]; attn_row8_v<ML>(Rs, Xs, Fs, Ds, xpad, ypad, Ps, dSs, la, ia & 255, ia >> 8, g.L - (ia >> 8), sub, inv_temp, q0, accK, accV); }
+      const int ia = tinfo[la];
+      const int kn = wave_trip_count<ML>(ia >> 8, g.k_trim != 0);
+      if (acta) trip_dispatch<ML>(kn, [&](auto kc) __attribute__((always_inline)) {
+        attn_row8_v<ML, decltype(kc)::value>(Rs, Xs, Fs, Ds, xpad, ypad, Ps, dSs, la, ia & 255, ia >> 8, g.L - (ia >> 8), sub, inv_temp, q0, accK, accV);
+      });
       __builtin_amdgcn_sched_barrier(0);
       FB_T(2);
       __syncthreads();
       FB_T(7);
       if (acta) {
-        attn_col8<ML>(Rs, Ds, Ps, dSs, la, ia & 255, ia >> 8, sub, k0, v0);
+        trip_dispatch<ML>(kn, [&](auto kc) __attribute__((always_inline)) {
+          attn_col8<ML, decltype(kc)::value>(Rs, Ds, Ps, dSs, la, ia & 255, ia >> 8, sub, k0, v0);
+        });
         st8(&Gs[la * kLd + 8 * sub], k0);
       } else {
         ZR8(&Gs[la * kLd + 8 * sub]);
@@ -456,14 +486,17 @@
       V8 o0, q0, k0, v0;
       const int la = wave * 8 + (lane >> 3);
       const bool acta = la < n_real;
-      int ia = 0;
-      if (acta) { ia = tinfo[la]; attn_row8_kv<ML>(Rs, Xs, Fs, xpad, Ps, dSs, la, ia & 255, ia >> 8, g.L - (ia >> 8), sub, inv_temp, o0, q0, accK, accV); }
+      const int ia = tinfo[la];
+      const int kn = wave_trip_count<ML>(ia >> 8, g.k_trim != 0);
+      if (acta) trip_dispatch<ML>(kn, [&](auto kc) __attribute__((always_inline)) {
+        attn_row8_kv<ML, decltype(kc)::value>(Rs, Xs, Fs, xpad, Ps, dSs, la, ia & 255, ia >> 8, g.L - (ia >> 8), sub, inv_temp, o0, q0, accK, accV);
+      });
       __builtin_amdgcn_sched_barrier(0);
       FB_T(2);
       __syncthreads();
       FB_T(7);
       if (acta) {
-        attn_col8<ML>(Rs, Fs, Ps, dSs, la, ia & 255, ia >> 8, sub, k0, v0);
+        trip_dispatch<ML>(kn, [&](auto kc) __attribute__((always_inline)) { attn_col8<ML, decltype(kc)::value>(Rs, Fs, Ps, dSs, la, ia & 255, ia >> 8, sub, k0, v0); });
         k0.a += v0.a; k0.b += v0.b; k0.c += v0.c; k0.d += v0.d;
         st8(&Gs[la * kLd + 8 * sub], k0);
       } else {
@@ -899,6 +932,7 @@
   {
     FusedBwdHArgs g;
     g.X = xrow ? xhatN : X; g.dDyn = a.dDyn; g.count = rg.count; g.half_meta = rg.half_meta; g.tok_pos = rg.tok_pos; g.L = L; g.nhalves = rg.nhalves; g.nchunks = nchunks;
+    g.k_trim = a.k_trim ? 1 : 0;
     g.mB = mv.B; g.mM = mv.M; g.dxh = dxh; g.tcap = tcap; g.dx_atomic = dx_atomic ? 1 : 0; g.wslab = wslab; g.rimg = a.rimg; g.xrow = xrow;
     g.rn = rn; g.rn_head = a.x.rows * 64; g.vn = vn; g.dx_node = a.dx_node ? dxh : nullptr;
     const size_t lds = kBwdLdsBytes;
diff --git a/matcha_amd/csrc/fused_fwd32.hip b/matcha_amd/csrc/fused_fwd32.hip
--- a/matcha_amd/csrc/fused_fwd32.hip
+++ b/matcha_amd/csrc/fused_fwd32.hip
@@ -201,6 +201,7 @@
   const float* X;
   const int32_t* xrow;
   const int32_t* row_off; const int32_t* tok_slot; const int32_t* count; const int32_t* half_meta; const int32_t* tok_pos;
+  const int32_t* row_ord;
   int L;
   const u32x4* wfrag;
   HeadParams hp;
@@ -666,6 +667,8 @@
   g.rn = a.x.rn; g.rn_rows = (int)a.x.rows;
   g.tail_dh2 = nullptr; g.dxs_node = nullptr;
   g.X = a.x.X; g.row_off = rg.row_off; g.tok_slot = rg.tok_slot; g.count = rg.count; g.half_meta = rg.half_meta; g.tok_pos = rg.tok_pos;
+  MATCHA_CHECK_ARG(!a.small || !a.row_ord, "fused forward: the small-batch kernel runs on the plan in the caller's row order");
+  g.row_ord = a.row_ord;
   g.L = L;
   g.wfrag = reinterpret_cast<const u32x4*>(a.frag);
   g.hp = HeadParams{p.pff_ln_g, p.pff_ln_b, p.ln1_g, p.ln1_b, p.ln2_g, p.ln2_b, p.cls_w, p.cls_b};
diff --git a/matcha_amd/csrc/fused_fwd32_tail.hpp b/matcha_amd/csrc/fused_fwd32_tail.hpp
--- a/matcha_amd/csrc/fused_fwd32_tail.hpp
+++ b/matcha_amd/csrc/fused_fwd32_tail.hpp
@@ -98,9 +98,10 @@
   }
   F32_TAIL_SYNC();
   for (int e = lane; e < n_h; e += 64) {
-    const int64_t b = b0 + e;
-    const int lo_g = g.row_off[b];
-    const int lo = lo_g - t0, kk = g.row_off[b + 1] - lo_g;
+    const int64_t pb = b0 + e;
+    const int64_t b = g.row_ord ? (int64_t)g.row_ord[pb] : pb;
+    const int lo_g = g.row_off[pb];
+    const int lo = lo_g - t0, kk = g.row_off[pb + 1] - lo_g;
     float yb = 0.f, wb = 0.f;
     const bool mse = g.objective == MATCHA_OBJECTIVE_SOFTPLUS_MSE;
     if (g.row_loss) { yb = g.y[b]; wb = mse ? 0.f : g.w[b]; }
diff --git a/matcha_amd/csrc/kernels.hpp b/matcha_amd/csrc/kernels.hpp
--- a/matcha_amd/csrc/kernels.hpp
+++ b/matcha_amd/csrc/kernels.hpp
@@ -48,6 +48,7 @@
   int32_t* sb_htiles;
   int32_t* sb_hcnt;
   int nhalves, sb_hcap;
+  int32_t* row_ord;
 };
 size_t ragged_bytes(int64_t B, int L);
 int ragged_tiles_cap(int64_t B, int L);
@@ -56,7 +57,9 @@
 struct PlanDeferred; struct TilePackArgs; struct CompactArgs;
 int launch_ragged_plan(const int64_t* x, int64_t B, int L, int64_t n_nodes, int32_t* status, const Ragged& r, hipStream_t st, int level = 2,
                        int64_t* node_ids = nullptr, int32_t* node_cnt = nullptr, float* node_zero = nullptr,
-                       PlanDeferred* defer = nullptr);
+                       PlanDeferred* defer = nullptr,
+                       int32_t* row_ord = nullptr);
+bool ragged_plan_small(int64_t B, const Ragged& r);
 
 struct HeadParams {
   const float *gp, *bp, *g1, *b1, *g2, *b2, *wc, *bc;
@@ -107,6 +110,8 @@
   int disable_node_v;
   int disable_node_dx;
   int disable_launch_pairs;
+  int disable_row_sort;
+  int disable_k_trim;
   int debug_nan, fused_dbg;
 };
 Options& options();
@@ -124,7 +129,8 @@
 int launch_head_bwd(const int32_t* row_off, const float* H2, const float* X, int64_t B, int L, int d, const HeadParams& hp,
                     const float* y, const float* w, const float* logits, const float* dlogits, float alpha, float* dH2,
                     float* dXs, float* slab, const HeadParams& ghp, hipStream_t st, int objective = MATCHA_OBJECTIVE_BCE,
-                    const int32_t* xrow = nullptr);
+                    const int32_t* xrow = nullptr,
+                    const int32_t* row_ord = nullptr);
 int launch_head_scores(const int32_t* row_off, const int32_t* tok_slot, const float* H2, const float* X, int64_t B, int L, int d,
                        const HeadParams& hp, float* scores, float* logits, int lowest, int64_t* order, hipStream_t st);
 size_t colsum_slab_bytes(int64_t n, int nv, int d);
@@ -163,6 +169,7 @@
   float *ddyn0, *dXs, *tslab; float alpha;
   float* rimg;
   float* tail_dh2;
+  const int32_t* row_ord = nullptr;
   float* dxs_node = nullptr;
 };
 int launch_fused_fwd32(const matcha_tensors& p, const Ragged& rg, int64_t B, int L, const FusedFwdLaunch& a, hipStream_t st);
@@ -189,6 +196,7 @@
   bool dx_node = false;
   const TailReduceArgs* tail;
   bool paired = false;
+  bool k_trim = false;
   Unfold2Args* unfold2 = nullptr;
 };
 int launch_fused_bwd_merged(const matcha_tensors& p, const Ragged& rg, int64_t B, int L, const FusedBwdLaunch& a, matcha_tensors& grads, hipStream_t st);
diff --git a/matcha_amd/csrc/layerwise.hip b/matcha_amd/csrc/layerwise.hip
--- a/matcha_amd/csrc/layerwise.hip
+++ b/matcha_amd/csrc/layerwise.hip
@@ -208,7 +208,7 @@
 }
 
 int chain_tail_bwd(const ChainCall& c, const TokenChain& w, const float* X, const int32_t* xrow, const float* y, const float* w_bce, const float* dlogits,
-                   int objective, matcha_tensors& g_) {
+                   int objective, matcha_tensors& g_, const int32_t* row_ord) {
   const matcha_tensors& p = c.p;
   const int64_t Tn = c.Tn();
   const int d = c.s.d;
@@ -217,7 +217,7 @@
   const bool drop_fc1 = train && c.o.p_drop_fc1 > 0.f, drop_pff = train && c.o.p_drop_pff > 0.f;
   HeadParams hp = {p.pff_ln_g, p.pff_ln_b, p.ln1_g, p.ln1_b, p.ln2_g, p.ln2_b, p.cls_w, p.cls_b};
   HeadParams ghp = {g_.pff_ln_g, g_.pff_ln_b, g_.ln1_g, g_.ln1_b, g_.ln2_g, g_.ln2_b, g_.cls_w, g_.cls_b};
-  MATCHA_TRY(launch_head_bwd(w.rg.row_off, w.H2, X, c.B, c.L, d, hp, y, w_bce, w.logits, dlogits, c.o.alpha, w.dH2, w.dXs, w.slab, ghp, c.st, objective, xrow));
+  MATCHA_TRY(launch_head_bwd(w.rg.row_off, w.H2, X, c.B, c.L, d, hp, y, w_bce, w.logits, dlogits, c.o.alpha, w.dH2, w.dXs, w.slab, ghp, c.st, objective, xrow, row_ord));
   MATCHA_TRY(launch_gemm_tn(w.dH2, w.H1, g_.pff1_w, g_.pff1_b, d, d, Tn, d, d, nullptr, true, w.gemm_ws, w.gemm_ws_bytes, c.st, cnt));
   {
     GemmArgs g = gemm1(w, w.dH2, p.pff1_w, w.dZ1, Tn, d, d, true);
diff --git a/matcha_amd/csrc/layerwise.hpp b/matcha_amd/csrc/layerwise.hpp
--- a/matcha_amd/csrc/layerwise.hpp
+++ b/matcha_amd/csrc/layerwise.hpp
@@ -50,7 +50,7 @@
 int chain_tail_fwd(const ChainCall& c, const TokenChain& w, const float* y, const float* w_bce, float* logits, float* losses, int objective,
                    bool stop_before_head);
 int chain_tail_bwd(const ChainCall& c, const TokenChain& w, const float* X, const int32_t* xrow, const float* y, const float* w_bce, const float* dlogits,
-                   int objective, matcha_tensors& g);
+                   int objective, matcha_tensors& g, const int32_t* row_ord = nullptr);
 int chain_attn_bwd(const ChainCall& c, const TokenChain& w, matcha_tensors& g);
 int chain_front_bwd(const ChainCall& c, const TokenChain& w, const float* drecon, matcha_tensors& g, int32_t* touched);
 
@@ -71,6 +71,8 @@
   bool node_r, node_v;
   bool node_dx;
   bool paired;
+  bool row_sorted;
+  bool k_trim;
   bool long_rows;
 };
 extern std::unordered_map<const void*, std::pair<StepRoute, uint64_t>> g_fwd_state;
diff --git a/matcha_amd/csrc/model.hip b/matcha_amd/csrc/model.hip
--- a/matcha_amd/csrc/model.hip
+++ b/matcha_amd/csrc/model.hip
@@ -88,7 +88,7 @@
 struct OptionName { const char* name; int Options::*field; };
 static const OptionName kOptionNames[] = {
     {"disable_fused", &Options::disable_fused}, {"disable_merged", &Options::disable_merged}, {"disable_small_batch", &Options::disable_small_batch},
-    {"disable_wide_gemm", &Options::disable_wide_gemm}, {"disable_node_front", &Options::disable_node_front}, {"disable_node_r", &Options::disable_node_r}, {"disable_node_v", &Options::disable_node_v}, {"disable_node_dx", &Options::disable_node_dx}, {"disable_launch_pairs", &Options::disable_launch_pairs}, {"debug_nan", &Options::debug_nan}, {"fused_dbg", &Options::fused_dbg}};
+    {"disable_wide_gemm", &Options::disable_wide_gemm}, {"disable_node_front", &Options::disable_node_front}, {"disable_node_r", &Options::disable_node_r}, {"disable_node_v", &Options::disable_node_v}, {"disable_node_dx", &Options::disable_node_dx}, {"disable_launch_pairs", &Options::disable_launch_pairs}, {"disable_row_sort", &Options::disable_row_sort}, {"disable_k_trim", &Options::disable_k_trim}, {"debug_nan", &Options::debug_nan}, {"fused_dbg", &Options::fused_dbg}};
 Options& options() {
   static Options o = [] {
     Options v;
@@ -203,6 +203,8 @@
   r.dx_zeroed = r.lif && atomics && (r.split_tail || r.small) && want_losses;
   r.node_dx = r.node_v && r.lif && r.split_tail && r.dx_zeroed && node_dx_shape(s, B, L) && !options().disable_node_dx;
   r.paired = r.fused && !options().disable_launch_pairs;
+  r.row_sorted = r.fused && r.half_plan && !r.small && !ragged_plan_small(B, w.rg) && !options().disable_row_sort;
+  r.k_trim = r.fused && !options().disable_k_trim;
   r.long_rows = false;
   return r;
 }
@@ -314,7 +316,7 @@
   deferred.pending = false;
   MATCHA_TRY(launch_ragged_plan(x, B, L, s.n_nodes, opts->status, w.rg, st, route.half_plan ? 1 : 0, route.node ? w.node_ids : nullptr, route.node ? w.node_cnt : nullptr,
                                 (route.node && keep) ? w.GN : nullptr,
-                                (route.paired && route.node) ? &deferred : nullptr));
+                                (route.paired && route.node) ? &deferred : nullptr, route.row_sorted ? w.rg.row_ord : nullptr));
   float* recon_out = losses ? losses + 1 : nullptr;
   const bool recon_zero_in_loss = s.mode == 0 && recon_out && route.fused && tgt;
   if (s.mode == 0) MATCHA_CHECK_ARG(p.table, "matcha_forward: table mode without table");
@@ -352,6 +354,7 @@
     a.seed = opts->seed; a.p_fc1 = train ? opts->p_drop_fc1 : 0.f; a.p_pff = train ? opts->p_drop_pff : 0.f; a.alpha = opts->alpha;
     a.ddyn0 = route.lif ? w.ddyn0 : nullptr; a.dXs = w.dXs; a.tslab = w.tslab; a.tail_dh2 = route.split_tail ? w.dH2 : nullptr;
     a.dxs_node = route.node_dx ? w.GN : nullptr;
+    a.row_ord = route.row_sorted ? w.rg.row_ord : nullptr;
     MATCHA_CHECK_ARG(!route.node_dx || nx.rows <= Tn, "matcha_forward: the heads' per-node d x_hat rows do not fit dO");
     MATCHA_TRY(launch_fused_fwd32(p, w.rg, B, L, a, st));
     if (route.split_tail)
@@ -501,7 +504,7 @@
     else if (route.small) tail_reduce_args(w.tslab, w.rg, L, g_, true, -1, false, tail_args);
     else MATCHA_TRY(launch_tail_reduce(w.tslab, w.rg, L, g_, st, true, w.tpart));
   } else {
-    MATCHA_TRY(chain_tail_bwd(chain, w, nx.X, nx.xrow, y, w_bce, dlogits, objective, g_));
+    MATCHA_TRY(chain_tail_bwd(chain, w, nx.X, nx.xrow, y, w_bce, dlogits, objective, g_, route.row_sorted ? w.rg.row_ord : nullptr));
   }
   if (route.fused) {
     const bool dx_atomic = !opts->deterministic && !opts->sparse_table_grad;
@@ -514,6 +517,7 @@
     Unfold2Args unfold2;
     const bool unfold2_in_scatter = route.paired && route.front && route.node;
     a.paired = route.paired; a.unfold2 = unfold2_in_scatter ? &unfold2 : nullptr;
+    a.k_trim = route.k_trim;
     MATCHA_CHECK_ARG(!route.node_dx || (dx_zeroed && nx.rows <= Tn), "matcha_backward: the heads' per-node d x_hat rows do not fit dO");
     MATCHA_TRY(launch_fused_bwd_merged(p, w.rg, B, L, a, g_, st));
     if (!unfold2_in_scatter) MATCHA_TRY(encoder_done(*opts, st));
diff --git a/matcha_amd/csrc/ragged.hip b/matcha_amd/csrc/ragged.hip
--- a/matcha_amd/csrc/ragged.hip
+++ b/matcha_amd/csrc/ragged.hip
@@ -69,8 +69,12 @@
                                                        int32_t* __restrict__ tok_slot, int64_t* __restrict__ tok_id,
                                                        int32_t* __restrict__ tok_pos, int32_t* __restrict__ sb_first, int super_tok,
                                                        int32_t* __restrict__ tok_key, int64_t n_nodes, int32_t* __restrict__ status,
-                                                       int64_t* __restrict__ node_ids, int32_t* __restrict__ node_cnt, float* __restrict__ node_zero) {
+                                                       int64_t* __restrict__ node_ids, int32_t* __restrict__ node_cnt, float* __restrict__ node_zero,
+                                                       int32_t* __restrict__ row_ord) {
   __shared__ int lds4[4];
+  __shared__ int cls_cnt[4][MATCHA_MAX_L + 2];
+  __shared__ int kmax_front[4];
+  const bool sorted = row_ord != nullptr;
   const int64_t b0 = (int64_t)blockIdx.x * kRowsPerBlock + threadIdx.x * kRpt;
   int64_t v[kRpt][MATCHA_MAX_L], vp[MATCHA_MAX_L];
 #pragma unroll
@@ -79,8 +83,9 @@
 #pragma unroll
     for (int l = 0; l < MATCHA_MAX_L; ++l) v[i][l] = x[bc * L + (l < L ? l : L - 1)];
   }
+  const bool has_front = sorted ? blockIdx.x > 0 : b0 > 0;
   {
-    const int64_t bp = b0 > 0 ? (b0 - 1 < B ? b0 - 1 : B - 1) : 0;
+    const int64_t bp = sorted ? (blockIdx.x > 0 ? b0 - kRowsPerBlock : 0) : (b0 > 0 ? (b0 - 1 < B ? b0 - 1 : B - 1) : 0);
 #pragma unroll
     for (int l = 0; l < MATCHA_MAX_L; ++l) vp[l] = x[bp * L + (l < L ? l : L - 1)];
   }
@@ -98,15 +103,49 @@
   }
   int kprev = 0;
 #pragma unroll
-  for (int l = 0; l < MATCHA_MAX_L; ++l) kprev += (b0 > 0 && l < L && vp[l] != 0) ? 1 : 0;
-  int pos = blk_base[blockIdx.x] + block_exclusive_scan_256(cnt, lds4, nullptr);
+  for (int l = 0; l < MATCHA_MAX_L; ++l) kprev += (has_front && l < L && vp[l] != 0) ? 1 : 0;
+  int pos;
+  int64_t r0 = b0;
+  if (sorted) {
+    static_assert(kRpt == 1, "one row per thread");
+    constexpr int NC = MATCHA_MAX_L + 2;
+    const int lane = threadIdx.x & 63, wave = threadIdx.x >> 6;
+    const int c = b0 < B ? kk[0] : MATCHA_MAX_L + 1;
+    int before = 0;
+#pragma unroll
+    for (int q = 0; q < NC; ++q) {
+      const unsigned long long m = __ballot(c == q);
+      if (lane == 0) cls_cnt[wave][q] = __popcll(m);
+      if (c == q) before = __popcll(m & ((1ull << lane) - 1ull));
+    }
+    int kf = kprev;
+#pragma unroll
+    for (int o = 1; o < 64; o <<= 1) { const int u = __shfl_xor(kf, o, 64); kf = u > kf ? u : kf; }
+    if (lane == 0) kmax_front[wave] = kf;
+    __syncthreads();
+    int start = 0, tok = 0, klow = -1;
+#pragma unroll
+    for (int q = 0; q < NC; ++q) {
+      const int tq = cls_cnt[0][q] + cls_cnt[1][q] + cls_cnt[2][q] + cls_cnt[3][q];
+      if (q < c) { start += tq; tok += q * tq; if (tq > 0) klow = q; }
+    }
+    int same = before;
+    for (int w2 = 0; w2 < wave; ++w2) same += cls_cnt[w2][c];
+    r0 = (int64_t)blockIdx.x * kRowsPerBlock + start + same;
+    pos = blk_base[blockIdx.x] + tok + c * same;
+    const int kfront = max(max(kmax_front[0], kmax_front[1]), max(kmax_front[2], kmax_front[3]));
+    kprev = same > 0 ? c : (klow >= 0 ? klow : kfront);
+  } else {
+    pos = blk_base[blockIdx.x] + block_exclusive_scan_256(cnt, lds4, nullptr);
+  }
 #pragma unroll
   for (int i = 0; i < kRpt; ++i) {
-    const int64_t b = b0 + i;
+    const int64_t b = b0 + i, r = r0 + i;
     if (b < B) {
-      row_off[b] = pos;
+      row_off[r] = pos;
+      if (sorted) row_ord[r] = (int32_t)b;
       const int k = kk[i];
-      if (b == 0 || pos / super_tok != (pos - kprev) / super_tok) sb_first[pos / super_tok] = (int32_t)b;
+      if (r == 0 || pos / super_tok != (pos - kprev) / super_tok) sb_first[pos / super_tok] = (int32_t)r;
       kprev = k;
       int nth = 0;
 #pragma unroll
@@ -380,6 +419,7 @@
   r.sb_htiles = (int32_t*)take((size_t)r.nsb * r.sb_hcap * 16);
   r.sb_hcnt = (int32_t*)take((size_t)r.nsb * 4);
   r.tok_tile = (int32_t*)take((size_t)(T + 1) * 4);
+  r.row_ord = r.tok_tile;
 }
 
 int launch_tile_pack(const TilePackArgs& a, hipStream_t st) {
@@ -393,10 +433,14 @@
   return MATCHA_OK;
 }
 
+bool ragged_plan_small(int64_t B, const Ragged& r) { return B <= kSmallRows && r.nsb <= kSmallSb && !options().disable_small_batch; }
+
 int launch_ragged_plan(const int64_t* x, int64_t B, int L, int64_t n_nodes, int32_t* status, const Ragged& r, hipStream_t st, int level,
-                       int64_t* node_ids, int32_t* node_cnt, float* node_zero, PlanDeferred* defer) {
+                       int64_t* node_ids, int32_t* node_cnt, float* node_zero, PlanDeferred* defer, int32_t* row_ord) {
   if (defer) defer->pending = false;
-  if (B <= kSmallRows && r.nsb <= kSmallSb && !options().disable_small_batch) {
+  MATCHA_CHECK_ARG(!row_ord || level == 1, "ragged plan: only a plan that stops at the half tiles sorts its rows (the order shares tok_tile's bytes)");
+  if (ragged_plan_small(B, r)) {
+    MATCHA_CHECK_ARG(!row_ord, "ragged plan: the one-launch plan of a small batch keeps the caller's row order");
     PlanSmallArgs a;
     a.x = x; a.B = B; a.L = L; a.n_nodes = n_nodes; a.status = status;
     a.row_off = r.row_off; a.tok_slot = r.tok_slot; a.tok_id = r.tok_id; a.tok_pos = r.tok_pos; a.tok_key = r.tok_key; a.count = r.count; a.sb_first = r.sb_first;
@@ -414,7 +458,7 @@
   hipLaunchKernelGGL(row_scan_kernel, dim3(1), dim3(1024), 0, st, r.blk_sum, r.nblk, r.count, r.sb_first, r.nsb, (int32_t)B);
   MATCHA_CHECK_LAUNCH("row_scan_kernel");
   hipLaunchKernelGGL(row_fill_kernel, dim3(r.nblk), dim3(256), 0, st, x, B, L, r.blk_sum, r.count, r.row_off, r.tok_slot, r.tok_id, r.tok_pos, r.sb_first, kSuperTok,
-                     r.tok_key, n_nodes, status, node_ids, node_cnt, node_zero);
+                     r.tok_key, n_nodes, status, node_ids, node_cnt, node_zero, row_ord);
   MATCHA_CHECK_LAUNCH("row_fill_kernel");
   if (level <= 0) return MATCHA_OK;
   const int first = level >= 2 ? 0 : 1;
diff --git a/matcha_amd/csrc/token_kernels.hip b/matcha_amd/csrc/token_kernels.hip
--- a/matcha_amd/csrc/token_kernels.hip
+++ b/matcha_amd/csrc/token_kernels.hip
@@ -416,7 +416,8 @@
                                                        const float* __restrict__ logits, const float* __restrict__ dlogits,
                                                        float alpha, float* __restrict__ dH2, float* __restrict__ dXs,
                                                        float* __restrict__ slab, int rows_per_blk, int objective,
-                                                       const int32_t* __restrict__ xrow) {
+                                                       const int32_t* __restrict__ xrow,
+                                                       const int32_t* __restrict__ row_ord) {
   __shared__ float lds[16 * 256];
   __shared__ float lds_bc[16];
   const int s = threadIdx.x & 15, slot = threadIdx.x >> 4;
@@ -435,16 +436,17 @@
     if (b >= B) break;
     const int t_lo = row_off[b], t_hi = row_off[b + 1];
     const float cnt = (float)(t_hi - t_lo);
+    const int64_t bo = row_ord ? (int64_t)row_ord[b] : b;
     float dz;
-    if (dlogits) dz = dlogits[b];
+    if (dlogits) dz = dlogits[bo];
     else if (objective == MATCHA_OBJECTIVE_SOFTPLUS_MSE) {
-      const float z = logits[b];
-      const float e = (z > 20.f ? z : log1pf(expf(z))) - y[b];
+      const float z = logits[bo];
+      const float e = (z > 20.f ? z : log1pf(expf(z))) - y[bo];
       dz = alpha * 2.f * e * (z > 20.f ? 1.f : 1.f / (1.f + expf(-z))) / (float)B;
     } else {
-      const float z = logits[b];
+      const float z = logits[bo];
       const float sg = 1.f / (1.f + expf(-z));
-      dz = alpha * w[b] * (sg - y[b]) / (float)B;
+      dz = alpha * w[bo] * (sg - y[bo]) / (float)B;
     }
     const float dout = dz / (cnt + 1e-15f);
     for (int64_t t = t_lo; t < t_hi; ++t) {
@@ -662,13 +664,13 @@
 
 int launch_head_bwd(const int32_t* row_off, const float* H2, const float* X, int64_t B, int L, int d, const HeadParams& hp,
                     const float* y, const float* w, const float* logits, const float* dlogits, float alpha, float* dH2,
-                    float* dXs, float* slab, const HeadParams& ghp, hipStream_t st, int objective, const int32_t* xrow) {
+                    float* dXs, float* slab, const HeadParams& ghp, hipStream_t st, int objective, const int32_t* xrow, const int32_t* row_ord) {
   if (B <= 0) return MATCHA_OK;
   int per;
   const int nblk = colsum_blocks(B, &per);
   {
     ProfScope ps(MATCHA_PROF_HEAD_BWD, (double)B * L * (16.0 * d + 8.0), st);
-    DISPATCH_NCH(d, hipLaunchKernelGGL((head_bwd_kernel<NCH>), dim3(nblk), dim3(256), 0, st, row_off, H2, X, B, L, d, hp, y, w, logits, dlogits, alpha, dH2, dXs, slab, per, objective, xrow));
+    DISPATCH_NCH(d, hipLaunchKernelGGL((head_bwd_kernel<NCH>), dim3(nblk), dim3(256), 0, st, row_off, H2, X, B, L, d, hp, y, w, logits, dlogits, alpha, dH2, dXs, slab, per, objective, xrow, row_ord));
   }
   MATCHA_CHECK_LAUNCH("head_bwd_kernel");
   ColsumDst dst = {{(float*)ghp.gp, (float*)ghp.bp, (float*)ghp.g1, (float*)ghp.b1, (float*)ghp.g2, (float*)ghp.b2, (float*)ghp.wc, (float*)ghp.bc}};
```

Result: slower. 58.62 million hyperedges/s (-1.7%).
